# valida-xyz/valida

Measured on AMD Instinct MI355X. Metric: proofs/sec, 2^20-row Fibonacci trace, higher is better.
Workload: dtype u32; 1 GPU; C2: Fibonacci 2^20 cpu rows (mem 2^22), 14 chips, one proof per GPU; field=BabyBear / Ext5, mmcs=Keccak-256, fri_blowup=2, log_blowup=1, num_queries=40, pow_bits=8, parallelism=single GPU, proofs_in_flight_per_gpu=3, comm_stuck=False

## Files before the change

bindings/rust/src/lib.rs:

```rust
#![allow(non_camel_case_types, dead_code)]
use core::ffi::{c_char, c_int, c_void};

pub const VGPU_CBOR_CANONICAL_FIELDS: u32 = 1;
pub const VGPU_CBOR_PLAIN_DIGESTS: u32 = 2;
pub const VGPU_CBOR_IN_BARE_IS_MONTGOMERY: u32 = 1;
pub const VGPU_CBOR_SAW_FIELD_STRUCT: u32 = 1;
pub const VGPU_CBOR_SAW_FIELD_BARE: u32 = 2;
pub const VGPU_CBOR_SAW_DIGEST_STRUCT: u32 = 4;
pub const VGPU_CBOR_SAW_DIGEST_PLAIN: u32 = 8;
pub const VGPU_COMM_ID_BYTES: u32 = 128;
pub const VGPU_OK: i32 = 0;
pub const VGPU_ERR_INVALID_ARG: i32 = -1;
pub const VGPU_ERR_OOM: i32 = -2;
pub const VGPU_ERR_HIP: i32 = -3;
pub const VGPU_ERR_UNSUPPORTED: i32 = -4;
pub const VGPU_ERR_INTERNAL: i32 = -5;
pub const VGPU_ERR_FABRIC: i32 = -6;
pub const VGPU_HASH_KECCAK256: i32 = 0;
pub const VGPU_HASH_POSEIDON16: i32 = 1;
pub const VGPU_CPU_STORE32: i32 = 0;
pub const VGPU_CPU_LOAD32: i32 = 1;
pub const VGPU_CPU_JAL: i32 = 2;
pub const VGPU_CPU_JALV: i32 = 3;
pub const VGPU_CPU_BEQ: i32 = 4;
pub const VGPU_CPU_BNE: i32 = 5;
pub const VGPU_CPU_IMM32: i32 = 6;
pub const VGPU_CPU_BUS: i32 = 7;
pub const VGPU_CPU_BUS_LEFT_IMM: i32 = 8;
pub const VGPU_CPU_STOP: i32 = 9;
pub const VGPU_CPU_LOADFP: i32 = 10;
pub const VGPU_CPU_LOAD_U8: i32 = 11;
pub const VGPU_CPU_LOAD_S8: i32 = 12;
pub const VGPU_CPU_STORE_U8: i32 = 13;
pub const VGPU_CPU_READ_ADVICE: i32 = 14;

#[repr(C)] pub struct VgpuAir { _private: [u8; 0] }
#[repr(C)] pub struct VgpuMachine { _private: [u8; 0] }
#[repr(C)] pub struct VgpuChallenger { _private: [u8; 0] }
#[repr(C)] pub struct VgpuProver { _private: [u8; 0] }
#[repr(C)] pub struct VgpuTrace { _private: [u8; 0] }
#[repr(C)] pub struct VgpuPdata { _private: [u8; 0] }
#[repr(C)] pub struct VgpuProof { _private: [u8; 0] }
#[repr(C)] pub struct VgpuOpening { _private: [u8; 0] }
#[repr(C)] pub struct VgpuVerifier { _private: [u8; 0] }
#[repr(C)] pub struct VgpuTicket { _private: [u8; 0] }
#[repr(C)] pub struct VgpuBusReport { _private: [u8; 0] }
#[repr(C)] pub struct VgpuConstraintReport { _private: [u8; 0] }
#[repr(C)] pub struct VgpuMutationReport { _private: [u8; 0] }
#[repr(C)] pub struct VgpuPairReport { _private: [u8; 0] }
#[repr(C)] pub struct VgpuRankReport { _private: [u8; 0] }
#[repr(C)] pub struct VgpuFieldReport { _private: [u8; 0] }
#[repr(C)] pub struct VgpuLinkReport { _private: [u8; 0] }
#[repr(C)] pub struct VgpuStepReport { _private: [u8; 0] }
#[repr(C)] pub struct VgpuInvariantReport { _private: [u8; 0] }
#[repr(C)] pub struct VgpuTransitionReport { _private: [u8; 0] }
#[repr(C)] pub struct VgpuProductReport { _private: [u8; 0] }
#[repr(C)] pub struct VgpuDomainReport { _private: [u8; 0] }
#[repr(C)] pub struct VgpuMemoryReport { _private: [u8; 0] }
#[repr(C)] pub struct VgpuProgramReport { _private: [u8; 0] }
#[repr(C)] pub struct VgpuCoverageReport { _private: [u8; 0] }
#[repr(C)] pub struct VgpuComm { _private: [u8; 0] }
#[repr(C)] pub struct VgpuOplog { _private: [u8; 0] }
#[repr(C)] pub struct VgpuWorkload { _private: [u8; 0] }

#[repr(C)]
#[derive(Clone, Copy)]
pub struct VgpuConfig {
    pub device: i32,
    pub log_blowup: u32,
    pub num_queries: u32,
    pub pow_bits: u32,
    pub hash_kind: u32,
    pub observe_final_poly: u32,
    pub poseidon_rc: [u32; 480],
    pub interpret_air: u32,
}
#[repr(C)]
#[derive(Clone, Copy)]
pub struct VgpuVcolTerm {
    pub is_preprocessed: u32,
    pub column: u32,
    pub weight: u32,
}
#[repr(C)]
#[derive(Clone, Copy)]
// ... 179 lines not shown
}
#[repr(C)]
#[derive(Clone, Copy)]
pub struct VgpuMemOp {
    pub clk: u32,
    pub addr: u32,
    pub value: u32,
    pub is_write: u32,
}
#[repr(C)]
#[derive(Clone, Copy)]
pub struct VgpuAluOp {
    pub opcode: u32,
    pub a: u32,
    pub b: u32,
    pub c: u32,
}
#[repr(C)]
#[derive(Clone, Copy)]
pub struct VgpuOutOp {
    pub clk: u32,
    pub byte: u32,
}
#[repr(C)]
#[derive(Clone, Copy)]
pub struct VgpuOplogDesc {
    pub struct_size: u64,
    pub cpu: *const VgpuCpuOp,
    pub n_cpu: u64,
    pub mem: *const VgpuMemOp,
    pub n_mem: u64,
    pub alu: [*const VgpuAluOp; 4],
    pub n_alu: [u64; 4],
    pub static_cells: *const u32,
    pub n_static: u64,
    pub rom_len: u32,
    pub alu2: [*const VgpuAluOp; 4],
    pub n_alu2: [u64; 4],
    pub output: *const VgpuOutOp,
    pub n_output: u64,
}

#[link(name = "vgpu")]
extern "C" {
    pub fn vgpu_last_error() -> *const c_char;
    pub fn vgpu_version() -> *const c_char;
    pub fn vgpu_air_new(name: *const c_char, width: u32, preprocessed_width: u32, out: *mut *mut VgpuAir) -> i32;
    pub fn vgpu_air_free(air: *mut VgpuAir);
    pub fn vgpu_air_constant(air: *mut VgpuAir, canonical: u32) -> u32;
    pub fn vgpu_air_variable(air: *mut VgpuAir, is_preprocessed: u32, column: u32, is_next: u32) -> u32;
    pub fn vgpu_air_is_first_row(air: *mut VgpuAir) -> u32;
    pub fn vgpu_air_is_last_row(air: *mut VgpuAir) -> u32;
    pub fn vgpu_air_is_transition(air: *mut VgpuAir) -> u32;
    pub fn vgpu_air_add(air: *mut VgpuAir, a: u32, b: u32) -> u32;
    pub fn vgpu_air_sub(air: *mut VgpuAir, a: u32, b: u32) -> u32;
    pub fn vgpu_air_mul(air: *mut VgpuAir, a: u32, b: u32) -> u32;
    pub fn vgpu_air_neg(air: *mut VgpuAir, a: u32) -> u32;
    pub fn vgpu_air_assert_zero(air: *mut VgpuAir, node: u32);
    pub fn vgpu_air_add_interaction(air: *mut VgpuAir, it: *const VgpuInteraction) -> i32;
    pub fn vgpu_machine_new(out: *mut *mut VgpuMachine) -> i32;
    pub fn vgpu_machine_push_air(m: *mut VgpuMachine, air: *const VgpuAir) -> i32;
    pub fn vgpu_machine_basic(out: *mut *mut VgpuMachine) -> i32;
    pub fn vgpu_machine_basic_via_ffi(out: *mut *mut VgpuMachine) -> i32;
    pub fn vgpu_machine_free(m: *mut VgpuMachine);
    pub fn vgpu_machine_num_chips(m: *const VgpuMachine) -> u32;
    pub fn vgpu_machine_chip_info(m: *const VgpuMachine, chip: u32, out: *mut u32) -> i32;
    pub fn vgpu_machine_interaction_words(m: *const VgpuMachine, chip: u32, out: *mut u32, cap: u64) -> i64;
    pub fn vgpu_machine_eval_constraints(m: *const VgpuMachine, chip: u32, main_local: *const u32, main_next: *const u32, prep_local: *const u32, prep_next: *const u32, is_first: u32, is_last: u32, is_transition: u32, out: *mut u32, cap: u32) -> i32;
    pub fn vgpu_challenger_new(poseidon_rc: *const u32, out: *mut *mut VgpuChallenger) -> i32;
    pub fn vgpu_challenger_free(ch: *mut VgpuChallenger);
    pub fn vgpu_challenger_observe(ch: *mut VgpuChallenger, values: *const u32, n: u64);
    pub fn vgpu_challenger_sample(ch: *mut VgpuChallenger, out: *mut u32, n: u64);
    pub fn vgpu_challenger_sample_bits(ch: *mut VgpuChallenger, bits: u32) -> u64;
    pub fn vgpu_challenger_grind(ch: *mut VgpuChallenger, bits: u32) -> u32;
    pub fn vgpu_poseidon16_permute(poseidon_rc: *const u32, state: *mut u32);
    pub fn vgpu_poseidon16_permute_sparse(poseidon_rc: *const u32, state: *mut u32) -> i32;
    pub fn vgpu_prover_create(cfg: *const VgpuConfig, machine: *const VgpuMachine, out: *mut *mut VgpuProver) -> i32;
    pub fn vgpu_prover_destroy(p: *mut VgpuProver);
    pub fn vgpu_prover_memory(p: *const VgpuProver, live_bytes: *mut u64, peak_bytes: *mut u64);
    pub fn vgpu_prover_trim(p: *mut VgpuProver) -> u64;
    pub fn vgpu_prover_memory_reset_peak(p: *mut VgpuProver);
    pub fn vgpu_prover_set_dense_lane(p: *mut VgpuProver, on: u32, min_nodes: u64);
    pub fn vgpu_prover_set_const_columns(p: *mut VgpuProver, on: u32);
    pub fn vgpu_prover_lane_stats(p: *const VgpuProver, entered: *mut u64, waited: *mut u64);
    pub fn vgpu_prover_set_profiling(p: *mut VgpuProver, on: u32);
    pub fn vgpu_prover_set_prep_cache(p: *mut VgpuProver, on: u32);
    pub fn vgpu_prover_set_profiling_filter(p: *mut VgpuProver, kernel_name: *const c_char);
    pub fn vgpu_prover_profile(p: *mut VgpuProver, out: *mut c_char, cap: u64) -> i64;
    pub fn vgpu_shader_clock_probe(device: i32, iters: u32, out: *mut u64) -> i32;
    pub fn vgpu_host_alloc(bytes: u64, out: *mut *mut c_void) -> i32;
    pub fn vgpu_host_free(ptr: *mut c_void);
    pub fn vgpu_trace_upload(p: *mut VgpuProver, data: *const u32, height: u64, width: u64, out: *mut *mut VgpuTrace) -> i32;
    pub fn vgpu_trace_free(t: *mut VgpuTrace);
    pub fn vgpu_commit_batches(p: *mut VgpuProver, mats: *const *const VgpuTrace, n_mats: u32, coset_shifts: *const u32, root: *mut u32, out: *mut *mut VgpuPdata) -> i32;
    pub fn vgpu_commit_batches_flagged(p: *mut VgpuProver, mats: *const *const VgpuTrace, n_mats: u32, root: *mut u32, out: *mut *mut VgpuPdata, varies_out: *mut u32) -> i32;
    pub fn vgpu_pdata_lde(p: *mut VgpuProver, pd: *const VgpuPdata, idx: u32, out: *mut u32, cap_words: u64) -> i32;
    pub fn vgpu_pdata_num_matrices(pd: *const VgpuPdata) -> u32;
    pub fn vgpu_pdata_lde_view(pd: *const VgpuPdata, idx: u32, out: *mut VgpuLdeView) -> i32;
    pub fn vgpu_pdata_free(pd: *mut VgpuPdata);
    pub fn vgpu_perm_trace(p: *mut VgpuProver, chip: u32, main: *const VgpuTrace, preprocessed_or_null: *const VgpuTrace, challenges: *const u32, out: *mut u32, cap_words: u64, cumulative_sum: *mut u32) -> i32;
    pub fn vgpu_perm_trace_device(p: *mut VgpuProver, chip: u32, main: *const VgpuTrace, preprocessed_or_null: *const VgpuTrace, challenges: *const u32, out: *mut *mut VgpuTrace, cumulative_sum: *mut u32) -> i32;
    pub fn vgpu_quotient(p: *mut VgpuProver, chip: u32, prep_pd: *const VgpuPdata, prep_idx: u32, main_pd: *const VgpuPdata, main_idx: u32, perm_pd: *const VgpuPdata, perm_idx: u32, perm_challenges: *const u32, alpha: *const u32, cumulative_sum: *const u32, out: *mut *mut VgpuTrace) -> i32;
    pub fn vgpu_open_multi_batches(p: *mut VgpuProver, rounds: *const *const VgpuPdata, n_rounds: u32, n_points: *const u32, points: *const u32, ch: *mut VgpuChallenger, out: *mut *mut VgpuOpening) -> i32;
    pub fn vgpu_opening_values_len(o: *const VgpuOpening) -> u64;
    pub fn vgpu_opening_values(o: *const VgpuOpening) -> *const u32;
    pub fn vgpu_opening_proof_len(o: *const VgpuOpening) -> u64;
    pub fn vgpu_opening_proof(o: *const VgpuOpening) -> *const u32;
    pub fn vgpu_opening_free(o: *mut VgpuOpening);
    pub fn vgpu_verify_multi_batches(cfg: *const VgpuConfig, commits: *const u32, n_rounds: u32, n_mats: *const u32, heights: *const u64, widths: *const u32, n_points: *const u32, points: *const u32, values: *const u32, n_value_words: u64, proof: *const u32, n_proof_words: u64, ch: *mut VgpuChallenger) -> i32;
    pub fn vgpu_verify(cfg: *const VgpuConfig, machine: *const VgpuMachine, preprocessed_commit: *const u32, proof_words: *const u32, n_words: u64) -> i32;
    pub fn vgpu_verifier_create(cfg: *const VgpuConfig, machine: *const VgpuMachine, out: *mut *mut VgpuVerifier) -> i32;
    pub fn vgpu_verifier_destroy(v: *mut VgpuVerifier);
    pub fn vgpu_verifier_set_chunk_words(v: *mut VgpuVerifier, chunk_words: u64) -> i32;
    pub fn vgpu_verify_batch(v: *mut VgpuVerifier, proofs: *const *const u32, n_words: *const u64, preprocessed_commits: *const u32, n_proofs: u32, status: *mut i32) -> i32;
    pub fn vgpu_verifier_message(v: *const VgpuVerifier, i: u32, out: *mut c_char, cap: u64) -> i64;
    pub fn vgpu_verifier_timing(v: *const VgpuVerifier, host_ms: *mut f64, device_ms: *mut f64);
    pub fn vgpu_host_commit_root(cfg: *const VgpuConfig, mats: *const *const u32, heights: *const u64, widths: *const u64, n_mats: u32, coset_shifts: *const u32, root: *mut u32) -> i32;
    pub fn vgpu_fri_fold(p: *mut VgpuProver, f: *const u32, n: u64, beta: *const u32, out: *mut u32) -> i32;
    pub fn vgpu_field_probe(p: *mut VgpuProver, op: u32, operands: *const u32, operand_words: u64, n_items: u64, results: *mut u32, result_words: u64) -> i32;
    pub fn vgpu_prover_set_pool_poison(p: *mut VgpuProver, mode: u32, word: u32) -> i32;
    pub fn vgpu_prover_pool_poison_stats(p: *const VgpuProver, out: *mut u64);
    pub fn vgpu_prover_pool_peek(p: *mut VgpuProver, bytes: u64, out: *mut u32, n_words: u64) -> i32;
    pub fn vgpu_verifier_set_poison(v: *mut VgpuVerifier, on: u32, word: u32) -> i32;
    pub fn vgpu_prove(p: *mut VgpuProver, main: *const *const VgpuTrace, n_main: u32, prep_chips: *const u32, prep: *const *const VgpuTrace, n_prep: u32, debug_flags: u32, out: *mut *mut VgpuProof) -> i32;
    pub fn vgpu_prove_async(p: *mut VgpuProver, main: *const *const VgpuTrace, n_main: u32, prep_chips: *const u32, prep: *const *const VgpuTrace, n_prep: u32, out: *mut *mut VgpuTicket) -> i32;
    pub fn vgpu_ticket_wait(t: *mut VgpuTicket, out: *mut *mut VgpuProof) -> i32;
    pub fn vgpu_proof_cbor(proof_words: *const u32, n_words: u64, flags: u32, out: *mut u8, cap_bytes: u64) -> i64;
    pub fn vgpu_proof_from_cbor(bytes: *const u8, n_bytes: u64, out: *mut u32, cap_words: u64) -> i64;
    pub fn vgpu_proof_from_cbor_ex(bytes: *const u8, n_bytes: u64, flags: u32, out: *mut u32, cap_words: u64, forms_seen: *mut u32) -> i64;
    pub fn vgpu_proof_len(pr: *const VgpuProof) -> u64;
    pub fn vgpu_proof_words(pr: *const VgpuProof) -> *const u32;
    pub fn vgpu_proof_phase_ms(pr: *const VgpuProof, out: *mut f64);
    pub fn vgpu_proof_transcript(pr: *const VgpuProof, out: *mut u32);
    pub fn vgpu_proof_debug_perm_trace(pr: *const VgpuProof, chip: u32, out: *mut u32, cap_words: u64) -> i64;
    pub fn vgpu_proof_debug_quotient(pr: *const VgpuProof, chip: u32, out: *mut u32, cap_words: u64) -> i64;
    pub fn vgpu_proof_free(pr: *mut VgpuProof);
    pub fn vgpu_bus_audit(p: *mut VgpuProver, main: *const *const VgpuTrace, n_main: u32, prep_chips: *const u32, prep: *const *const VgpuTrace, n_prep: u32, opts: *const VgpuBusAuditOpts, out: *mut *mut VgpuBusReport) -> i32;
    pub fn vgpu_bus_audit_host(machine: *const VgpuMachine, main: *const *const u32, heights: *const u64, widths: *const u64, n_main: u32, prep_chips: *const u32, prep: *const *const u32, prep_heights: *const u64, prep_widths: *const u64, n_prep: u32, opts: *const VgpuBusAuditOpts, out: *mut *mut VgpuBusReport) -> i32;
    pub fn vgpu_bus_report_len(r: *const VgpuBusReport) -> u64;
    pub fn vgpu_bus_report_words(r: *const VgpuBusReport) -> *const u32;
    pub fn vgpu_bus_report_timing(r: *const VgpuBusReport, out: *mut f64);
    pub fn vgpu_bus_report_free(r: *mut VgpuBusReport);
    pub fn vgpu_constraint_audit(p: *mut VgpuProver, main: *const *const VgpuTrace, n_main: u32, prep_chips: *const u32, prep: *const *const VgpuTrace, n_prep: u32, opts: *const VgpuConstraintAuditOpts, out: *mut *mut VgpuConstraintReport) -> i32;
    pub fn vgpu_constraint_audit_host(machine: *const VgpuMachine, main: *const *const u32, heights: *const u64, widths: *const u64, n_main: u32, prep_chips: *const u32, prep: *const *const u32, prep_heights: *const u64, prep_widths: *const u64, n_prep: u32, opts: *const VgpuConstraintAuditOpts, out: *mut *mut VgpuConstraintReport) -> i32;
    pub fn vgpu_constraint_report_len(r: *const VgpuConstraintReport) -> u64;
    pub fn vgpu_constraint_report_words(r: *const VgpuConstraintReport) -> *const u32;
    pub fn vgpu_constraint_report_timing(r: *const VgpuConstraintReport, out: *mut f64);
    pub fn vgpu_constraint_report_free(r: *mut VgpuConstraintReport);
    pub fn vgpu_mutation_audit(p: *mut VgpuProver, main: *const *const VgpuTrace, n_main: u32, prep_chips: *const u32, prep: *const *const VgpuTrace, n_prep: u32, opts: *const VgpuMutationAuditOpts, out: *mut *mut VgpuMutationReport) -> i32;
    pub fn vgpu_mutation_audit_host(machine: *const VgpuMachine, main: *const *const u32, heights: *const u64, widths: *const u64, n_main: u32, prep_chips: *const u32, prep: *const *const u32, prep_heights: *const u64, prep_widths: *const u64, n_prep: u32, opts: *const VgpuMutationAuditOpts, out: *mut *mut VgpuMutationReport) -> i32;
    pub fn vgpu_mutation_report_len(r: *const VgpuMutationReport) -> u64;
    pub fn vgpu_mutation_report_words(r: *const VgpuMutationReport) -> *const u32;
    pub fn vgpu_mutation_report_timing(r: *const VgpuMutationReport, out: *mut f64);
    pub fn vgpu_mutation_report_free(r: *mut VgpuMutationReport);
    pub fn vgpu_pair_audit(p: *mut VgpuProver, main: *const *const VgpuTrace, n_main: u32, prep_chips: *const u32, prep: *const *const VgpuTrace, n_prep: u32, opts: *const VgpuPairAuditOpts, out: *mut *mut VgpuPairReport) -> i32;
    pub fn vgpu_pair_audit_host(machine: *const VgpuMachine, main: *const *const u32, heights: *const u64, widths: *const u64, n_main: u32, prep_chips: *const u32, prep: *const *const u32, prep_heights: *const u64, prep_widths: *const u64, n_prep: u32, opts: *const VgpuPairAuditOpts, out: *mut *mut VgpuPairReport) -> i32;
    pub fn vgpu_pair_report_len(r: *const VgpuPairReport) -> u64;
    pub fn vgpu_pair_report_words(r: *const VgpuPairReport) -> *const u32;
    pub fn vgpu_pair_report_timing(r: *const VgpuPairReport, out: *mut f64);
    pub fn vgpu_pair_report_free(r: *mut VgpuPairReport);
    pub fn vgpu_rank_audit(p: *mut VgpuProver, main: *const *const VgpuTrace, n_main: u32, prep_chips: *const u32, prep: *const *const VgpuTrace, n_prep: u32, opts: *const VgpuRankAuditOpts, out: *mut *mut VgpuRankReport) -> i32;
    pub fn vgpu_rank_audit_host(machine: *const VgpuMachine, main: *const *const u32, heights: *const u64, widths: *const u64, n_main: u32, prep_chips: *const u32, prep: *const *const u32, prep_heights: *const u64, prep_widths: *const u64, n_prep: u32, opts: *const VgpuRankAuditOpts, out: *mut *mut VgpuRankReport) -> i32;
    pub fn vgpu_rank_report_len(r: *const VgpuRankReport) -> u64;
    pub fn vgpu_rank_report_words(r: *const VgpuRankReport) -> *const u32;
    pub fn vgpu_rank_report_timing(r: *const VgpuRankReport, out: *mut f64);
    pub fn vgpu_rank_report_free(r: *mut VgpuRankReport);
// ... 94 lines not shown
```

include/vgpu.h:

```cpp
#ifndef VGPU_H
#define VGPU_H
#include <stdint.h>
#ifdef __cplusplus
extern "C" {
#endif

enum {
    VGPU_OK = 0,
    VGPU_ERR_INVALID_ARG = -1,
    VGPU_ERR_OOM = -2,
    VGPU_ERR_HIP = -3,
    VGPU_ERR_UNSUPPORTED = -4,
    VGPU_ERR_INTERNAL = -5,
    VGPU_ERR_FABRIC = -6
};
enum {
    VGPU_HASH_KECCAK256 = 0,
    VGPU_HASH_POSEIDON16 = 1
};

const char* vgpu_last_error(void);
const char* vgpu_version(void);

typedef struct vgpu_config {
    int32_t device;
    uint32_t log_blowup;
    uint32_t num_queries;
    uint32_t pow_bits;
    uint32_t hash_kind;
    uint32_t observe_final_poly;
    uint32_t poseidon_rc[480];
    uint32_t interpret_air;
} vgpu_config_t;

typedef struct vgpu_air vgpu_air_t;
typedef struct vgpu_vcol_term { uint32_t is_preprocessed; uint32_t column; uint32_t weight; } vgpu_vcol_term_t;
typedef struct vgpu_vcol { const vgpu_vcol_term_t* terms; uint32_t n_terms; uint32_t constant; } vgpu_vcol_t;
typedef struct vgpu_interaction {
    const vgpu_vcol_t* fields; uint32_t n_fields;
    vgpu_vcol_t count;
    uint32_t is_global;
    uint32_t bus_index;
    uint32_t is_send;
} vgpu_interaction_t;

int32_t vgpu_air_new(const char* name, uint32_t width, uint32_t preprocessed_width, vgpu_air_t** out);
void vgpu_air_free(vgpu_air_t* air);
uint32_t vgpu_air_constant(vgpu_air_t* air, uint32_t canonical);
uint32_t vgpu_air_variable(vgpu_air_t* air, uint32_t is_preprocessed, uint32_t column, uint32_t is_next);
uint32_t vgpu_air_is_first_row(vgpu_air_t* air);
uint32_t vgpu_air_is_last_row(vgpu_air_t* air);
uint32_t vgpu_air_is_transition(vgpu_air_t* air);
uint32_t vgpu_air_add(vgpu_air_t* air, uint32_t a, uint32_t b);
uint32_t vgpu_air_sub(vgpu_air_t* air, uint32_t a, uint32_t b);
uint32_t vgpu_air_mul(vgpu_air_t* air, uint32_t a, uint32_t b);
uint32_t vgpu_air_neg(vgpu_air_t* air, uint32_t a);
void vgpu_air_assert_zero(vgpu_air_t* air, uint32_t node);
int32_t vgpu_air_add_interaction(vgpu_air_t* air, const vgpu_interaction_t* it);

typedef struct vgpu_machine vgpu_machine_t;
int32_t vgpu_machine_new(vgpu_machine_t** out);
int32_t vgpu_machine_push_air(vgpu_machine_t* m, const vgpu_air_t* air);
int32_t vgpu_machine_basic(vgpu_machine_t** out);
int32_t vgpu_machine_basic_via_ffi(vgpu_machine_t** out);
void vgpu_machine_free(vgpu_machine_t* m);
uint32_t vgpu_machine_num_chips(const vgpu_machine_t* m);
int32_t vgpu_machine_chip_info(const vgpu_machine_t* m, uint32_t chip, uint32_t out[8]);
int64_t vgpu_machine_interaction_words(const vgpu_machine_t* m, uint32_t chip, uint32_t* out, uint64_t cap);
int32_t vgpu_machine_eval_constraints(const vgpu_machine_t* m, uint32_t chip, const uint32_t* main_local, const uint32_t* main_next,
                                      const uint32_t* prep_local, const uint32_t* prep_next, uint32_t is_first, uint32_t is_last,
                                      uint32_t is_transition, uint32_t* out, uint32_t cap);

typedef struct vgpu_challenger vgpu_challenger_t;
int32_t vgpu_challenger_new(const uint32_t poseidon_rc[480], vgpu_challenger_t** out);
void vgpu_challenger_free(vgpu_challenger_t* ch);
void vgpu_challenger_observe(vgpu_challenger_t* ch, const uint32_t* values, uint64_t n);
void vgpu_challenger_sample(vgpu_challenger_t* ch, uint32_t* out, uint64_t n);
uint64_t vgpu_challenger_sample_bits(vgpu_challenger_t* ch, uint32_t bits);
uint32_t vgpu_challenger_grind(vgpu_challenger_t* ch, uint32_t bits);
void vgpu_poseidon16_permute(const uint32_t poseidon_rc[480], uint32_t state[16]);
int32_t vgpu_poseidon16_permute_sparse(const uint32_t poseidon_rc[480], uint32_t state[16]);

typedef struct vgpu_prover vgpu_prover_t;
typedef struct vgpu_trace vgpu_trace_t;
typedef struct vgpu_pdata vgpu_pdata_t;
typedef struct vgpu_proof vgpu_proof_t;

int32_t vgpu_prover_create(const vgpu_config_t* cfg, const vgpu_machine_t* machine, vgpu_prover_t** out);
void vgpu_prover_destroy(vgpu_prover_t* p);
void vgpu_prover_memory(const vgpu_prover_t* p, uint64_t* live_bytes, uint64_t* peak_bytes);
uint64_t vgpu_prover_trim(vgpu_prover_t* p);
void vgpu_prover_memory_reset_peak(vgpu_prover_t* p);
void vgpu_prover_set_dense_lane(vgpu_prover_t* p, uint32_t on, uint64_t min_nodes);
void vgpu_prover_set_const_columns(vgpu_prover_t* p, uint32_t on);
void vgpu_prover_lane_stats(const vgpu_prover_t* p, uint64_t* entered, uint64_t* waited);

void vgpu_prover_set_profiling(vgpu_prover_t* p, uint32_t on);
void vgpu_prover_set_prep_cache(vgpu_prover_t* p, uint32_t on);
void vgpu_prover_set_profiling_filter(vgpu_prover_t* p, const char* kernel_name);
int64_t vgpu_prover_profile(vgpu_prover_t* p, char* out, uint64_t cap);
int32_t vgpu_shader_clock_probe(int32_t device, uint32_t iters, uint64_t out[2]);

int32_t vgpu_host_alloc(uint64_t bytes, void** out);
void vgpu_host_free(void* ptr);

int32_t vgpu_trace_upload(vgpu_prover_t* p, const uint32_t* data, uint64_t height, uint64_t width, vgpu_trace_t** out);
void vgpu_trace_free(vgpu_trace_t* t);

int32_t vgpu_commit_batches(vgpu_prover_t* p, const vgpu_trace_t* const* mats, uint32_t n_mats, const uint32_t* coset_shifts,
                            uint32_t root[8], vgpu_pdata_t** out);
int32_t vgpu_commit_batches_flagged(vgpu_prover_t* p, const vgpu_trace_t* const* mats, uint32_t n_mats, uint32_t root[8], vgpu_pdata_t** out,
                                    uint32_t* varies_out);
int32_t vgpu_pdata_lde(vgpu_prover_t* p, const vgpu_pdata_t* pd, uint32_t idx, uint32_t* out, uint64_t cap_words);
typedef struct vgpu_lde_view {
    const uint32_t* data;
    uint64_t height, width, stride;
    uint32_t log_blowup;
} vgpu_lde_view_t;
uint32_t vgpu_pdata_num_matrices(const vgpu_pdata_t* pd);
int32_t vgpu_pdata_lde_view(const vgpu_pdata_t* pd, uint32_t idx, vgpu_lde_view_t* out);
void vgpu_pdata_free(vgpu_pdata_t* pd);

int32_t vgpu_perm_trace(vgpu_prover_t* p, uint32_t chip, const vgpu_trace_t* main, const vgpu_trace_t* preprocessed_or_null,
                        const uint32_t challenges[15], uint32_t* out, uint64_t cap_words, uint32_t cumulative_sum[5]);

int32_t vgpu_perm_trace_device(vgpu_prover_t* p, uint32_t chip, const vgpu_trace_t* main, const vgpu_trace_t* preprocessed_or_null,
                               const uint32_t challenges[15], vgpu_trace_t** out, uint32_t cumulative_sum[5]);

int32_t vgpu_quotient(vgpu_prover_t* p, uint32_t chip, const vgpu_pdata_t* prep_pd, uint32_t prep_idx, const vgpu_pdata_t* main_pd, uint32_t main_idx,
                      const vgpu_pdata_t* perm_pd, uint32_t perm_idx, const uint32_t perm_challenges[15], const uint32_t alpha[5],
                      const uint32_t cumulative_sum[5], vgpu_trace_t** out);

typedef struct vgpu_opening vgpu_opening_t;
int32_t vgpu_open_multi_batches(vgpu_prover_t* p, const vgpu_pdata_t* const* rounds, uint32_t n_rounds, const uint32_t* n_points,
                                const uint32_t* points, vgpu_challenger_t* ch, vgpu_opening_t** out);
uint64_t vgpu_opening_values_len(const vgpu_opening_t* o);
const uint32_t* vgpu_opening_values(const vgpu_opening_t* o);
uint64_t vgpu_opening_proof_len(const vgpu_opening_t* o);
const uint32_t* vgpu_opening_proof(const vgpu_opening_t* o);
void vgpu_opening_free(vgpu_opening_t* o);

int32_t vgpu_verify_multi_batches(const vgpu_config_t* cfg, const uint32_t* commits, uint32_t n_rounds, const uint32_t* n_mats, const uint64_t* heights,
                                  const uint32_t* widths, const uint32_t* n_points, const uint32_t* points, const uint32_t* values, uint64_t n_value_words,
                                  const uint32_t* proof, uint64_t n_proof_words, vgpu_challenger_t* ch);

int32_t vgpu_verify(const vgpu_config_t* cfg, const vgpu_machine_t* machine, const uint32_t* preprocessed_commit, const uint32_t* proof_words,
                    uint64_t n_words);
typedef struct vgpu_verifier vgpu_verifier_t;
int32_t vgpu_verifier_create(const vgpu_config_t* cfg, const vgpu_machine_t* machine, vgpu_verifier_t** out);
void vgpu_verifier_destroy(vgpu_verifier_t* v);
int32_t vgpu_verifier_set_chunk_words(vgpu_verifier_t* v, uint64_t chunk_words);
int32_t vgpu_verify_batch(vgpu_verifier_t* v, const uint32_t* const* proofs, const uint64_t* n_words, const uint32_t* preprocessed_commits,
                          uint32_t n_proofs, int32_t* status);
int64_t vgpu_verifier_message(const vgpu_verifier_t* v, uint32_t i, char* out, uint64_t cap);
void vgpu_verifier_timing(const vgpu_verifier_t* v, double* host_ms, double* device_ms);
int32_t vgpu_host_commit_root(const vgpu_config_t* cfg, const uint32_t* const* mats, const uint64_t* heights, const uint64_t* widths, uint32_t n_mats,
                              const uint32_t* coset_shifts, uint32_t root[8]);

int32_t vgpu_fri_fold(vgpu_prover_t* p, const uint32_t* f, uint64_t n, const uint32_t beta[5], uint32_t* out);

int32_t vgpu_field_probe(vgpu_prover_t* p, uint32_t op, const uint32_t* operands, uint64_t operand_words, uint64_t n_items, uint32_t* results, uint64_t result_words);

int32_t vgpu_prover_set_pool_poison(vgpu_prover_t* p, uint32_t mode, uint32_t word);
void vgpu_prover_pool_poison_stats(const vgpu_prover_t* p, uint64_t out[4]);
int32_t vgpu_prover_pool_peek(vgpu_prover_t* p, uint64_t bytes, uint32_t* out, uint64_t n_words);
int32_t vgpu_verifier_set_poison(vgpu_verifier_t* v, uint32_t on, uint32_t word);

int32_t vgpu_prove(vgpu_prover_t* p, const vgpu_trace_t* const* main, uint32_t n_main, const uint32_t* prep_chips,
                   const vgpu_trace_t* const* prep, uint32_t n_prep, uint32_t debug_flags, vgpu_proof_t** out);
typedef struct vgpu_ticket vgpu_ticket_t;
int32_t vgpu_prove_async(vgpu_prover_t* p, const vgpu_trace_t* const* main, uint32_t n_main, const uint32_t* prep_chips,
                         const vgpu_trace_t* const* prep, uint32_t n_prep, vgpu_ticket_t** out);
int32_t vgpu_ticket_wait(vgpu_ticket_t* t, vgpu_proof_t** out);
#define VGPU_CBOR_CANONICAL_FIELDS 1u
#define VGPU_CBOR_PLAIN_DIGESTS 2u
int64_t vgpu_proof_cbor(const uint32_t* proof_words, uint64_t n_words, uint32_t flags, uint8_t* out, uint64_t cap_bytes);
int64_t vgpu_proof_from_cbor(const uint8_t* bytes, uint64_t n_bytes, uint32_t* out, uint64_t cap_words);
// ... 357 lines not shown
```

valida_amd/__init__.py:

```python
import ctypes
import os

import numpy as np

P = 2013265921
NUM_CHIPS = 14
CHIP_NAMES = ["cpu", "program", "mem", "add", "sub", "mul", "div", "shift", "lt", "com", "bitwise", "output", "range", "static_data"]

_HERE = os.path.dirname(os.path.abspath(__file__))
_LIB_PATH = os.environ.get("VGPU_LIB_PATH") or os.path.join(_HERE, "libvgpu.so")

c_u32p = ctypes.POINTER(ctypes.c_uint32)
c_u64p = ctypes.POINTER(ctypes.c_uint64)


HASH_KECCAK256, HASH_POSEIDON16 = 0, 1


class VgpuError(RuntimeError):
    def __init__(self, code, msg):
        super().__init__("vgpu error %d: %s" % (code, msg))
        self.code = code


class VgpuConfig(ctypes.Structure):
    _fields_ = [
        ("device", ctypes.c_int32),
        ("log_blowup", ctypes.c_uint32),
        ("num_queries", ctypes.c_uint32),
        ("pow_bits", ctypes.c_uint32),
        ("hash_kind", ctypes.c_uint32),
        ("observe_final_poly", ctypes.c_uint32),
        ("poseidon_rc", ctypes.c_uint32 * 480),
        ("interpret_air", ctypes.c_uint32),
    ]


_lib = None


def lib():
    global _lib
    if _lib is None:
        if not os.path.exists(_LIB_PATH):
            raise ImportError("libvgpu.so is not built: run `python valida_amd/build.py` (or __graft_entry__.build())")
        L = ctypes.CDLL(_LIB_PATH)
        L.vgpu_last_error.restype = ctypes.c_char_p
        L.vgpu_version.restype = ctypes.c_char_p
        L.vgpu_proof_len.restype = ctypes.c_uint64
        L.vgpu_proof_words.restype = c_u32p
        L.vgpu_challenger_sample_bits.restype = ctypes.c_uint64
        L.vgpu_proof_debug_perm_trace.restype = ctypes.c_int64
        L.vgpu_proof_debug_quotient.restype = ctypes.c_int64
        L.vgpu_prover_profile.restype = ctypes.c_int64
        L.vgpu_verifier_message.restype = ctypes.c_int64
        L.vgpu_verifier_message.argtypes = [ctypes.c_void_p, ctypes.c_uint32, ctypes.c_char_p, ctypes.c_uint64]
        L.vgpu_verifier_timing.argtypes = [ctypes.c_void_p, ctypes.POINTER(ctypes.c_double), ctypes.POINTER(ctypes.c_double)]
        L.vgpu_verifier_timing.restype = None
        L.vgpu_shader_clock_probe.argtypes = [ctypes.c_int32, ctypes.c_uint32, ctypes.POINTER(ctypes.c_uint64)]
        L.vgpu_shader_clock_probe.restype = ctypes.c_int32
        L.vgpu_workload_from_executable.argtypes = [ctypes.c_char_p, ctypes.c_uint64, ctypes.c_uint32, ctypes.c_char_p, ctypes.c_uint64, ctypes.c_uint64,
                                                    ctypes.POINTER(ctypes.c_void_p)]
        L.vgpu_workload_output.argtypes = [ctypes.c_void_p, ctypes.c_char_p, ctypes.c_uint64]
        L.vgpu_workload_output.restype = ctypes.c_int64
        for name in ("vgpu_air_constant", "vgpu_air_variable", "vgpu_air_is_first_row", "vgpu_air_is_last_row", "vgpu_air_is_transition", "vgpu_air_add",
                     "vgpu_air_sub", "vgpu_air_mul", "vgpu_air_neg", "vgpu_machine_num_chips", "vgpu_challenger_grind"):
            getattr(L, name).restype = ctypes.c_uint32
        _lib = L
    return _lib


def _check(code):
    if code != 0:
        raise VgpuError(code, lib().vgpu_last_error().decode())


def _u32(a):
    a = np.ascontiguousarray(a, dtype=np.uint32)
    return a, a.ctypes.data_as(c_u32p)


def shader_clock_hz(device=0, iters=8192):
    out = (ctypes.c_uint64 * 2)()
    _check(lib().vgpu_shader_clock_probe(ctypes.c_int32(device), ctypes.c_uint32(iters), out))
    return float(out[0]) / float(out[1]) * 1e8


def poseidon_round_constants(seed=0x56414C494441, source="splitmix", **cli_switches):
    if source == "cli":
        from .cli_constants import cli_poseidon_round_constants

        return cli_poseidon_round_constants(**cli_switches)
    if source != "splitmix":
        raise ValueError("source must be 'splitmix' or 'cli'")
    out = []
    x = seed & 0xFFFFFFFFFFFFFFFF
    while len(out) < 480:
        x = (x + 0x9E3779B97F4A7C15) & 0xFFFFFFFFFFFFFFFF
        z = x
# ... 1900 lines not shown

def _coverage_opts(deltas, max_cells, max_workgroups):
    if int(max_cells) < 1:
        raise VgpuError(-1, "coverage_audit: max_cells must be at least 1")
    ds = [int(d) for d in ((1, P - 1) if deltas is None else deltas)]
    if not 1 <= len(ds) <= 4:
        raise VgpuError(-1, "coverage_audit: 1 to 4 deltas (got %d)" % len(ds))
    if any(d < 0 or d > 0xFFFFFFFF for d in ds):
        raise VgpuError(-1, "coverage_audit: a delta must be a canonical value in 1..p-1")
    if not 0 <= int(max_workgroups) <= 0xFFFFFFFF:
        raise VgpuError(-1, "coverage_audit: max_workgroups is a 32-bit count (0: the default)")
    return CoverageAuditOpts(int(max_cells), len(ds), (ctypes.c_uint32 * 4)(*ds), int(max_workgroups), (ctypes.c_uint32 * 2)(0, 0))


def coverage_audit_host(machine, main_matrices, preprocessed, deltas=None, max_cells=8192):
    opts = _coverage_opts(deltas, max_cells, 0)
    return _audit_host("coverage", machine, main_matrices, preprocessed, opts)


_AUDIT_REPORTS = dict(bus=BusReport, constraint=ConstraintReport, mutation=MutationReport, pair=PairReport, rank=RankReport, step=StepReport, invariant=InvariantReport, transition=TransitionReport, product=ProductReport, domain=DomainReport, memory=MemoryReport, program=ProgramReport, field=FieldReport,
                      link=LinkReport, coverage=CoverageReport)


def _report_of(name):
    return lambda h: _audit_report(name, _AUDIT_REPORTS[name], h)


_rank_report, _step_report, _field_report, _link_report = _report_of("rank"), _report_of("step"), _report_of("field"), _report_of("link")

def _pool_poison_from_env(environ):
    text = environ.get("VGPU_POOL_POISON", "").strip()
    if not text:
        return None
    hexa = text[:2] in ("0x", "0X")
    digits = text[2:] if hexa else text
    if not digits or any(ch not in ("0123456789abcdefABCDEF" if hexa else "0123456789") for ch in digits):
        raise ValueError("VGPU_POOL_POISON must be a 32-bit word in decimal or 0x hex, not %r" % text)
    word = int(digits, 16 if hexa else 10)
    if word > 0xFFFFFFFF:
        raise ValueError("VGPU_POOL_POISON must be a 32-bit word (at most 0xFFFFFFFF), not %r" % text)
    return word


class Ticket:

    def __init__(self, handle, keep):
        self._h, self._keep = handle, keep

    def wait(self):
        h = ctypes.c_void_p()
        t, self._h = self._h, None
        _check(lib().vgpu_ticket_wait(t, ctypes.byref(h)))
        self._keep = None
        return Proof(h)

    def __del__(self):
        if getattr(self, "_h", None):
            try:
                self.wait()
            except Exception:
                pass


class Prover:

    def __init__(self, machine, rc, device=0, log_blowup=1, num_queries=40, pow_bits=8, observe_final_poly=False, interpret_air=False, hash_kind=HASH_KECCAK256):
        cfg = VgpuConfig()
        cfg.device, cfg.log_blowup, cfg.num_queries, cfg.pow_bits = device, log_blowup, num_queries, pow_bits
        cfg.hash_kind, cfg.observe_final_poly, cfg.interpret_air = int(hash_kind), int(observe_final_poly), int(interpret_air)
        rc = np.ascontiguousarray(rc, dtype=np.uint32)
        assert rc.size == 480
        ctypes.memmove(cfg.poseidon_rc, rc.ctypes.data, 480 * 4)
        self.machine, self.rc, self.log_blowup, self.num_queries, self.pow_bits = machine, rc, log_blowup, num_queries, pow_bits
        self._h = ctypes.c_void_p()
        lane_off, lane_min = os.environ.get("VGPU_DENSE_LANE", "1") == "0", os.environ.get("VGPU_DENSE_LANE_MIN_NODES", "").strip()
        if lane_min and not lane_min.isdigit():
            raise ValueError("VGPU_DENSE_LANE_MIN_NODES must be a number of leaf rows, not %r" % lane_min)
        poison = _pool_poison_from_env(os.environ)
        _check(lib().vgpu_prover_create(ctypes.byref(cfg), machine._h, ctypes.byref(self._h)))
        if lane_off or int(lane_min or 0) > 0:
            self.set_dense_lane(not lane_off, int(lane_min or 0))
        if os.environ.get("VGPU_CONST_COLS", "1") == "0":
            self.set_const_columns(False)
        if poison is not None:
            self.set_pool_poison(poison)

    def set_const_columns(self, on):
        lib().vgpu_prover_set_const_columns(self._h, ctypes.c_uint32(1 if on else 0))

    def set_dense_lane(self, on, min_nodes=0):
        lib().vgpu_prover_set_dense_lane(self._h, ctypes.c_uint32(1 if on else 0), ctypes.c_uint64(int(min_nodes)))

    def upload(self, matrix):
        m = np.ascontiguousarray(matrix, dtype=np.uint32)
        assert m.ndim == 2
        h = ctypes.c_void_p()
        _check(lib().vgpu_trace_upload(self._h, m.ctypes.data_as(c_u32p), ctypes.c_uint64(m.shape[0]), ctypes.c_uint64(m.shape[1]), ctypes.byref(h)))
        return DeviceTrace(self, h, m.shape)

    def upload_oplog(self, desc):
        h = ctypes.c_void_p()
        _check(lib().vgpu_oplog_upload(self._h, ctypes.byref(desc), ctypes.byref(h)))
        nbytes = 48 * desc.n_cpu + 16 * desc.n_mem + 16 * sum(desc.n_alu) + 8 * desc.n_static
        log = DeviceOplog(self, h, int(nbytes))
        log._desc = desc
        return log

    def generate_trace(self, log, chip):
        h = ctypes.c_void_p()
        _check(lib().vgpu_generate_trace(self._h, log._h, ctypes.c_uint32(chip), ctypes.byref(h)))
        hh, ww = ctypes.c_uint64(), ctypes.c_uint64()
        lib().vgpu_trace_shape(h, ctypes.byref(hh), ctypes.byref(ww))
        return DeviceTrace(self, h, (int(hh.value), int(ww.value)))

    def commit_batches(self, traces, coset_shifts=None):
        arr = (ctypes.c_void_p * len(traces))(*[t._h for t in traces])
        root = np.zeros(8, dtype=np.uint32)
        sh = None
        if coset_shifts is not None:
            shv, sh = _u32(coset_shifts)
        h = ctypes.c_void_p()
        _check(lib().vgpu_commit_batches(self._h, arr, ctypes.c_uint32(len(traces)), sh, root.ctypes.data_as(c_u32p), ctypes.byref(h)))
        return ProverData(self, h, root, [t.shape for t in traces])

    def commit_batches_flagged(self, traces):
        arr = (ctypes.c_void_p * len(traces))(*[t._h for t in traces])
        root = np.zeros(8, dtype=np.uint32)
        varies = np.zeros(sum(t.shape[1] for t in traces), dtype=np.uint32)
        h = ctypes.c_void_p()
        _check(lib().vgpu_commit_batches_flagged(self._h, arr, ctypes.c_uint32(len(traces)), root.ctypes.data_as(c_u32p), ctypes.byref(h), varies.ctypes.data_as(c_u32p)))
        return ProverData(self, h, root, [t.shape for t in traces]), np.split(varies, np.cumsum([t.shape[1] for t in traces])[:-1])

    def generate_permutation_trace(self, chip, main, challenges, preprocessed=None):
        info = self.machine.chip_info(chip)
        n = main.shape[0]
        out = np.zeros((n, 5 * (info["interactions"] + 1)), dtype=np.uint32)
        ch, chp = _u32(challenges)
        cs = np.zeros(5, dtype=np.uint32)
        _check(lib().vgpu_perm_trace(self._h, ctypes.c_uint32(chip), main._h, preprocessed._h if preprocessed is not None else None, chp,
                                     out.ctypes.data_as(c_u32p), ctypes.c_uint64(out.size), cs.ctypes.data_as(c_u32p)))
        return out, cs

    def permutation_trace_device(self, chip, main, challenges, preprocessed=None):
        ch, chp = _u32(challenges)
        cs = np.zeros(5, dtype=np.uint32)
        h = ctypes.c_void_p()
        _check(lib().vgpu_perm_trace_device(self._h, ctypes.c_uint32(chip), main._h, preprocessed._h if preprocessed is not None else None, chp, ctypes.byref(h),
                                            cs.ctypes.data_as(c_u32p)))
        hh, ww = ctypes.c_uint64(), ctypes.c_uint64()
        lib().vgpu_trace_shape(h, ctypes.byref(hh), ctypes.byref(ww))
        return DeviceTrace(self, h, (int(hh.value), int(ww.value))), cs

    def quotient(self, chip, main_pd, main_idx, perm_pd, perm_idx, perm_challenges, alpha, cumulative_sum, prep_pd=None, prep_idx=0):
        a, ap = _u32(perm_challenges)
        b, bp = _u32(alpha)
        c, cp = _u32(cumulative_sum)
        h = ctypes.c_void_p()
        _check(lib().vgpu_quotient(self._h, ctypes.c_uint32(chip), prep_pd._h if prep_pd is not None else None, ctypes.c_uint32(prep_idx), main_pd._h,
                                   ctypes.c_uint32(main_idx), perm_pd._h, ctypes.c_uint32(perm_idx), ap, bp, cp, ctypes.byref(h)))
        hh, ww = ctypes.c_uint64(), ctypes.c_uint64()
        lib().vgpu_trace_shape(h, ctypes.byref(hh), ctypes.byref(ww))
        return DeviceTrace(self, h, (int(hh.value), int(ww.value)))

    def open_multi_batches(self, rounds, points, challenger):
        arr = (ctypes.c_void_p * len(rounds))(*[r._h for r in rounds])
        n_points = np.array([len(pts) for rnd in points for pts in rnd], dtype=np.uint32)
        flat = np.array([w for rnd in points for pts in rnd for z in pts for w in z], dtype=np.uint32)
        h = ctypes.c_void_p()
# ... 172 lines not shown
```

valida_amd/csrc/capi.cpp:

```cpp
#include "../../include/vgpu.h"
#include <algorithm>
#include <cstring>
#include <future>
#include <map>
#include <mutex>
#include <memory>
#include <string>
#include "host/cbor.hpp"
#include "host/comm.hpp"
#include "host/sharded.hpp"
#include "host/sharded_prover.hpp"
#include "host/verifier.hpp"
#include "host/machine_verifier.hpp"
#include "host/verify_batch.hpp"
#include "host/poseidon_opt.hpp"
#include "host/prover.hpp"
#include "workload/basic_vm.hpp"
#include "workload/executable.hpp"

using namespace vhost;

static thread_local std::string g_err;
static int32_t fail(int32_t code, const std::string& msg) { g_err = msg; return code; }
#define VG_TRY(...)                                                         \
// ... 237 lines not shown
        for (auto& f : it.fields) vcol(f);
    }
    if (out && cap >= w.size()) memcpy(out, w.data(), w.size() * 4);
    return (int64_t)w.size();
}
int32_t vgpu_machine_eval_constraints(const vgpu_machine_t* m, uint32_t chip, const uint32_t* main_local, const uint32_t* main_next,
                                      const uint32_t* prep_local, const uint32_t* prep_next, uint32_t is_first, uint32_t is_last,
                                      uint32_t is_transition, uint32_t* out, uint32_t cap) {
    try {
        if (!m || chip >= m->desc.airs.size()) throw std::invalid_argument("bad chip index");
        const AirDesc& a = m->desc.airs[chip];
        std::vector<Fp> ml(a.width), mn(a.width), pl(a.prep_width), pn(a.prep_width);
        for (uint32_t i = 0; i < a.width; i++) { ml[i] = Fp::from_canonical(main_local[i]); mn[i] = Fp::from_canonical(main_next[i]); }
        for (uint32_t i = 0; i < a.prep_width; i++) { pl[i] = Fp::from_canonical(prep_local[i]); pn[i] = Fp::from_canonical(prep_next[i]); }
        vair::HostEval ev{ml.data(), mn.data(), pl.data(), pn.data(), Fp::from_canonical(is_first), Fp::from_canonical(is_last), Fp::from_canonical(is_transition)};
        auto vals = ev.run(a.program);
        if (vals.size() > cap) throw std::invalid_argument("output buffer too small");
        for (size_t i = 0; i < vals.size(); i++) out[i] = vals[i].canonical();
        return (int32_t)vals.size();
    } catch (const std::exception& e) { return fail(VGPU_ERR_INVALID_ARG, e.what()); }
}

int32_t vgpu_challenger_new(const uint32_t rc[480], vgpu_challenger_t** out) {
    VG_TRY({
        if (!rc || !out) throw std::invalid_argument("null argument");
        auto* c = new vgpu_challenger();
        c->perm.reset(new Poseidon16(rc));
        c->ch.reset(new Challenger(c->perm.get()));
        *out = c;
    })
}
void vgpu_challenger_free(vgpu_challenger_t* ch) { delete ch; }
void vgpu_challenger_observe(vgpu_challenger_t* ch, const uint32_t* v, uint64_t n) { for (uint64_t i = 0; i < n; i++) ch->ch->observe_canonical(v[i]); }
void vgpu_challenger_sample(vgpu_challenger_t* ch, uint32_t* out, uint64_t n) { for (uint64_t i = 0; i < n; i++) out[i] = ch->ch->sample().canonical(); }
uint64_t vgpu_challenger_sample_bits(vgpu_challenger_t* ch, uint32_t bits) { return ch->ch->sample_bits(bits); }
uint32_t vgpu_challenger_grind(vgpu_challenger_t* ch, uint32_t bits) { return ch->ch->grind(bits); }
void vgpu_poseidon16_permute(const uint32_t rc[480], uint32_t state[16]) {
    Poseidon16 p(rc);
    Fp st[16];
    for (int i = 0; i < 16; i++) st[i] = Fp::from_canonical(state[i]);
    p.permute(st);
    for (int i = 0; i < 16; i++) state[i] = st[i].canonical();
}

int32_t vgpu_poseidon16_permute_sparse(const uint32_t rc[480], uint32_t state[16]) {
    Poseidon16 p(rc);
    PoseidonOptTables t(p);
    if (!t.valid) return VGPU_ERR_UNSUPPORTED;
    Fp st[16];
    for (int i = 0; i < 16; i++) st[i] = Fp::from_canonical(state[i]);
    t.permute(p, st);
    for (int i = 0; i < 16; i++) state[i] = st[i].canonical();
    return VGPU_OK;
}

int32_t vgpu_prover_create(const vgpu_config_t* cfg, const vgpu_machine_t* machine, vgpu_prover_t** out) {
    VG_TRY({
        if (!cfg || !machine || !out) throw std::invalid_argument("null argument");
        if (cfg->hash_kind != VGPU_HASH_KECCAK256 && cfg->hash_kind != VGPU_HASH_POSEIDON16) { g_err = "hash_kind must be VGPU_HASH_KECCAK256 or VGPU_HASH_POSEIDON16"; return VGPU_ERR_UNSUPPORTED; }
        if (cfg->log_blowup < 1 || cfg->log_blowup > 4) throw std::invalid_argument("log_blowup must be in 1..4");
        int count = 0;
        if (hipGetDeviceCount(&count) != hipSuccess || count <= cfg->device) throw std::runtime_error("hip: no usable device (the product path has no CPU fallback)");
        FriParams fp;
        fp.log_blowup = cfg->log_blowup; fp.num_queries = cfg->num_queries; fp.pow_bits = cfg->pow_bits; fp.observe_final_poly = cfg->observe_final_poly != 0;
        fp.interpret_air = cfg->interpret_air != 0;
        fp.hash_kind = (int)cfg->hash_kind;
        auto* p = new vgpu_prover();
        p->p.reset(new Prover(cfg->device, machine->desc, cfg->poseidon_rc, fp));
        *out = p;
    })
}
void vgpu_prover_destroy(vgpu_prover_t* p) { delete p; }
void vgpu_prover_memory(const vgpu_prover_t* p, uint64_t* live, uint64_t* peak) {
    auto& c = const_cast<vgpu_prover_t*>(p)->p->ctx();
    if (live) *live = c.live;
    if (peak) *peak = c.peak_live;
}
void vgpu_prover_set_const_columns(vgpu_prover_t* p, uint32_t on) {
    if (!p) return;
    DeviceCtx& c = p->p->ctx();
    std::lock_guard<std::mutex> lk(c.prove_mu);
    c.const_cols_on = on != 0;
}
void vgpu_prover_set_dense_lane(vgpu_prover_t* p, uint32_t on, uint64_t min_nodes) {
    if (!p) return;
    DeviceCtx& c = p->p->ctx();
    std::lock_guard<std::mutex> lk(c.prove_mu);
    c.lane_on = on != 0;
    if (min_nodes) c.lane_min_nodes = min_nodes;
}
void vgpu_prover_lane_stats(const vgpu_prover_t* p, uint64_t* entered, uint64_t* waited) {
    if (!p) return;
    auto& c = const_cast<vgpu_prover_t*>(p)->p->ctx();
    if (entered) *entered = c.lane_entered.load();
    if (waited) *waited = c.lane_waited.load();
}
void vgpu_prover_memory_reset_peak(vgpu_prover_t* p) {
    if (!p) return;
    DeviceCtx& c = p->p->ctx();
    std::lock_guard<std::mutex> lk(c.pool_mu);
    c.peak_live = c.live;
}
uint64_t vgpu_prover_trim(vgpu_prover_t* p) {
    if (!p) return 0;
    DeviceCtx& c = p->p->ctx();
    (void)hipSetDevice(c.device);
    return (uint64_t)c.trim();
}
void vgpu_prover_set_profiling(vgpu_prover_t* p, uint32_t on) {
    auto& c = p->p->ctx();
    c.profiler.reset();
    c.profiler.enabled = on != 0;
}
int32_t vgpu_shader_clock_probe(int32_t device, uint32_t iters, uint64_t out[2]) {
    VG_TRY({
        if (!out || !iters) throw std::invalid_argument("shader_clock_probe: null output or zero iterations");
        struct Probe { hipStream_t st = nullptr; uint64_t* buf = nullptr; };
        static std::mutex mu;
        static std::map<int, Probe> probes;
        std::lock_guard<std::mutex> lk(mu);
        VG_HIP_CHECK(hipSetDevice(device));
        Probe& pr = probes[device];
        if (!pr.st) {
            VG_HIP_CHECK(hipStreamCreateWithFlags(&pr.st, hipStreamNonBlocking));
            VG_HIP_CHECK(hipHostMalloc((void**)&pr.buf, 64));
        }
        pr.buf[0] = pr.buf[1] = 0;
        vk::launch_clock_probe(pr.st, pr.buf, iters);
        VG_HIP_CHECK(hipStreamSynchronize(pr.st));
        if (!pr.buf[1]) throw std::runtime_error("hip: the clock probe wrote nothing");
        out[0] = pr.buf[0]; out[1] = pr.buf[1];
    })
}
void vgpu_prover_set_prep_cache(vgpu_prover_t* p, uint32_t on) { if (p) p->p->set_prep_cache(on != 0); }
void vgpu_prover_set_profiling_filter(vgpu_prover_t* p, const char* kernel_name) { p->p->ctx().profiler.only = kernel_name ? kernel_name : ""; }
int64_t vgpu_prover_profile(vgpu_prover_t* p, char* out, uint64_t cap) {
    std::string s;
    {
        DeviceCtx& c = p->p->ctx();
        (void)hipSetDevice(c.device);
        (void)hipDeviceSynchronize();
        c.profiler.collect();
    }
    for (auto& kv : p->p->ctx().profiler.stats) {
        char line[256];
        snprintf(line, sizeof line, "%s %llu %.6f %.0f %.0f\n", kv.first.c_str(), (unsigned long long)kv.second.launches, kv.second.ms, kv.second.bytes,
                 kv.second.valu_ops);
        s += line;
    }
    if (out && cap > s.size()) memcpy(out, s.c_str(), s.size() + 1);
    return (int64_t)s.size() + 1;
}
int32_t vgpu_host_alloc(uint64_t bytes, void** out) {
    VG_TRY({
        if (!out || !bytes) throw std::invalid_argument("vgpu_host_alloc: null output or zero size");
        void* ptr = nullptr;
        hipError_t e = hipHostMalloc(&ptr, bytes, hipHostMallocPortable);
        if (e == hipErrorOutOfMemory) throw std::bad_alloc();
        if (e != hipSuccess) throw std::runtime_error(std::string("hipHostMalloc: ") + hipGetErrorString(e));
        *out = ptr;
    })
}
void vgpu_host_free(void* ptr) { if (ptr) (void)hipHostFree(ptr); }
int32_t vgpu_trace_upload(vgpu_prover_t* p, const uint32_t* data, uint64_t height, uint64_t width, vgpu_trace_t** out) {
    VG_TRY({
        if (!p || !data || !out || !height || !width) throw std::invalid_argument("bad trace");
        std::unique_ptr<vgpu_trace> t(new vgpu_trace());
        t->owner = p->p;
        p->p->ctx().activate();
        t->t = p->p->upload_trace(HostMatrix{data, height, width});
        *out = t.release();
    })
}
void vgpu_trace_free(vgpu_trace_t* t) { delete t; }
void vgpu_trace_shape(const vgpu_trace_t* t, uint64_t* height, uint64_t* width) { *height = t->t->height; *width = t->t->width; }
int32_t vgpu_trace_download(vgpu_prover_t* p, const vgpu_trace_t* t, uint32_t* out, uint64_t cap_words) {
    VG_TRY({
        if (!p || !t || !out) throw std::invalid_argument("null argument");
        if (cap_words < t->t->height * t->t->width) throw std::invalid_argument("output buffer too small");
        p->p->ctx().activate();
        p->p->download_trace(*t->t, out);
    })
}
static HostOplog checked_oplog(const vgpu_oplog_desc_t* log) {
    if (log->struct_size != sizeof(vgpu_oplog_desc_t))
        throw std::invalid_argument("oplog: struct_size " + std::to_string(log->struct_size) + " is not this library's sizeof(vgpu_oplog_desc_t) = " + std::to_string(sizeof(vgpu_oplog_desc_t)) +
                                    " (host compiled against another vgpu.h?)");
    HostOplog h;
    h.cpu = (const vk::TgCpuOp*)log->cpu; h.n_cpu = log->n_cpu;
    h.mem = (const vk::TgMemOp*)log->mem; h.n_mem = log->n_mem;
// ... 20 lines not shown
    }
    for (uint64_t i = 1; i < h.n_static; i++)
        if (log->static_cells[2 * i] <= log->static_cells[2 * i - 2]) throw std::invalid_argument("oplog: static cells must be in ascending address order");
    if (!h.n_cpu || !log->cpu) throw std::invalid_argument("oplog: empty cpu log");
    if ((h.n_mem && !log->mem) || (h.n_static && !log->static_cells)) throw std::invalid_argument("oplog: null log with a nonzero length");
    for (int k = 0; k < 4; k++) if (h.n_alu[k] && !h.alu[k]) throw std::invalid_argument("oplog: null ALU log with a nonzero length");
    for (uint64_t i = 0; i < h.n_cpu; i++) {
        const vgpu_cpu_op_t& o = log->cpu[i];
        if (o.mem_first > h.n_mem || (i && o.mem_first < log->cpu[i - 1].mem_first) || o.kind > VGPU_CPU_READ_ADVICE)
            throw std::invalid_argument("oplog: cpu record " + std::to_string(i) + " is malformed");
        if (h.rom_len && o.pc >= h.rom_len) throw std::invalid_argument("oplog: cpu record " + std::to_string(i) + ": pc beyond the ROM length");
        if (o.kind == VGPU_CPU_BUS || o.kind == VGPU_CPU_BUS_LEFT_IMM) {
            using namespace vchips;
            const uint32_t op = o.opcode;
            const bool known = (op >= OP_ADD32 && op <= OP_SLE32) || op == OP_WRITE;
            if (!known) throw std::invalid_argument("oplog: cpu record " + std::to_string(i) + ": opcode " + std::to_string(op) + " is no bus operation of the BasicMachine's chips");
        }
    }
    for (uint64_t i = 1; i < h.n_mem; i++)
        if (log->mem[i].clk < log->mem[i - 1].clk) throw std::invalid_argument("oplog: memory log entry " + std::to_string(i) + " is out of clock order");
    return h;
}
int32_t vgpu_oplog_validate(const vgpu_oplog_desc_t* log) {
    VG_TRY({
        if (!log) throw std::invalid_argument("null argument");
        checked_oplog(log);
    })
}
int32_t vgpu_oplog_upload(vgpu_prover_t* p, const vgpu_oplog_desc_t* log, vgpu_oplog_t** out) {
    VG_TRY({
        if (!p || !log || !out) throw std::invalid_argument("null argument");
        const HostOplog h = checked_oplog(log);
        p->p->ctx().activate();
        std::unique_ptr<vgpu_oplog> l(new vgpu_oplog());
        l->owner = p->p;
        l->log = p->p->upload_oplog(h);
        *out = l.release();
    })
}
void vgpu_oplog_free(vgpu_oplog_t* log) { delete log; }
int32_t vgpu_generate_trace(vgpu_prover_t* p, const vgpu_oplog_t* log, uint32_t chip, vgpu_trace_t** out) {
    VG_TRY({
        if (!p || !log || !out) throw std::invalid_argument("null argument");
        p->p->ctx().activate();
        std::unique_ptr<vgpu_trace> t(new vgpu_trace());
        t->owner = p->p;
        t->t = p->p->generate_trace(*log->log, (int)chip);
        *out = t.release();
    })
}

static DMat ingest(DeviceCtx& c, const DeviceTrace& t) {
    if (t.height & (t.height - 1)) throw std::invalid_argument("matrix height must be a power of two");
    DMat m(&c, t.height, t.width);
    if (!t.nat.empty()) VG_HIP_CHECK(hipMemcpyAsync(m.data, t.nat.data, t.height * t.width * 4, hipMemcpyDeviceToDevice, c.stream));
    else vk::launch_ingest(c.stream, t.raw.data, m.view(), false);
    return m;
}

int32_t vgpu_commit_batches(vgpu_prover_t* p, const vgpu_trace_t* const* mats, uint32_t n_mats, const uint32_t* coset_shifts, uint32_t root[8],
                            vgpu_pdata_t** out) {
    VG_TRY({
        if (!p || !mats || !n_mats || !root || !out) throw std::invalid_argument("null argument");
        DeviceCtx& c = p->p->ctx();
        c.activate();
        std::vector<DMat> nat;
        for (uint32_t i = 0; i < n_mats; i++) { if (!mats[i] || mats[i]->owner != p->p) throw std::invalid_argument("null trace or trace of another prover"); nat.push_back(ingest(c, *mats[i]->t)); }
        std::vector<CommitInput> in;
        for (uint32_t i = 0; i < n_mats; i++) in.push_back({&nat[i], mats[i]->t->nat_rows_bitrev, mats[i]->t->nat_rows_bitrev});
        std::vector<Fp> shifts;
        if (coset_shifts) for (uint32_t i = 0; i < n_mats; i++) shifts.push_back(Fp::from_canonical(coset_shifts[i]));
        std::unique_ptr<vgpu_pdata> pd(new vgpu_pdata());
        pd->owner = p->p;
        pd->pd = commit_batches(&c, in, coset_shifts ? &shifts : nullptr, p->p->fri());
        memcpy(root, pd->pd->tree.root, 32);
        *out = pd.release();
    })
}
int32_t vgpu_commit_batches_flagged(vgpu_prover_t* p, const vgpu_trace_t* const* mats, uint32_t n_mats, uint32_t root[8], vgpu_pdata_t** out, uint32_t* varies_out) {
    VG_TRY({
        if (!p || !mats || !n_mats || !root || !out) throw std::invalid_argument("null argument");
        DeviceCtx& c = p->p->ctx();
        c.activate();
        size_t words = 0;
        for (uint32_t i = 0; i < n_mats; i++) {
            if (!mats[i] || mats[i]->owner != p->p) throw std::invalid_argument("null trace or trace of another prover");
            const DeviceTrace& t = *mats[i]->t;
            if (!t.nat.empty()) throw std::invalid_argument("commit_batches_flagged: uploaded (row-major) matrices only");
            if (t.height == 0 || (t.height & (t.height - 1))) throw std::invalid_argument("matrix height must be a power of two");
            words += t.width;
        }
        DBuf flags(&c, words);
        VG_HIP_CHECK(hipMemsetAsync(flags.data, 0, words * 4, c.stream));
        std::vector<DMat> nat;
        std::vector<CommitInput> in;
        size_t off = 0;
        for (uint32_t i = 0; i < n_mats; i++) {
            const DeviceTrace& t = *mats[i]->t;
            nat.emplace_back(&c, t.height, t.width);
            vk::launch_ingest(c.stream, t.raw.data, nat.back().view(), false, flags.data + off);
            off += t.width;
        }
        off = 0;
        for (uint32_t i = 0; i < n_mats; i++) { in.push_back({&nat[i], false, false, c.const_cols_on ? flags.data + off : nullptr}); off += nat[i].width; }
        std::unique_ptr<vgpu_pdata> pd(new vgpu_pdata());
        pd->owner = p->p;
        pd->pd = commit_batches(&c, in, nullptr, p->p->fri());
        memcpy(root, pd->pd->tree.root, 32);
        if (varies_out) c.download(varies_out, flags.data, words * 4);
        *out = pd.release();
    })
}
int32_t vgpu_pdata_lde(vgpu_prover_t* p, const vgpu_pdata_t* pd, uint32_t idx, uint32_t* out, uint64_t cap_words) {
    VG_TRY({
        if (!p || !pd || idx >= pd->pd->ldes.size() || !out) throw std::invalid_argument("bad argument");
        DeviceCtx& c = p->p->ctx();
        c.activate();
        const DMat& l = pd->pd->ldes[idx];
        if (cap_words < l.height * l.width) throw std::invalid_argument("output buffer too small");
        DBuf tmp(&c, (size_t)(l.height * l.width));
        vk::launch_export_rows(c.stream, l.view(), 0, l.height, tmp.data);
        c.download(out, tmp.data, l.height * l.width * 4);
    })
}
uint32_t vgpu_pdata_num_matrices(const vgpu_pdata_t* pd) { return pd ? (uint32_t)pd->pd->ldes.size() : 0; }
int32_t vgpu_pdata_lde_view(const vgpu_pdata_t* pd, uint32_t idx, vgpu_lde_view_t* out) {
    VG_TRY({
        if (!pd || !out || idx >= pd->pd->ldes.size()) throw std::invalid_argument("bad argument");
        const DMat& l = pd->pd->ldes[idx];
        out->data = l.data; out->height = l.height; out->width = l.width; out->stride = l.height;
        out->log_blowup = pd->owner->fri().log_blowup;
    })
}
void vgpu_pdata_free(vgpu_pdata_t* pd) { delete pd; }

static Ext5 ext_of(const uint32_t* w) { Ext5 e; for (int k = 0; k < 5; k++) e.c[k] = Fp::from_canonical(w[k]); return e; }

int32_t vgpu_perm_trace_device(vgpu_prover_t* p, uint32_t chip, const vgpu_trace_t* main, const vgpu_trace_t* prep, const uint32_t challenges[15],
                               vgpu_trace_t** out, uint32_t cumulative_sum[5]) {
    VG_TRY({
        if (!p || !main || !challenges || !out) throw std::invalid_argument("null argument");
        const MachineDesc& md = p->p->machine();
        if (chip >= md.airs.size()) throw std::invalid_argument("bad chip index");
        if (main->t->width != md.airs[chip].width) throw std::invalid_argument("trace width mismatch");
        DeviceCtx& c = p->p->ctx();
        c.activate();
        DMat m = ingest(c, *main->t);
        DMat pm;
        if (prep) pm = ingest(c, *prep->t);
        Ext5 rnd[3] = {ext_of(challenges), ext_of(challenges + 5), ext_of(challenges + 10)};
        Ext5 cs;
        std::unique_ptr<vgpu_trace> t(new vgpu_trace());
        t->owner = p->p;
        t->t = std::make_shared<DeviceTrace>();
        t->t->nat = p->p->permutation_trace((int)chip, m, prep ? &pm : nullptr, rnd, &cs);
        t->t->height = t->t->nat.height; t->t->width = t->t->nat.width;
        if (cumulative_sum) for (int k = 0; k < 5; k++) cumulative_sum[k] = cs.c[k].canonical();
        *out = t.release();
    })
}

int32_t vgpu_quotient(vgpu_prover_t* p, uint32_t chip, const vgpu_pdata_t* prep_pd, uint32_t prep_idx, const vgpu_pdata_t* main_pd, uint32_t main_idx,
                      const vgpu_pdata_t* perm_pd, uint32_t perm_idx, const uint32_t perm_challenges[15], const uint32_t alpha[5],
                      const uint32_t cumulative_sum[5], vgpu_trace_t** out) {
    VG_TRY({
        if (!p || !main_pd || !perm_pd || !perm_challenges || !alpha || !cumulative_sum || !out) throw std::invalid_argument("null argument");
// ... 1219 lines not shown
```

valida_amd/csrc/host/pcs.hpp:

```cpp
#pragma once
#include <algorithm>
#include <functional>
#include <memory>
#include "fri_params.hpp"
#include "runtime.hpp"

namespace vhost {


struct ColMat {
    uint64_t height = 0;
    std::vector<const uint32_t*> cols;
};

struct DeviceTree {
    static constexpr uint64_t TOP_FIRST_LEN = 256;
    DeviceCtx* ctx = nullptr;
    std::vector<DBuf> layers;
    std::vector<uint64_t> layer_len;
    unsigned log_max_height = 0;
    uint32_t root[8] = {0};
    static constexpr uint64_t DROP_MIN_LEAVES = 1ull << 16;
    bool drop_bottom = false;
    unsigned dropped = 0;
// ... 96 lines not shown
            mid.block_len = vk::KECCAK_LEVELS_BLOCK_LEN;
            if (leaves_in_mid) {
                if (mid.prev != layers[0].data) throw std::logic_error("mmcs: leaf prologue without a launch over the leaf layer");
                mid.leaf_base = single_view->data; mid.leaf_stride = single_view->stride; mid.leaf_elems = (int)single_view->width; mid.leaf_rows = maxh;
            }
            vk::launch_keccak_levels(st, mid);
            mid.levels = 0;
        };
        for (uint64_t len = maxh / 2; len >= 1; len /= 2) {
            layers.emplace_back(c, (size_t)len * 8);
            layer_len.push_back(len);
            const Group* inj = (gi < groups.size() && groups[gi].height == len) ? &groups[gi] : nullptr;
            if (inj && before_injection_) { (*before_injection_)(); before_injection_ = nullptr; }
            if (pos ? vk::poseidon_levels_take(len) : (len <= TOP_FIRST_LEN || vk::keccak_levels_fused(len))) lane_guard.leave();
            if (pos) {
                if (!vk::poseidon_levels_take(len)) vk::launch_poseidon_compress(st, tab, c->poseidon_sparse, layers[layers.size() - 2].data, inj ? pd + inj->first : nullptr, inj ? (int)inj->count : 0, len, layers.back().data);
                else {
                    if (pgrp.levels && vk::poseidon_levels_group(len) != pgroup) flush_pos(false);
                    pgroup = vk::poseidon_levels_group(len);
                    add_level(pgrp, len, inj);
                }
            } else if (len > TOP_FIRST_LEN) {
                if (vk::keccak_levels_fused(len)) add_level(mid, len, inj);
                else vk::launch_keccak_compress(st, layers[layers.size() - 2].data, inj ? pd + inj->first : nullptr, inj ? (int)inj->count : 0, len,
                                                layers.back().data);
            } else {
                flush_mid();
                add_level(top, len, inj);
            }
            if (inj) gi++;
            if (len == 1) break;
        }
        lane_guard.leave();
        flush_mid();
        if (leaves_in_mid && layers.size() < 2) throw std::logic_error("mmcs: leaf prologue on a tree without parents");
        if (leaves_in_top) {
            if (!top.levels || top.prev != layers[0].data) throw std::logic_error("mmcs: leaf prologue without a top launch over the leaf layer");
            top.leaf_base = single_view->data; top.leaf_stride = single_view->stride; top.leaf_elems = (int)single_view->width; top.leaf_rows = maxh;
        }
        flush_pos(true);
        if (challenger_ && !pos) {
            if (!top.levels) throw std::logic_error("mmcs: the challenger epilogue needs a tree with at least one parent layer");
            top.ch_pos = challenger_->pos; top.ch_state = challenger_->state; top.ch_beta5 = challenger_->beta5; top.ch_commit8 = challenger_->commit8;
        }
        if (top.levels) vk::launch_keccak_top(st, top);
        if (gi != groups.size()) throw std::runtime_error("mmcs: matrix heights must be powers of two >= 1 and <= max height");
        c->check_launch("mmcs build");
        dropped = 0;
        if (drop_bottom && st == c->stream && !c->in_section && maxh >= DROP_MIN_LEAVES && layers.size() >= 4) {
            leaf_elems = (int)groups[0].count;
            if (single) { leaf_ptr = single_view->data; leaf_stride = single_view->stride; }
            else { leaf_ptr = pd + groups[0].first; leaf_stride = 0; }
            layers[0] = DBuf();
            dropped = 1;
            if (!(groups.size() > 1 && groups[1].height == maxh / 2)) { layers[1] = DBuf(); dropped = 2; }
        }
        if (fetch_root) c->download_small(root, layers.back().data, 32);
        if (!fetch_root || dropped) ptr_table_ = std::move(ptr_buf);
    }

};

struct ProverData {
    std::vector<DMat> ldes;
    DeviceTree tree;
};

struct CommitInput {
    DMat* mat;
    bool rows_bitrev;
    bool consume;
    const uint32_t* varies = nullptr;
};

inline DMat coset_lde(DeviceCtx* c, hipStream_t st, const CommitInput& in, unsigned log_blowup, Fp lde_shift) {
    const uint64_t n = in.mat->height, b = 1ull << log_blowup;
    if (n == 0 || (n & (n - 1))) throw std::invalid_argument("commit: matrix heights must be powers of two");
    if (vg::log2_strict_u64(n) + log_blowup > 27)
        throw std::invalid_argument("commit: LDE height 2^" + std::to_string(vg::log2_strict_u64(n) + log_blowup) + " exceeds the field's two-adicity (2^27)");
    const unsigned k = vg::log2_strict_u64(n);
    static const bool fused = [] { const char* e = getenv("VGPU_LDE_FUSED"); return !(e && e[0] == '0'); }();
    if (!in.rows_bitrev && fused) {
        DMat lde(c, n * b, in.mat->width);
        const vk::LdeTables lt = c->lde_tables((int)k, (int)log_blowup, lde_shift);
        DMat s1, s2;
        if (k > 12) { s1 = DMat(c, n, in.mat->width); s2 = DMat(c, n * b, in.mat->width); }
        DBuf colmap;
        if (in.varies && k > 12) {
            colmap = DBuf(c, vk::lde_colmap_words(in.mat->width));
            vk::launch_lde_colmap(st, in.varies, in.mat->width, colmap.data);
        }
        vk::launch_lde_natural(st, in.mat->view(), lde.view(), (int)log_blowup, c->tables, lt, s1.empty() ? vk::DMatView{nullptr, 0, 0, 0} : s1.view(),
                               s2.empty() ? vk::DMatView{nullptr, 0, 0, 0} : s2.view(), colmap.data);
        c->check_launch("coset_lde");
        return lde;
    }
    DMat coeffs;
    if (in.rows_bitrev && in.consume) coeffs = std::move(*in.mat);
    else {
        coeffs = DMat(c, n, in.mat->width);
        if (in.rows_bitrev) VG_HIP_CHECK(hipMemcpyAsync(coeffs.data, in.mat->data, n * in.mat->width * 4, hipMemcpyDeviceToDevice, st));
        else vk::launch_bitrev_rows(st, in.mat->view(), coeffs.view());
    }
    vk::launch_intt(st, coeffs.view(), c->tables);
    DMat lde(c, n * b, coeffs.width);
    Fp w = vg::two_adic_generator(k + log_blowup), wt = Fp::one();
    for (uint64_t t = 0; t < b; t++) {
        uint64_t block = vg::reverse_bits_len((uint32_t)t, log_blowup);
        vk::launch_coset_ntt(st, coeffs.view(), lde.view(), block * n, lde_shift * wt, c->tables);
        wt *= w;
    }
    c->check_launch("coset_lde");
    return lde;
}

struct CommitRider {
    const std::vector<CommitInput>* mats;
    std::unique_ptr<ProverData>* out;
};
inline std::unique_ptr<ProverData> commit_batches(DeviceCtx* c, const std::vector<CommitInput>& mats, const std::vector<Fp>* coset_shifts,
                                                  const FriParams& fri, const CommitRider* rider = nullptr) {
    auto pd = std::make_unique<ProverData>();
    Fp g = Fp::from_canonical(vg::GENERATOR);
    uint64_t maxh = 0;
    for (auto& m : mats) maxh = std::max<uint64_t>(maxh, m.mat->height);
    Section lde_section(c);
    if (rider) {
        auto rp = std::make_unique<ProverData>();
        hipStream_t ax = c->aux[0];
        for (auto& m : *rider->mats) rp->ldes.push_back(coset_lde(c, ax, m, fri.log_blowup, g));
        std::vector<vk::DMatView> rviews;
        for (auto& l : rp->ldes) rviews.push_back(l.view());
        rp->tree.build(c, rviews, false, nullptr, nullptr, ax);
        VG_HIP_CHECK(hipMemcpyAsync(c->rider_root_pin, rp->tree.layers.back().data, 32, hipMemcpyDeviceToHost, ax));
        *rider->out = std::move(rp);
    }
    pd->ldes.resize(mats.size());
    for (int pass = 0; pass < 2; pass++)
        for (size_t i = 0; i < mats.size(); i++) {
            const bool tallest = mats[i].mat->height == maxh;
            if (tallest != (pass == 0)) continue;
            Fp shift = coset_shifts ? g * (*coset_shifts)[i].inv() : g;
            hipStream_t st = c->stream_for(i, mats[i].mat->height);
            pd->ldes[i] = coset_lde(c, st, mats[i], fri.log_blowup, shift);
        }
    std::vector<vk::DMatView> views;
    for (auto& l : pd->ldes) views.push_back(l.view());
    lde_section.join();
    pd->tree.drop_bottom = true;
    pd->tree.build(c, views);
    if (rider) {
        VG_HIP_CHECK(hipStreamSynchronize(c->aux[0]));
        memcpy((*rider->out)->tree.root, c->rider_root_pin, 32);
    }
    return pd;
}

}
```

valida_amd/csrc/host/prover.cpp:

```cpp
#include "prover.hpp"
#include "poseidon_opt.hpp"

namespace vhost {

static Ext5 ext_from_canonical(const uint32_t* w) { Ext5 e; for (int k = 0; k < 5; k++) e.c[k] = Fp::from_canonical(w[k]); return e; }
static void ext_to_canonical(const Ext5& e, uint32_t* w) { for (int k = 0; k < 5; k++) w[k] = e.c[k].canonical(); }

Prover::Prover(int device, const MachineDesc& machine, const uint32_t* poseidon_rc480, const FriParams& fri)
    : ctx_(new DeviceCtx(device)), machine_(machine), fri_(fri), perm16_(poseidon_rc480) {
    for (auto& a : machine_.airs) {
        if (a.log_quotient_degree < 1 || a.log_quotient_degree > 3) throw std::invalid_argument("chip " + a.name + ": log_quotient_degree must be 1..3");
        if (a.native_chip != -2 && (a.native_chip < 0 || a.native_chip >= 14)) throw std::invalid_argument("chip " + a.name + ": native_chip must be a BasicMachine chip id (0..13) or -2 (captured AIR)");
        if (a.log_quotient_degree != 1 && a.native_chip >= 0) throw std::invalid_argument("chip " + a.name + ": the compiled chip kernels assume log_quotient_degree = 1");
        if (fri_.log_blowup < a.log_quotient_degree)
            throw std::invalid_argument("chip " + a.name + ": log_blowup must be >= log_quotient_degree (the quotient domain must lie inside the committed LDE)");
        std::vector<uint32_t> pw(a.program.instrs.size() * 2 + 2, 0);
        if (!a.program.instrs.empty()) memcpy(pw.data(), a.program.instrs.data(), a.program.instrs.size() * 8);
        prog_dev_.emplace_back(ctx_.get(), pw);
        iw_dev_.emplace_back(ctx_.get(), a.interaction_words);
    }
    bool sparse = false;
    const std::vector<uint32_t> pos = poseidon_device_image(poseidon_rc480, perm16_, sparse);
    pow_pos_ = DBuf(ctx_.get(), pos);
    VG_HIP_CHECK(hipHostMalloc((void**)&cs_pinned_, CS_PINNED_WORDS * 4));
// ... 193 lines not shown
DMat Prover::permutation_trace(int chip, const DMat& main_nat, const DMat* prep_nat, const Ext5 rnd[3], Ext5* cumulative_sum) {
    DeviceCtx& c = *ctx_;
    const AirDesc& air = machine_.airs.at((size_t)chip);
    const uint32_t M = (uint32_t)air.interactions.size();
    std::vector<uint32_t> pool;
    size_t maxf = 0;
    for (auto& it : air.interactions) { put_ext(pool, (it.is_local() ? rnd[0] : rnd[1]).pow((uint64_t)it.bus_index + 1)); maxf = std::max(maxf, it.fields.size()); }
    Ext5 bp = Ext5::one();
    for (size_t j = 0; j < maxf; j++) { put_ext(pool, bp); bp *= rnd[2]; }
    pool.push_back(0);
    DBuf pool_dev(&c, pool), scratch(&c, (size_t)vk::perm_scratch_words(main_nat.height));
    DMat perm(&c, main_nat.height, 5 * (M + 1));
    vk::launch_perm_trace(c.stream, main_nat.view(), prep_nat ? prep_nat->view() : vk::DMatView{nullptr, 0, 0, 0}, iw_dev_[chip].data, pool_dev.data, M, perm.view(), scratch.data, fri_.interpret_air ? -2 : machine_.airs[(size_t)chip].native_chip);
    c.check_launch("perm trace");
    if (cumulative_sum) {
        GatherList gl;
        const uint64_t n = main_nat.height;
        gl.add(perm.data + (uint64_t)(5 * M) * n + (n - 1), n, 5, 0);
        DBuf gd(&c, gl.desc), gout(&c, 8);
        vk::launch_gather(c.stream, gd.data, gl.n(), gout.data);
        uint32_t cs[5];
        c.download(cs, gout.data, 20);
        *cumulative_sum = ext_from_canonical(cs);
    } else c.sync();
    return perm;
}

DMat Prover::quotient_chunks(int chip, const DMat& main_lde, const DMat& perm_lde, const DMat* prep_lde, const Ext5 rnd[3], const Ext5& alpha,
                             const Ext5& cumulative_sum) {
    DeviceCtx& c = *ctx_;
    const AirDesc& air = machine_.airs.at((size_t)chip);
    const unsigned lb = fri_.log_blowup;
    const unsigned log_n = vg::log2_strict_u64(main_lde.height) - lb;
    if (main_lde.width != air.width || perm_lde.width != 5 * (air.interactions.size() + 1) || perm_lde.height != main_lde.height ||
        (air.prep_width && (!prep_lde || prep_lde->width != air.prep_width || prep_lde->height != main_lde.height)))
        throw std::invalid_argument("quotient: LDE shapes do not match chip " + air.name);
    std::vector<uint32_t> pool;
    vk::QuotientArgs a{};
    a.K = quotient_consts(air, rnd, alpha, cumulative_sum, pool);
    DBuf pool_dev(&c, pool);
    fill_quotient_args(a, chip, main_lde.view(), perm_lde.view(), prep_lde ? prep_lde->view() : vk::DMatView{nullptr, 0, 0, 0}, log_n, pool_dev.data);
    DMat q(&c, 1ull << log_n, 5ull << air.log_quotient_degree);
    a.out = q.view();
    vk::launch_quotient(c.stream, a, c.tables);
    c.check_launch("quotient");
    c.sync();
    return q;
}

void Prover::fill_quotient_args(vk::QuotientArgs& a, int chip, vk::DMatView main_lde, vk::DMatView perm_lde, vk::DMatView prep_lde, unsigned log_n, const uint32_t* consts_dev) {
    const AirDesc& air = machine_.airs[(size_t)chip];
    const Fp s = Fp::from_canonical(vg::GENERATOR);
    a.main_lde = main_lde; a.perm_lde = perm_lde; a.prep_lde = prep_lde;
    a.log_n = (int)log_n;
    a.prog = (const vair::Instr*)prog_dev_[chip].data;
    a.n_instrs = (uint32_t)air.program.instrs.size();
    a.n_regs = air.program.num_regs;
    a.n_air_asserts = air.program.num_asserts;
    a.native_chip = fri_.interpret_air ? vk::QuotientArgs::INTERPRET : air.native_chip;
    a.iw = iw_dev_[chip].data;
    a.consts = consts_dev;
    a.coset_shift = s.v;
    a.coset_shift_inv = s.inv().v;
    a.lqd = (int)air.log_quotient_degree;
    const Fp sn = s.exp_power_of_2(log_n), wq = vg::two_adic_generator(air.log_quotient_degree);
    Fp wp = Fp::one();
    for (unsigned r = 0; r < (1u << air.log_quotient_degree); r++) { Fp z = sn * wp - Fp::one(); a.zh[r] = z.v; a.zh_inv[r] = z.inv().v; wp *= wq; }
    a.g_inv = vg::two_adic_generator(log_n).inv().v;
}


std::vector<uint32_t> Prover::prove(const std::vector<const DeviceTrace*>& main, const std::vector<std::pair<int, const DeviceTrace*>>& preprocessed,
                                    PhaseTimes* times, ProveDebugOut* dbg) {
    DeviceCtx& c = *ctx_;
    c.activate();
    std::unique_lock<std::mutex> one_at_a_time(c.prove_mu);
    c.activate();
    struct Running {
        std::atomic<int>& n;
        explicit Running(std::atomic<int>& a) : n(a) { n.fetch_add(1); }
        ~Running() { n.fetch_sub(1); }
    } running(c.proofs_running);
    struct LaneOpen { explicit LaneOpen(const DeviceCtx* x) { DeviceCtx::lane_thread_ctx() = x; } ~LaneOpen() { DeviceCtx::lane_thread_ctx() = nullptr; } } lane_open(&c);
    const size_t NC = machine_.airs.size();
    if (main.size() != NC) throw std::invalid_argument("prove: need one main trace per chip");
    const Fp s = Fp::from_canonical(vg::GENERATOR);
    const unsigned lb = fri_.log_blowup;
    Challenger ch(&perm16_);
    PhaseTimes tm;
    auto t_total = Clock::now();
    auto t0 = Clock::now();

    std::vector<unsigned> log_deg(NC);
    std::vector<DMat> main_own(NC);
    std::vector<const DMat*> main_nat(NC);
    const size_t NO_FLAGS = (size_t)-1;
    std::vector<size_t> main_flags(NC, NO_FLAGS), prep_flags(preprocessed.size(), NO_FLAGS);
    size_t flag_words = 0;
    auto wants_flags = [&](const DeviceTrace* t) { return c.const_cols_on && t->nat.empty() && t->height > (1ull << 12) && t->width <= vk::INGEST_FLAGS_MAX_WIDTH; };
    for (size_t i = 0; i < NC; i++)
        if (wants_flags(main[i])) { main_flags[i] = flag_words; flag_words += main[i]->width; }
    for (size_t k = 0; k < preprocessed.size(); k++)
        if (wants_flags(preprocessed[k].second)) { prep_flags[k] = flag_words; flag_words += preprocessed[k].second->width; }
    DBuf flags;
    if (flag_words) {
        flags = DBuf(&c, flag_words);
        VG_HIP_CHECK(hipMemsetAsync(flags.data, 0, flag_words * 4, c.stream));
    }
    auto flags_at = [&](size_t off) -> uint32_t* { return off == NO_FLAGS ? nullptr : flags.data + off; };
    Section ingest_section(&c);
    for (size_t i = 0; i < NC; i++) {
        if (main[i]->width != machine_.airs[i].width) throw std::invalid_argument("prove: trace width mismatch for chip " + machine_.airs[i].name);
        uint64_t h = main[i]->height;
        if (h == 0 || (h & (h - 1))) throw std::invalid_argument("prove: trace heights must be powers of two");
        log_deg[i] = vg::log2_strict_u64(h);
        if (!main[i]->nat.empty()) { main_nat[i] = &main[i]->nat; continue; }
        main_own[i] = DMat(&c, h, main[i]->width);
        main_nat[i] = &main_own[i];
        vk::launch_ingest(c.stream_for(i, h), main[i]->raw.data, main_own[i].view(), false, flags_at(main_flags[i]));
    }
    std::vector<std::pair<int, uint64_t>> prep_key;
    for (auto& pr : preprocessed) prep_key.emplace_back(pr.first, pr.second->uid);
    const bool prep_hit = prep_cache_enabled_ && !prep_key.empty() && prep_key == prep_key_ && prep_pd_cache_;
    if (!prep_hit) { prep_key_.clear(); prep_pd_cache_.reset(); prep_nat_cache_.clear(); prep_nat_cache_.resize(preprocessed.size()); }
    std::vector<DMat>& prep_nat = prep_nat_cache_;
    struct DropPrep { Prover* p; ~DropPrep() { if (!p->prep_cache_enabled_) { p->prep_key_.clear(); p->prep_pd_cache_.reset(); p->prep_nat_cache_.clear(); } } } drop_prep{this};
    std::vector<int> prep_slot(NC, -1);
    for (size_t k = 0; k < preprocessed.size(); k++) {
        const DeviceTrace* t = preprocessed[k].second;
        int chip = preprocessed[k].first;
        if (chip < 0 || (size_t)chip >= NC || prep_slot[chip] >= 0) throw std::invalid_argument("prove: bad or repeated preprocessed chip index");
        if (t->width != machine_.airs[chip].prep_width || t->height != main[chip]->height) throw std::invalid_argument("prove: preprocessed trace shape mismatch");
        prep_slot[chip] = (int)k;
        if (prep_hit) continue;
        prep_nat[k] = DMat(&c, t->height, t->width);
        if (!t->nat.empty())
            VG_HIP_CHECK(hipMemcpyAsync(prep_nat[k].data, t->nat.data, t->height * t->width * 4, hipMemcpyDeviceToDevice, c.stream_for(k, t->height)));
        else
            vk::launch_ingest(c.stream_for(k, t->height), t->raw.data, prep_nat[k].view(), false, flags_at(prep_flags[k]));
    }
    ingest_section.join();
    c.check_launch("ingest");
    tm.ingest = ms_since(t0);

    t0 = Clock::now();
    ProverData* prep_pd = nullptr;
    std::vector<CommitInput> prep_in;
    const bool ride = !prep_nat.empty() && !prep_hit;
    if (ride)
        for (size_t k = 0; k < prep_nat.size(); k++) prep_in.push_back({&prep_nat[k], false, false, flags_at(prep_flags[k])});
    std::unique_ptr<ProverData> main_pd;
    {
        std::vector<CommitInput> in;
        for (size_t i = 0; i < NC; i++) in.push_back({const_cast<DMat*>(main_nat[i]), false, false, flags_at(main_flags[i])});
        const CommitRider rider{&prep_in, &prep_pd_cache_};
        main_pd = commit_batches(&c, in, nullptr, fri_, ride ? &rider : nullptr);
    }
    if (!prep_nat.empty()) {
        if (!prep_hit && prep_cache_enabled_) prep_key_ = prep_key;
        prep_pd = prep_pd_cache_.get();
        ch.observe_digest(prep_pd->tree.root);
    }
    ch.observe_digest(main_pd->tree.root);
    tm.commit_main = ms_since(t0);

    t0 = Clock::now();
// ... 67 lines not shown
            uint32_t M = (uint32_t)air.interactions.size(), K = air.program.num_asserts + M + 3;
            Ks[i] = K;
            off[i] = pool.size();
            Ext5 pw = Ext5::one();
            std::vector<Ext5> ap(K);
            for (uint32_t k = 0; k < K; k++) { ap[K - 1 - k] = pw; pw *= rnd[2]; }
            for (auto& e : ap) put_ext(pool, e);
            for (auto& e : bus_alphas[i]) put_ext(pool, e);
            for (auto& e : betas[i]) put_ext(pool, e);
            put_ext(pool, cumulative_sums[i]);
        }
        DBuf pool_dev(&c, pool);
        std::vector<uint32_t> init(2 * NC, 0xffffffffu);
        DBuf bad_dev(&c, init);
        for (size_t i = 0; i < NC; i++) {
            auto& air = machine_.airs[i];
            vk::QuotientArgs a{};
            a.main_lde = main_nat[i]->view();
            a.perm_lde = perm_nat[i].view();
            a.prep_lde = prep_slot[i] >= 0 ? prep_nat[prep_slot[i]].view() : vk::DMatView{nullptr, 0, 0, 0};
            a.log_n = (int)log_deg[i];
            a.prog = (const vair::Instr*)prog_dev_[i].data;
            a.n_instrs = (uint32_t)air.program.instrs.size();
            a.n_regs = air.program.num_regs;
            a.n_air_asserts = air.program.num_asserts;
            a.iw = iw_dev_[i].data;
            a.consts = pool_dev.data + off[i];
            a.K = Ks[i];
            a.native_chip = fri_.interpret_air ? vk::QuotientArgs::INTERPRET : air.native_chip;
            vk::launch_check_constraints(c.stream, a, reinterpret_cast<unsigned long long*>(bad_dev.data) + i);
        }
        c.check_launch("check_constraints");
        std::vector<uint32_t> bad(2 * NC);
        c.download(bad.data(), bad_dev.data, bad.size() * 4);
        for (size_t i = 0; i < NC; i++) {
            const uint64_t v = ((uint64_t)bad[2 * i + 1] << 32) | bad[2 * i];
            if (v == ~0ull) continue;
            const uint64_t row = v >> 16;
            const uint32_t code = (uint32_t)(v & 0xffff);
            std::string what = code == 0xFFFE ? "a permutation (bus) constraint" : code == 0xFFFD ? "an AIR constraint" : "AIR constraint " + std::to_string(code);
            throw std::invalid_argument("check_constraints: chip " + machine_.airs[i].name + ": " + what + " is not satisfied on row " + std::to_string(row));
        }
        Ext5 total = Ext5::zero();
        for (auto& s5 : cumulative_sums) total += s5;
        if (!total.is_zero()) throw std::invalid_argument("check_cumulative_sums: the chips' cumulative sums do not cancel (a bus is unbalanced)");
    }
    t0 = Clock::now();
    std::unique_ptr<ProverData> perm_pd;
    {
        std::vector<CommitInput> in;
        for (auto& m : perm_nat) in.push_back({&m, false, false});
        perm_pd = commit_batches(&c, in, nullptr, fri_);
    }
    ch.observe_digest(perm_pd->tree.root);
    read_cumulative_sums();
    perm_nat.clear();
    main_own.clear();
    tm.commit_perm = ms_since(t0);

    t0 = Clock::now();
    const Ext5 alpha = ch.sample_ext();
    std::vector<DMat> quot(NC);
    std::vector<char> quot_is_natural(NC, 0);
    std::vector<Fp> quot_shifts(NC);
    {
        std::vector<uint32_t> pool;
        std::vector<size_t> off(NC);
        std::vector<uint32_t> Ks(NC);
        uint32_t maxK = 0;
        for (size_t i = 0; i < NC; i++) maxK = std::max<uint32_t>(maxK, machine_.airs[i].program.num_asserts + (uint32_t)machine_.airs[i].interactions.size() + 3);
        std::vector<Ext5> apow_all(maxK);
        { Ext5 p = Ext5::one(); for (auto& e : apow_all) { e = p; p *= alpha; } }
        for (size_t i = 0; i < NC; i++) {
            auto& air = machine_.airs[i];
            uint32_t M = (uint32_t)air.interactions.size(), K = air.program.num_asserts + M + 3;
            Ks[i] = K;
            off[i] = pool.size();
            for (uint32_t k = 0; k < K; k++) put_ext(pool, apow_all[K - 1 - k]);
            for (auto& e : bus_alphas[i]) put_ext(pool, e);
            for (auto& e : betas[i]) put_ext(pool, e);
            put_ext(pool, cumulative_sums[i]);
        }
        DBuf pool_dev(&c, pool);
        Section quotient_section(&c);
        for (size_t i = 0; i < NC; i++) {
            auto& air = machine_.airs[i];
            vk::QuotientArgs a{};
            fill_quotient_args(a, (int)i, main_pd->ldes[i].view(), perm_pd->ldes[i].view(),
                               prep_slot[i] >= 0 ? prep_pd->ldes[prep_slot[i]].view() : vk::DMatView{nullptr, 0, 0, 0}, log_deg[i], pool_dev.data + off[i]);
            a.K = Ks[i];
            quot[i] = DMat(&c, 1ull << log_deg[i], 5ull << air.log_quotient_degree);
            a.out = quot[i].view();
            a.out_natural = air.log_quotient_degree == 1 ? 1 : 0;
            quot_is_natural[i] = a.out_natural != 0;
            vk::launch_quotient(c.stream_for(i, 1ull << log_deg[i]), a, c.tables);
            quot_shifts[i] = s.exp_power_of_2(air.log_quotient_degree);
        }
        quotient_section.join();
        c.check_launch("quotient");
    }
    tm.quotient = ms_since(t0);
    if (dbg && dbg->keep_matrices) {
        dbg->quotient_chunks.resize(NC);
        for (size_t i = 0; i < NC; i++) {
            auto& q = quot[i];
            DMat nat(&c, q.height, q.width);
            if (q.height > 1 && !quot_is_natural[i]) vk::launch_bitrev_rows(c.stream, q.view(), nat.view());
            else VG_HIP_CHECK(hipMemcpyAsync(nat.data, q.data, q.height * q.width * 4, hipMemcpyDeviceToDevice, c.stream));
            DBuf tmp(&c, (size_t)(q.height * q.width));
            vk::launch_export_rows(c.stream, nat.view(), 0, q.height, tmp.data);
            dbg->quotient_chunks[i].resize(q.height * q.width);
            c.download(dbg->quotient_chunks[i].data(), tmp.data, dbg->quotient_chunks[i].size() * 4);
        }
    }
    t0 = Clock::now();
    std::unique_ptr<ProverData> quot_pd;
    {
        std::vector<CommitInput> in;
        for (size_t i = 0; i < quot.size(); i++) in.push_back({&quot[i], !quot_is_natural[i], !quot_is_natural[i]});
        quot_pd = commit_batches(&c, in, &quot_shifts, fri_);
    }
    ch.observe_digest(quot_pd->tree.root);
    quot.clear();
    tm.commit_quotient = ms_since(t0);

    const Ext5 zeta = ch.sample_ext();
    std::vector<OpenRound> rounds(3);
    rounds[0].pd = main_pd.get(); rounds[1].pd = perm_pd.get(); rounds[2].pd = quot_pd.get();
    for (size_t i = 0; i < NC; i++) {
        Fp g = vg::two_adic_generator(log_deg[i]);
        rounds[0].points.push_back({zeta, zeta * g});
        rounds[1].points.push_back({zeta, zeta * g});
        rounds[2].points.push_back({zeta.exp_power_of_2(machine_.airs[i].log_quotient_degree)});
    }
    PcsOpening opening = open_multi_batches(rounds, ch);
    tm.open_values = opening.ms_values; tm.open_reduce = opening.ms_reduce; tm.fri = opening.ms_fri;
    t0 = Clock::now();
    const auto& opened = opening.opened;

    std::vector<uint32_t> pw;
    {
        size_t chip_words = 26;
        for (size_t i = 0; i < NC; i++) chip_words += 11 + 5 * (2 * machine_.airs[i].width + 10 * (machine_.airs[i].interactions.size() + 1) + 10);
        pw.reserve(chip_words + opening.proof_words.size());
    }
    pw.push_back(PROOF_MAGIC);
    pw.push_back((uint32_t)NC);
    for (int k = 0; k < 8; k++) pw.push_back(main_pd->tree.root[k]);
    for (int k = 0; k < 8; k++) pw.push_back(perm_pd->tree.root[k]);
    for (int k = 0; k < 8; k++) pw.push_back(quot_pd->tree.root[k]);
    auto put_vec = [&](const std::vector<Ext5>& v) {
        pw.push_back((uint32_t)v.size());
        for (auto& e : v) { uint32_t w5[5]; ext_to_canonical(e, w5); pw.insert(pw.end(), w5, w5 + 5); }
    };
    for (size_t i = 0; i < NC; i++) {
        pw.push_back(log_deg[i]);
        put_vec(opened[0][i][0]); put_vec(opened[0][i][1]);
        put_vec(opened[1][i][0]); put_vec(opened[1][i][1]);
        put_vec(opened[2][i][0]);
        uint32_t w5[5]; ext_to_canonical(cumulative_sums[i], w5); pw.insert(pw.end(), w5, w5 + 5);
    }
    pw.insert(pw.end(), opening.proof_words.begin(), opening.proof_words.end());
    tm.queries = opening.ms_queries + ms_since(t0);
    c.profiler.collect();
    tm.total = ms_since(t_total);
    if (times) *times = tm;
    if (dbg) {
        if (prep_pd) memcpy(dbg->prep_root, prep_pd->tree.root, 32); else memset(dbg->prep_root, 0, 32);
        for (int i = 0; i < 3; i++) ext_to_canonical(rnd[i], dbg->perm_challenges + 5 * i);
        ext_to_canonical(alpha, dbg->alpha);
// ... 431 lines not shown
```

valida_amd/csrc/host/runtime.hpp:

```cpp
#pragma once
#include <new>
#include <cstdio>
#include <cstdlib>
#include <hip/hip_runtime.h>
#include <cstring>
#include <atomic>
#include <map>
#include <mutex>
#include <stdexcept>
#include <string>
#include <tuple>
#include <vector>
#include "../kernels/launch.hpp"
#include "dense_lane.hpp"

namespace vhost {
using vg::Ext5;
using vg::Fp;

struct HipLaneApi {
    using Event = hipEvent_t;
    using Stream = hipStream_t;
    static Event create() { hipEvent_t e = nullptr; VG_HIP_CHECK(hipEventCreateWithFlags(&e, hipEventDisableTiming)); return e; }
    static void destroy(Event e) noexcept { if (e) (void)hipEventDestroy(e); }
    static bool record(Event e, Stream s) noexcept { return hipEventRecord(e, s) == hipSuccess; }
    static void wait(Stream s, Event e) { VG_HIP_CHECK(hipStreamWaitEvent(s, e, 0)); }
};
using HipDenseLane = DenseLane<HipLaneApi>;
inline HipDenseLane& dense_lane_of(int device) {
    static std::mutex* mu = new std::mutex;
    static std::map<int, HipDenseLane*>* lanes = new std::map<int, HipDenseLane*>;
    std::lock_guard<std::mutex> lk(*mu);
    HipDenseLane*& l = (*lanes)[device];
    if (!l) l = new HipDenseLane;
    return *l;
}

struct DeviceCtx {
    int device = 0;
    hipStream_t stream = nullptr;
    vk::DeviceTables tables{};
    std::multimap<size_t, void*> free_blocks;
    std::map<void*, size_t> live_blocks;
    size_t bytes_allocated = 0, peak_live = 0, live = 0;
    uint32_t* table_mem = nullptr;
    void* pinned = nullptr;
    size_t pinned_bytes = 0;
    uint8_t* stage = nullptr;
    static constexpr size_t STAGE_BYTES = 16u << 20;
    size_t stage_pos = 0;
    vk::Profiler profiler;
    int hash_kind = 0;
    const uint32_t* poseidon_tab = nullptr;
    bool poseidon_sparse = false;
    static constexpr int NUM_AUX = 1;
    hipStream_t aux[NUM_AUX] = {};
    hipEvent_t fork_ev = nullptr, join_ev[NUM_AUX] = {};
    hipEvent_t rider_ev = nullptr;
    uint32_t* rider_root_pin = nullptr;
    bool in_section = false;
    HipDenseLane* lane = nullptr;
    HipDenseLane::SlotPtr lane_slot;
    bool lane_on = true;
    uint64_t lane_min_nodes = 1ull << 18;
    std::atomic<uint64_t> lane_entered{0}, lane_waited{0};
    static const DeviceCtx*& lane_thread_ctx() { static thread_local const DeviceCtx* c = nullptr; return c; }
    bool lane_open_here() const { return lane_on && lane && lane_thread_ctx() == this; }
    bool const_cols_on = true;
    std::vector<void*> deferred;
    std::mutex pool_mu;
    uint32_t poison_mode = 0, poison_word = 0;
    uint64_t poison_stats[4] = {0, 0, 0, 0};
    std::atomic<int> proofs_running{0};
    std::atomic<int> async_pending{0};
    std::mutex prove_mu;
    std::mutex upload_mu;
    hipStream_t upload_stream = nullptr;
    hipEvent_t upload_ev = nullptr;

    explicit DeviceCtx(int dev) : device(dev) {
        VG_HIP_CHECK(hipSetDevice(dev));
        VG_HIP_CHECK(hipStreamCreateWithFlags(&stream, hipStreamNonBlocking));
        for (int i = 0; i < NUM_AUX; i++) {
            VG_HIP_CHECK(hipStreamCreateWithFlags(&aux[i], hipStreamNonBlocking));
            VG_HIP_CHECK(hipEventCreateWithFlags(&join_ev[i], hipEventDisableTiming));
        }
        VG_HIP_CHECK(hipEventCreateWithFlags(&fork_ev, hipEventDisableTiming));
        VG_HIP_CHECK(hipEventCreateWithFlags(&rider_ev, hipEventDisableTiming));
        VG_HIP_CHECK(hipHostMalloc((void**)&rider_root_pin, 64));
        lane = &dense_lane_of(dev);
        lane_slot = std::make_shared<HipDenseLane::Slot>();
        init_tables();
    }
    void activate() {
        VG_HIP_CHECK(hipSetDevice(device));
        vk::g_profiler = &profiler;
    }
    ~DeviceCtx() {
        if (vk::g_profiler == &profiler) vk::g_profiler = nullptr;
        (void)hipSetDevice(device);
        (void)hipStreamSynchronize(stream);
        if (lane) lane->retire(lane_slot);
        for (int i = 0; i < NUM_AUX; i++) { (void)hipStreamSynchronize(aux[i]); (void)hipStreamDestroy(aux[i]); (void)hipEventDestroy(join_ev[i]); }
        (void)hipEventDestroy(fork_ev);
        if (rider_ev) (void)hipEventDestroy(rider_ev);
        if (rider_root_pin) (void)hipHostFree(rider_root_pin);
        if (sync_ev) (void)hipEventDestroy(sync_ev);
        for (auto& kv : free_blocks) (void)hipFree(kv.second);
        for (auto& kv : live_blocks) (void)hipFree(kv.first);
        if (table_mem) (void)hipFree(table_mem);
        for (auto& kv : lde_tabs) (void)hipFree(kv.second);
        if (upload_stream) { (void)hipStreamSynchronize(upload_stream); (void)hipStreamDestroy(upload_stream); (void)hipEventDestroy(upload_ev); }
        if (pinned) (void)hipHostFree(pinned);
        if (stage) (void)hipHostFree(stage);
        (void)hipStreamDestroy(stream);
    }
    DeviceCtx(const DeviceCtx&) = delete;

    void* alloc(size_t bytes) {
        std::lock_guard<std::mutex> lk(pool_mu);
        if (bytes == 0) bytes = 4;
        bytes = (bytes + 255) & ~(size_t)255;
        auto it = free_blocks.find(bytes);
        void* p;
        if (it != free_blocks.end()) { p = it->second; free_blocks.erase(it); }
        else {
            hipError_t e = hipMalloc(&p, bytes);
            if (e == hipErrorOutOfMemory) {
                (void)hipGetLastError();
                trim_locked();
                e = hipMalloc(&p, bytes);
            }
            if (e != hipSuccess) throw std::bad_alloc();
            bytes_allocated += bytes;
        }
        live_blocks[p] = bytes;
        live += bytes;
        if (live > peak_live) peak_live = live;
        if (poison_mode & 1) {
            if (!poison_fill_locked(p, bytes)) throw std::runtime_error("hip: the pool's poison fill failed");
            poison_stats[0]++; poison_stats[1] += bytes;
        }
        return p;
    }
    bool poison_fill_locked(void* p, size_t bytes) noexcept {
        int cur = -1;
        if (hipGetDevice(&cur) != hipSuccess) { (void)hipGetLastError(); cur = -1; }
        if (cur != device && hipSetDevice(device) != hipSuccess) { (void)hipGetLastError(); return false; }
        bool ok = hipDeviceSynchronize() == hipSuccess;
        ok = ok && hipMemsetD32((hipDeviceptr_t)p, (int)poison_word, bytes / 4) == hipSuccess;
        ok = ok && hipDeviceSynchronize() == hipSuccess;
        if (!ok) (void)hipGetLastError();
        if (cur >= 0 && cur != device) (void)hipSetDevice(cur);
        return ok;
    }
    size_t trim() {
        std::lock_guard<std::mutex> lk(pool_mu);
        return trim_locked();
    }
    size_t trim_locked() {
        (void)hipDeviceSynchronize();
        size_t freed = 0;
        for (auto& kv : free_blocks) { (void)hipFree(kv.second); freed += kv.first; }
        free_blocks.clear();
        bytes_allocated -= freed;
        return freed;
    }
    void fork() {
        if (in_section) throw std::runtime_error("nested fork");
        VG_HIP_CHECK(hipEventRecord(fork_ev, stream));
        for (int i = 0; i < NUM_AUX; i++) VG_HIP_CHECK(hipStreamWaitEvent(aux[i], fork_ev, 0));
        std::lock_guard<std::mutex> lk(pool_mu);
        in_section = true;
    }
    void join() {
        for (int i = 0; i < NUM_AUX; i++) {
            VG_HIP_CHECK(hipEventRecord(join_ev[i], aux[i]));
            VG_HIP_CHECK(hipStreamWaitEvent(stream, join_ev[i], 0));
        }
        std::vector<void*> d;
        {
            std::lock_guard<std::mutex> lk(pool_mu);
            in_section = false;
            d.swap(deferred);
        }
        for (void* p : d) release(p);
    }
    hipStream_t stream_for(size_t i, uint64_t rows) const {
        if (!in_section || rows >= (1ull << 16)) return stream;
        return aux[i % NUM_AUX];
    }
    void release(void* p) {
        if (!p) return;
        std::lock_guard<std::mutex> lk(pool_mu);
// ... 22 lines not shown
        static const bool on = [] { const char* e = getenv("VGPU_SPIN_WAIT"); return e && e[0] == '1'; }();
        return on;
    }
    std::recursive_mutex host_mu;
    void sync() {
        if (!spin_wait()) { VG_HIP_CHECK(hipStreamSynchronize(stream)); return; }
        hipEvent_t ev;
        {
            std::lock_guard<std::recursive_mutex> lk(host_mu);
            if (!sync_ev) VG_HIP_CHECK(hipEventCreateWithFlags(&sync_ev, hipEventDisableTiming));
            ev = sync_ev;
            VG_HIP_CHECK(hipEventRecord(ev, stream));
        }
        for (;;) {
            hipError_t e = hipEventQuery(ev);
            if (e == hipSuccess) return;
            if (e != hipErrorNotReady) throw std::runtime_error(std::string("hipEventQuery: ") + hipGetErrorString(e));
#if defined(__x86_64__)
            __builtin_ia32_pause();
#endif
        }
    }
    void check_launch(const char* what) {
        hipError_t e = hipGetLastError();
        if (e != hipSuccess) throw std::runtime_error(std::string(what) + ": " + hipGetErrorString(e));
    }
    void upload(void* dst, const void* src, size_t bytes) {
        VG_HIP_CHECK(hipMemcpyAsync(dst, src, bytes, hipMemcpyHostToDevice, stream));
        sync();
    }
    void upload_beside_proof(void* dst, const void* src, size_t bytes) {
        std::lock_guard<std::mutex> lk(upload_mu);
        if (!upload_stream) {
            VG_HIP_CHECK(hipStreamCreateWithFlags(&upload_stream, hipStreamNonBlocking));
            VG_HIP_CHECK(hipEventCreateWithFlags(&upload_ev, hipEventDisableTiming));
        }
        VG_HIP_CHECK(hipEventRecord(upload_ev, stream));
        VG_HIP_CHECK(hipStreamWaitEvent(upload_stream, upload_ev, 0));
        VG_HIP_CHECK(hipMemcpyAsync(dst, src, bytes, hipMemcpyHostToDevice, upload_stream));
        VG_HIP_CHECK(hipStreamSynchronize(upload_stream));
    }
    void download(void* dst, const void* src, size_t bytes) {
        VG_HIP_CHECK(hipMemcpyAsync(dst, src, bytes, hipMemcpyDeviceToHost, stream));
        sync();
    }
    void download_small(void* dst, const void* src, size_t bytes) {
        std::lock_guard<std::recursive_mutex> lk(host_mu);
        void* pin = pinned_buffer(bytes);
        VG_HIP_CHECK(hipMemcpyAsync(pin, src, bytes, hipMemcpyDeviceToHost, stream));
        sync();
        memcpy(dst, pin, bytes);
    }
    void upload_async(void* dst, const void* src, size_t bytes) {
        if (!bytes) return;
        if (bytes > STAGE_BYTES / 2) { upload(dst, src, bytes); return; }
        std::lock_guard<std::recursive_mutex> lk(host_mu);
        if (!stage) VG_HIP_CHECK(hipHostMalloc((void**)&stage, STAGE_BYTES));
        size_t pos = (stage_pos + 63) & ~(size_t)63;
        if (pos + bytes > STAGE_BYTES) {
            VG_HIP_CHECK(hipStreamSynchronize(stream));
            pos = 0;
        }
        memcpy(stage + pos, src, bytes);
        VG_HIP_CHECK(hipMemcpyAsync(dst, stage + pos, bytes, hipMemcpyHostToDevice, stream));
        stage_pos = pos + bytes;
    }
    std::map<std::tuple<int, int, uint32_t>, uint32_t*> lde_tabs;
    std::mutex lde_tabs_mu;
    vk::LdeTables lde_tables(int k, int log_blowup, Fp shift) {
        std::lock_guard<std::mutex> lk(lde_tabs_mu);
        const auto key = std::make_tuple(k, log_blowup, shift.v);
        auto it = lde_tabs.find(key);
        if (it == lde_tabs.end()) {
            std::vector<uint32_t> h(vk::lde_tables_words(k, log_blowup));
            vk::build_lde_tables(k, log_blowup, shift, h.data());
            uint32_t* d = nullptr;
            VG_HIP_CHECK(hipMalloc((void**)&d, h.size() * 4));
            VG_HIP_CHECK(hipMemcpy(d, h.data(), h.size() * 4, hipMemcpyHostToDevice));
            it = lde_tabs.emplace(key, d).first;
        }
        const size_t n_lo = (size_t)1 << vk::lde_k_lo(k);
        return vk::LdeTables{it->second, it->second + ((size_t)1 << log_blowup) * n_lo};
    }
    uint32_t* upload_words(const std::vector<uint32_t>& w) {
        uint32_t* d = alloc_words(w.size());
        upload_async(d, w.data(), w.size() * 4);
        return d;
    }

  private:
    void init_tables() {
        std::vector<uint32_t> t(vk::device_tables_words(), 0);
        vk::build_device_tables(tables, t.data());
        VG_HIP_CHECK(hipMalloc((void**)&table_mem, t.size() * 4));
        VG_HIP_CHECK(hipMemcpy(table_mem, t.data(), t.size() * 4, hipMemcpyHostToDevice));
        vk::bind_device_tables(tables, table_mem);
    }
};

struct Section {
    DeviceCtx* c;
    bool open;
    explicit Section(DeviceCtx* ctx) : c(ctx), open(true) { c->fork(); }
    void join() { if (open) { open = false; c->join(); } }
    ~Section() { if (open) { try { c->join(); } catch (...) { std::lock_guard<std::mutex> lk(c->pool_mu); c->in_section = false; } } }
    Section(const Section&) = delete;
    Section& operator=(const Section&) = delete;
};

struct DMat {
    DeviceCtx* ctx = nullptr;
    uint32_t* data = nullptr;
    uint64_t height = 0, width = 0;
    DMat() {}
    DMat(DeviceCtx* c, uint64_t h, uint64_t w) : ctx(c), data(c->alloc_words(h * w)), height(h), width(w) {}
    DMat(DMat&& o) noexcept { *this = std::move(o); }
    DMat& operator=(DMat&& o) noexcept {
        if (this != &o) { reset(); ctx = o.ctx; data = o.data; height = o.height; width = o.width; o.data = nullptr; o.ctx = nullptr; }
        return *this;
    }
    DMat(const DMat&) = delete;
    DMat& operator=(const DMat&) = delete;
    ~DMat() { reset(); }
    void reset() { if (data && ctx) ctx->release(data); data = nullptr; }
    vk::DMatView view() const { return vk::DMatView{data, height, width, height}; }
    bool empty() const { return data == nullptr; }
};

struct DBuf {
    DeviceCtx* ctx = nullptr;
    uint32_t* data = nullptr;
    size_t words = 0;
    DBuf() {}
    DBuf(DeviceCtx* c, size_t n) : ctx(c), data(c->alloc_words(n)), words(n) {}
    DBuf(DeviceCtx* c, const std::vector<uint32_t>& w) : ctx(c), data(c->upload_words(w)), words(w.size()) {}
    DBuf(DBuf&& o) noexcept { *this = std::move(o); }
    DBuf& operator=(DBuf&& o) noexcept {
        if (this != &o) { reset(); ctx = o.ctx; data = o.data; words = o.words; o.data = nullptr; o.ctx = nullptr; }
        return *this;
    }
    DBuf(const DBuf&) = delete;
    DBuf& operator=(const DBuf&) = delete;
    ~DBuf() { reset(); }
    void reset() { if (data && ctx) ctx->release(data); data = nullptr; }
};

inline void put_ext(std::vector<uint32_t>& w, const Ext5& e) { for (int k = 0; k < 5; k++) w.push_back(e.c[k].v); }
inline void put_ptr(std::vector<uint32_t>& w, const void* p) { uint64_t v = (uint64_t)p; w.push_back((uint32_t)v); w.push_back((uint32_t)(v >> 32)); }
inline void put_u64(std::vector<uint32_t>& w, uint64_t v) { w.push_back((uint32_t)v); w.push_back((uint32_t)(v >> 32)); }

}
```

valida_amd/csrc/kernels/device_common.hpp:

```cpp
#pragma once
#include <hip/hip_runtime.h>
#include "../field.hpp"

namespace vk {
using vg::Ext5;
using vg::Fp;

struct DMatView {
    uint32_t* data;
    uint64_t height, width, stride;
    __device__ __forceinline__ Fp get(uint64_t r, uint64_t c) const { return Fp::raw(data[c * stride + r]); }
    __device__ __forceinline__ void set(uint64_t r, uint64_t c, Fp v) const { data[c * stride + r] = v.v; }
    __device__ __forceinline__ uint32_t* col(uint64_t c) const { return data + c * stride; }
};

#ifndef VGPU_QUOT_SADDR
#define VGPU_QUOT_SADDR 1
#endif
__device__ __forceinline__ uint32_t load_at(const uint32_t* ubase, uint32_t byte_off) {
#if VGPU_QUOT_SADDR && defined(__HIP_DEVICE_COMPILE__)
    const __amdgpu_buffer_rsrc_t r = __builtin_amdgcn_make_buffer_rsrc(const_cast<uint32_t*>(ubase), 0, 0x7fffffff, 0x00020000);
    return (uint32_t)__builtin_amdgcn_raw_buffer_load_b32(r, (int)byte_off, 0, 0);
#else
    return *reinterpret_cast<const uint32_t*>(reinterpret_cast<const char*>(ubase) + byte_off);
#endif
}
__device__ __forceinline__ void store_at(uint32_t* ubase, uint32_t byte_off, uint32_t v) {
#if VGPU_QUOT_SADDR && defined(__HIP_DEVICE_COMPILE__)
    const __amdgpu_buffer_rsrc_t r = __builtin_amdgcn_make_buffer_rsrc(ubase, 0, 0x7fffffff, 0x00020000);
    __builtin_amdgcn_raw_buffer_store_b32((int)v, r, (int)byte_off, 0, 0);
#else
    *reinterpret_cast<uint32_t*>(reinterpret_cast<char*>(ubase) + byte_off) = v;
#endif
}

__device__ __forceinline__ uint32_t load_at(const uint32_t* ubase, uint32_t byte_off, uint32_t uniform_off) {
#if VGPU_QUOT_SADDR && defined(__HIP_DEVICE_COMPILE__)
    const __amdgpu_buffer_rsrc_t r = __builtin_amdgcn_make_buffer_rsrc(const_cast<uint32_t*>(ubase), 0, 0x7fffffff, 0x00020000);
    return (uint32_t)__builtin_amdgcn_raw_buffer_load_b32(r, (int)byte_off, (int)uniform_off, 0);
#else
    return *reinterpret_cast<const uint32_t*>(reinterpret_cast<const char*>(ubase) + byte_off + uniform_off);
#endif
}
__device__ __forceinline__ void store_at(uint32_t* ubase, uint32_t byte_off, uint32_t uniform_off, uint32_t v) {
#if VGPU_QUOT_SADDR && defined(__HIP_DEVICE_COMPILE__)
    const __amdgpu_buffer_rsrc_t r = __builtin_amdgcn_make_buffer_rsrc(ubase, 0, 0x7fffffff, 0x00020000);
    __builtin_amdgcn_raw_buffer_store_b32((int)v, r, (int)byte_off, (int)uniform_off, 0);
#else
    *reinterpret_cast<uint32_t*>(reinterpret_cast<char*>(ubase) + byte_off + uniform_off) = v;
#endif
}

struct DeviceTables {
    uint32_t roots[28];
    uint32_t inv_roots[28];
    const uint32_t* brt_lo;
    const uint32_t* brt_hi;
    const uint32_t* brt_top;
    const uint32_t* ibrt_lo;
    const uint32_t* ibrt_hi;
    const uint32_t* ibrt_top;
    const uint32_t* twc;
    const uint32_t* itwc;
};

constexpr int DEVICE_TABLES_TWC = 1 << 14;
inline size_t device_tables_words() { return 2048 * 4 + 64 + 2 * DEVICE_TABLES_TWC; }
inline void build_device_tables(DeviceTables& tb, uint32_t* h) {
    Fp roots[28], inv_roots[28];
    for (int i = 0; i <= 27; i++) { roots[i] = vg::two_adic_generator(i); inv_roots[i] = roots[i].inv(); }
    for (int i = 0; i < 28; i++) { tb.roots[i] = roots[i].v; tb.inv_roots[i] = inv_roots[i].v; }
    auto fill = [&](uint32_t* dst, int count, int first_bit, const Fp* r) {
        for (int j = 0; j < count; j++) {
            Fp p = Fp::one();
            for (int b = 0; (j >> b) != 0; b++) if ((j >> b) & 1) p *= r[first_bit + b + 1];
            dst[j] = p.v;
        }
    };
    for (size_t i = 0; i < device_tables_words(); i++) h[i] = 0;
    fill(h, 2048, 0, roots);
    fill(h + 2048, 2048, 11, roots);
    fill(h + 4096, 32, 22, roots);
    fill(h + 4096 + 32, 2048, 0, inv_roots);
    fill(h + 4096 + 32 + 2048, 2048, 11, inv_roots);
    fill(h + 4096 + 32 + 4096, 32, 22, inv_roots);
    uint32_t* twc = h + 4096 + 32 + 4096 + 32;
    for (int s = 1; s <= 14; s++) {
        Fp ws = roots[s], wsi = inv_roots[s], a = Fp::one(), b = Fp::one();
        int off = (1 << (s - 1)) - 1;
        for (int j = 0; j < (1 << (s - 1)); j++) { twc[off + j] = a.v; twc[DEVICE_TABLES_TWC + off + j] = b.v; a *= ws; b *= wsi; }
    }
}
inline void bind_device_tables(DeviceTables& tb, const uint32_t* base) {
    tb.brt_lo = base;
    tb.brt_hi = base + 2048;
    tb.brt_top = base + 4096;
    tb.ibrt_lo = base + 4096 + 32;
    tb.ibrt_hi = base + 4096 + 32 + 2048;
    tb.ibrt_top = base + 4096 + 32 + 4096;
    tb.twc = base + 4096 + 32 + 4096 + 32;
    tb.itwc = tb.twc + DEVICE_TABLES_TWC;
}

struct LdeTables { const uint32_t* fac; const uint32_t* sig; };
inline int lde_k_lo(int k) { return k < 12 ? k : (k >= 23 ? 14 : 12); }
inline size_t lde_tables_words(int k, int log_blowup) { const int k_lo = lde_k_lo(k); return ((size_t)1 << log_blowup) * (((size_t)1 << k_lo) + ((size_t)1 << (k - k_lo))); }
inline void build_lde_tables(int k, int log_blowup, Fp shift, uint32_t* h) {
    const int k_lo = lde_k_lo(k), k_hi = k - k_lo;
    const size_t n_lo = (size_t)1 << k_lo, n_hi = (size_t)1 << k_hi, b = (size_t)1 << log_blowup;
    const Fp w = vg::two_adic_generator((unsigned)(k + log_blowup)), ninv = Fp::from_canonical((uint32_t)(((uint64_t)1 << k) % vg::P)).inv();
    uint32_t* fac = h;
    uint32_t* sig = h + b * n_lo;
    Fp sigma = shift;
    for (size_t t = 0; t < b; t++) {
        const Fp g = sigma.exp_power_of_2((unsigned)k_hi);
        Fp pw = ninv;
        for (size_t j = 0; j < n_lo; j++) { fac[t * n_lo + (k_lo ? vg::reverse_bits_len((uint32_t)j, (unsigned)k_lo) : 0)] = pw.v; pw *= g; }
        Fp a = Fp::one();
        for (size_t c = 0; c < n_hi; c++) { sig[t * n_hi + c] = a.v; a *= sigma; }
        sigma *= w;
    }
}

__device__ __forceinline__ Fp domain_point(const DeviceTables& t, uint32_t j) {
    Fp r = Fp::raw(t.brt_lo[j & 2047]);
    if (j >> 11) r *= Fp::raw(t.brt_hi[(j >> 11) & 2047]);
    if (j >> 22) r *= Fp::raw(t.brt_top[j >> 22]);
    return r;
}
__device__ __forceinline__ Fp inv_domain_point(const DeviceTables& t, uint32_t j) {
    Fp r = Fp::raw(t.ibrt_lo[j & 2047]);
    if (j >> 11) r *= Fp::raw(t.ibrt_hi[(j >> 11) & 2047]);
    if (j >> 22) r *= Fp::raw(t.ibrt_top[j >> 22]);
    return r;
}

__device__ __forceinline__ Ext5 load_ext(const uint32_t* base, uint64_t stride, uint64_t r) {
    Ext5 e;
#pragma unroll
    for (int k = 0; k < 5; k++) e.c[k] = Fp::raw(base[k * stride + r]);
    return e;
}
__device__ __forceinline__ void store_ext(uint32_t* base, uint64_t stride, uint64_t r, const Ext5& e) {
#pragma unroll
    for (int k = 0; k < 5; k++) base[k * stride + r] = e.c[k].v;
}
__device__ __forceinline__ Ext5 ext_from_words(const uint32_t* w) {
    Ext5 e;
#pragma unroll
    for (int k = 0; k < 5; k++) e.c[k] = Fp::raw(w[k]);
    return e;
}

}

#define VG_HIP_CHECK(expr)                                                                                     \
    do {                                                                                                       \
        hipError_t _e = (expr);                                                                                \
        if (_e != hipSuccess) throw std::runtime_error(std::string(#expr) + ": " + hipGetErrorString(_e));     \
    } while (0)
```

valida_amd/csrc/kernels/launch.hpp:

```cpp
#pragma once
#include <vector>
#include "device_common.hpp"
#include "profiler.hpp"
#include "../air/symbolic.hpp"
#include "verify_args.hpp"

namespace vk {

struct QuotientArgs {
    DMatView main_lde, perm_lde, prep_lde;
    int log_n;
    const vair::Instr* prog;
    uint32_t n_instrs, n_regs, n_air_asserts;
    const uint32_t* iw;
    const uint32_t* consts;
    uint32_t K;
    uint32_t coset_shift, coset_shift_inv;
    int lqd;
    uint32_t zh_inv[8];
    uint32_t zh[8];
    uint32_t g_inv;
    DMatView out;
    int out_natural;
    static constexpr int INTERPRET = -2;
    int native_chip;
    const uint32_t* main_nx;
    const uint32_t* perm_nx;
    const uint32_t* prep_nx;
    uint32_t next_step_p1;
    QuotientArgs normalised() const {
        QuotientArgs b = *this;
        if (!b.main_nx) b.main_nx = b.main_lde.data;
        if (!b.perm_nx) b.perm_nx = b.perm_lde.data;
        if (!b.prep_nx) b.prep_nx = b.prep_lde.data;
        if (!b.next_step_p1) b.next_step_p1 = 1u + (1u << (b.lqd > 0 ? b.lqd : 1));
        return b;
    }
};

constexpr uint32_t INTERP_LDS_MIN_THREADS = 64;
constexpr uint32_t INTERP_LDS_BYTES_PAIR = 148 * 1024, INTERP_LDS_BYTES_GENERAL = 160 * 1024;
constexpr uint32_t INTERP_LDS_MAX_REGS_PAIR = INTERP_LDS_BYTES_PAIR / (4 * INTERP_LDS_MIN_THREADS);
constexpr uint32_t INTERP_LDS_MAX_REGS_GENERAL = INTERP_LDS_BYTES_GENERAL / (4 * INTERP_LDS_MIN_THREADS);
constexpr uint32_t interp_lds_max_regs(unsigned lqd) { return lqd == 1 ? INTERP_LDS_MAX_REGS_PAIR : INTERP_LDS_MAX_REGS_GENERAL; }
inline unsigned interp_lds_threads(uint32_t n_regs) {
    unsigned threads = 256;
    while (threads > INTERP_LDS_MIN_THREADS && (size_t)n_regs * threads * 4 > 64 * 1024) threads >>= 1;
    return threads;
}

void launch_ingest(hipStream_t st, const uint32_t* src_dev, DMatView dst, bool bitrev, uint32_t* varies = nullptr);
constexpr uint64_t INGEST_FLAGS_MAX_WIDTH = 512;
void launch_bitrev_rows(hipStream_t st, DMatView src, DMatView dst);
void launch_clock_probe(hipStream_t st, uint64_t* out3, uint32_t iters);
void launch_interleave_blocks(hipStream_t st, const uint32_t* src, uint32_t* dst, uint64_t rows, uint32_t log_wq, uint64_t n_cols);
void launch_export_rows(hipStream_t st, DMatView src, uint64_t row0, uint64_t nrows, uint32_t* dst_dev);
enum FieldProbeOp {
    FP_REDUCE_ONCE = 0, FP_SUB_MOD, FP_ADD, FP_SUB, FP_NEG, FP_MUL, FP_MONTY_REDUCE, FP_MONTY_REDUCE_WIDE, FP_FROM_CANONICAL, FP_CANONICAL, FP_INV,
    FP_EXT_MUL, FP_EXT_SQUARE, FP_EXT_SCALE, FP_EXT_INV, FP_BFLY_DIT_LB0, FP_BFLY_DIT, FP_BFLY_DIF_LB0, FP_BFLY_DIF, FP_MONTY_SIGNED, FP_SBOX, FP_SBOX_PLUS,
    FP_PERMUTE, FP_PERMUTE_PLAIN, FIELD_PROBE_OPS
};
bool field_probe_shape(uint32_t op, int* in_words, int* out_words);
void field_probe_check_twiddle_range(uint32_t op, const uint32_t* in_host, uint64_t n);
void launch_field_probe(hipStream_t st, uint32_t op, const uint32_t* in_dev, uint64_t n, const DeviceTables& tb, const uint32_t* pos_dev, bool sparse, uint32_t* out_dev);
void launch_intt(hipStream_t st, DMatView m, const DeviceTables& tb);
void launch_coset_ntt(hipStream_t st, DMatView coeffs, DMatView dst, uint64_t dst_row0, Fp shift, const DeviceTables& tb);
void launch_lde_natural(hipStream_t st, DMatView nat, DMatView lde, int log_blowup, const DeviceTables& tb, const LdeTables& lt, DMatView s1, DMatView s2,
                        const uint32_t* colmap = nullptr);
constexpr uint32_t COLMAP_LIVE_COUNT = 0, COLMAP_CONST_COUNT = 1, COLMAP_LIVE = 2;
inline size_t lde_colmap_words(uint64_t width) { return 2 + 2 * (size_t)width; }
void launch_lde_colmap(hipStream_t st, const uint32_t* varies, uint64_t width, uint32_t* colmap);
void launch_verify_chunk(hipStream_t st, const VerifyChunkArgs& a);
void launch_keccak_leaves(hipStream_t st, const uint32_t* const* cols_dev, int n_elems, uint64_t n_rows, uint32_t* digests);
void launch_keccak_leaves_strided(hipStream_t st, const uint32_t* base, uint64_t stride, int n_elems, uint64_t n_rows, uint32_t* digests);
void launch_keccak_compress(hipStream_t st, const uint32_t* prev, const uint32_t* const* cols_dev, int n_elems, uint64_t n_out, uint32_t* next);
void launch_keccak_bottom_q(hipStream_t st, const uint32_t* jobs_dev, uint32_t n_jobs, const uint32_t* indices_dev, uint32_t* dst);
void launch_poseidon_bottom_q(hipStream_t st, const uint32_t* pos_dev, bool sparse, const uint32_t* jobs_dev, uint32_t n_jobs, const uint32_t* indices_dev, uint32_t* dst);
constexpr int KECCAK_TOP_MAX_LEVELS = 11;
struct KeccakTopArgs {
    const uint32_t* prev;
    uint64_t first_len;
    int levels;
    uint32_t* out[KECCAK_TOP_MAX_LEVELS];
    const uint32_t* const* cols[KECCAK_TOP_MAX_LEVELS];
    int n_elems[KECCAK_TOP_MAX_LEVELS];
    const uint32_t* leaf_base = nullptr;
    uint64_t leaf_stride = 0;
    int leaf_elems = 0;
    uint64_t leaf_rows = 0;
    uint64_t block_len = 0;
    const uint32_t* ch_pos = nullptr;
    uint32_t* ch_state = nullptr;
    uint32_t* ch_beta5 = nullptr;
    uint32_t* ch_commit8 = nullptr;
};
void launch_keccak_top(hipStream_t st, const KeccakTopArgs& a);
constexpr uint64_t KECCAK_LEVELS_BLOCK_LEN = 64;
void launch_keccak_levels(hipStream_t st, const KeccakTopArgs& a);
bool keccak_levels_fused(uint64_t len);
bool keccak_levels_take_leaves(uint64_t n_rows);
bool keccak_top_takes_leaves(uint64_t n_rows);
void launch_poseidon_leaves(hipStream_t st, const uint32_t* pos_dev, bool sparse, const uint32_t* const* cols_dev, int n_elems, uint64_t n_rows, uint32_t* digests);
void launch_poseidon_leaves_strided(hipStream_t st, const uint32_t* pos_dev, bool sparse, const uint32_t* base, uint64_t stride, int n_elems, uint64_t n_rows, uint32_t* digests);
void launch_poseidon_compress(hipStream_t st, const uint32_t* pos_dev, bool sparse, const uint32_t* prev, const uint32_t* const* cols_dev, int n_elems, uint64_t n_out, uint32_t* next);
bool poseidon_levels_take(uint64_t parents);
int poseidon_levels_group(uint64_t parents);
void launch_poseidon_levels(hipStream_t st, const uint32_t* pos_dev, bool sparse, const KeccakTopArgs& a);
void launch_poseidon_top(hipStream_t st, const uint32_t* pos_dev, bool sparse, const KeccakTopArgs& a);
uint64_t perm_scratch_words(uint64_t n);
void launch_add_ext_const(hipStream_t st, uint32_t* data, uint64_t stride, uint64_t n, const uint32_t* off5_dev);
void launch_perm_trace(hipStream_t st, DMatView main, DMatView prep, const uint32_t* iw_dev, const uint32_t* chal_dev, uint32_t M, DMatView perm,
                       uint32_t* scratch, int native_chip = -2);
void launch_quotient(hipStream_t st, const QuotientArgs& a, const DeviceTables& tb);
void launch_check_constraints(hipStream_t st, const QuotientArgs& a, unsigned long long* first_bad_dev);
struct TgCpuOp { uint32_t pc, fp, opcode; int32_t operands[5]; uint32_t kind, has_imm, imm, mem_first; };
struct TgMemOp { uint32_t clk, addr, value, is_write; };
struct TgAluOp { uint32_t opcode, a, b, c; };
struct TgOutOp { uint32_t clk, byte; };
enum { TG_CPU_STORE32 = 0, TG_CPU_LOAD32, TG_CPU_JAL, TG_CPU_JALV, TG_CPU_BEQ, TG_CPU_BNE, TG_CPU_IMM32, TG_CPU_BUS, TG_CPU_BUS_LEFT_IMM, TG_CPU_STOP,
       TG_CPU_LOADFP, TG_CPU_LOAD_U8, TG_CPU_LOAD_S8, TG_CPU_STORE_U8, TG_CPU_READ_ADVICE };
void launch_tracegen_cpu(hipStream_t st, const TgCpuOp* ops, uint64_t n, const TgMemOp* mem, uint64_t n_mem, DMatView t);
size_t tracegen_mem_sort_scratch_bytes(uint64_t n);
hipError_t launch_tracegen_mem(hipStream_t st, const TgMemOp* mem, uint64_t n, const uint32_t* static_cells, uint64_t n_static, uint32_t* keys2, uint32_t* idx2,
                               void* sort_tmp, size_t sort_tmp_bytes, DMatView t);
void launch_tracegen_alu(hipStream_t st, int chip, const TgAluOp* ops, uint64_t n, DMatView t);
void launch_tracegen_idle(hipStream_t st, int mode, const uint32_t* static_cells, uint64_t n_static, DMatView t);
hipError_t launch_tracegen_range(hipStream_t st, const TgCpuOp* ops, uint64_t n, const TgMemOp* mem, uint64_t n_mem, uint32_t* counts, DMatView t);
void launch_tracegen_alu2(hipStream_t st, int chip, const TgAluOp* ops, uint64_t n, DMatView t);
void launch_tracegen_output(hipStream_t st, const TgOutOp* vals, const uint32_t* row0, uint64_t n, uint64_t n_rows, DMatView t);
hipError_t launch_tracegen_program(hipStream_t st, const TgCpuOp* ops, uint64_t n, uint64_t padded_n, uint32_t rom_len, uint32_t* counts, DMatView t);
size_t bus_audit_sort_scratch_words(uint64_t n);
size_t bus_audit_scan_scratch_words(uint64_t n);
void launch_ba_records(hipStream_t st, const uint32_t* desc, uint32_t chip, uint64_t height, uint32_t width, uint32_t M, uint32_t hash_bits, unsigned long long* keys, uint32_t* ids,
                       uint32_t* cnt, uint32_t* live_out);
void launch_ba_iota(hipStream_t st, uint32_t* ids, uint64_t n);
void launch_ba_rekey(hipStream_t st, const uint32_t* desc, uint32_t chunk, const uint32_t* ids, const uint32_t* cnt, unsigned long long* keys, uint64_t n);
int launch_ba_sort(hipStream_t st, unsigned long long* keys2, uint32_t* vals2, uint64_t n, uint32_t* counts, const int* shifts, int n_shifts, int half);
void launch_ba_groups(hipStream_t st, const uint32_t* desc, const unsigned long long* keys, const uint32_t* ids, uint64_t n, bool exact, uint32_t* gid, uint32_t* head_pos,
                      uint32_t* scan_tmp, uint32_t* counters);
void launch_ba_reduce(hipStream_t st, const uint32_t* desc, const uint32_t* ids, const uint32_t* cnt, const uint32_t* gid, const uint32_t* head_pos, uint64_t n, bool check,
                      unsigned long long* sums, uint32_t* nrec, uint32_t* counters);
void launch_ba_select(hipStream_t st, const uint32_t* desc, const uint32_t* ids, const uint32_t* head_pos, const unsigned long long* sums, uint64_t n_groups_max, bool collect,
                      uint32_t cap, unsigned long long* ukeys, uint32_t* uvals, uint32_t* counters);
void launch_ba_report(hipStream_t st, const uint32_t* desc, const uint32_t* ids, const uint32_t* cnt, const uint32_t* head_pos, const unsigned long long* sums, const uint32_t* nrec,
                      const uint32_t* uvals, uint32_t n_rep, uint32_t R, uint32_t* out);
constexpr uint32_t CA_MAX_CONSTRAINTS = 96, CA_MASK_WORDS = 3;
constexpr int CA_INTERPRET = -2;
struct CaListed { uint32_t w[CA_MASK_WORDS]; };
struct CaArgs {
    const uint32_t* main;
    uint64_t mstride;
    const uint32_t* prep;
    uint64_t pstride;
    uint64_t n;
    uint32_t width, prep_width;
    const vair::Instr* prog;
    uint32_t n_instrs, n_regs, K;
    int native_chip;
    uint32_t T, NB;
};
uint32_t ca_block_threads(const CaArgs& a);
void launch_ca_count(hipStream_t st, const CaArgs& a, unsigned long long* totals, uint32_t* table);
void launch_ca_scan(hipStream_t st, const CaArgs& a, const uint32_t* table, uint32_t* prefix, const CaListed& listed);
void launch_ca_list(hipStream_t st, const CaArgs& a, const uint32_t* table, const uint32_t* prefix, const CaListed& listed, uint32_t R, uint32_t* rows);
void launch_ca_values(hipStream_t st, const CaArgs& a, const unsigned long long* totals, const CaListed& listed, uint32_t R, const uint32_t* rows, uint32_t* values);
constexpr int MA_BUS_ONLY = -1;
constexpr uint32_t MA_COUNT = 0, MA_LIST = 1;
struct MaArgs {
    const uint32_t* main;
    uint64_t mstride;
    const uint32_t* prep;
    uint64_t pstride;
    uint64_t n;
    uint32_t width, prep_width;
    const vair::Instr* prog;
    uint32_t n_instrs, n_regs, K;
    const uint32_t* iw;
    const uint32_t* flags;
    uint32_t bus_walk;
    uint32_t CY;
    uint32_t D, delta[4];
    int native_chip;
    uint32_t T, NB;
    double evaluations;
};
uint32_t ma_block_threads(const MaArgs& a);
uint32_t ma_column_slices(const MaArgs& a, uint32_t NB);
void launch_ma_count(hipStream_t st, const MaArgs& a, unsigned long long* totals, uint32_t* table);
void launch_ma_scan(hipStream_t st, const MaArgs& a, const unsigned long long* totals, const uint32_t* table, uint32_t* prefix, uint32_t e_cut);
void launch_ma_list(hipStream_t st, const MaArgs& a, const uint32_t* table, const uint32_t* prefix, uint32_t e_cut, uint32_t R, uint32_t* rows);
constexpr uint32_t PA_SLICE_ENTRIES = 1024;
struct PaArgs {
    MaArgs m;
    const uint32_t* pairs;
    const uint32_t* pmasks;
    uint32_t P, PPS;
// ... 226 lines not shown
```

valida_amd/csrc/kernels/ntt.hip:

```cpp
#include "launch.hpp"
#include "butterfly.hpp"

namespace vk {

template <bool PAD> __device__ __forceinline__ int tile_addr(int i, int c, int LD) { return PAD ? i + (i >> 4) : i * LD + c; }

template <int R>
__device__ __forceinline__ void load_round_twiddles(Fp (&held)[(1 << R) - 1], const uint32_t* tw, int low, int lowbits) {
#pragma unroll
    for (int st = 0; st < R; st++) {
        const uint32_t* t = tw + ((1 << (lowbits + st)) - 1) + low;
#pragma unroll
        for (int k = 0; k < (1 << st); k++) held[(1 << st) - 1 + k] = Fp::raw(t[k << lowbits]);
    }
}

template <int R, bool DIT, bool PAD, int LB>
__device__ __forceinline__ void ntt_round(uint32_t* buf, const uint32_t* tw, int logn, int s_lo, int logT, int LD) {
    constexpr int G = 1 << R;
    const int n_items = (1 << (logn - R)) << logT;
    const int maskT = (1 << logT) - 1, lowbits = LB >= 0 ? LB : s_lo - 1, lowmask = (1 << lowbits) - 1;
    const bool linear = !PAD || lowbits >= 4 || lowbits + R <= 4;
    const int gs = PAD ? (lowbits >= 4 ? (1 << lowbits) + (1 << (lowbits - 4)) : (1 << lowbits)) : (LD << lowbits);
    for (int w = threadIdx.x; w < n_items; w += blockDim.x) {
// ... 340 lines not shown
template <int FK_HI, int FLOGT, bool MAPPED = false>
__global__ void __launch_bounds__(FK_HI ? 512 : 1024) k_lde_a(DMatView src, DMatView dst, int k, int k_lo, int logT_arg, DeviceTables tb, const uint32_t* colmap) {
    extern __shared__ uint32_t lds[];
    uint64_t src_col = blockIdx.y;
    if constexpr (MAPPED) {
        if (blockIdx.y >= colmap[COLMAP_LIVE_COUNT]) return;
        src_col = colmap[COLMAP_LIVE + blockIdx.y];
    }
    const int k_hi = FK_HI ? FK_HI : k - k_lo, logT = FK_HI ? FLOGT : logT_arg, n_hi = 1 << k_hi, T = 1 << logT, LD = T + 1;
    const uint64_t n_lo = 1ull << k_lo, r0 = (uint64_t)strided_tile_of_block(blockIdx.x, gridDim.x) * T;
    uint32_t* tw = lds + n_hi * LD;
    const uint32_t* in = src.col(src_col) + r0;
    uint32_t* out = dst.col(blockIdx.y) + r0;
    const int total = n_hi << logT;
    if constexpr (FK_HI != 0) strided_tile_load<FK_HI, FLOGT, false>(in, (uint32_t)n_lo, lds);
    else {
        int e = threadIdx.x;
        for (; e + 7 * (int)blockDim.x < total; e += 8 * blockDim.x) {
            uint32_t v[8];
#pragma unroll
            for (int u = 0; u < 8; u++) { const int eu = e + u * (int)blockDim.x; v[u] = in[(uint64_t)(eu >> logT) * n_lo + (eu & (T - 1))]; }
#pragma unroll
            for (int u = 0; u < 8; u++) { const int eu = e + u * (int)blockDim.x; lds[(eu >> logT) * LD + (eu & (T - 1))] = v[u]; }
        }
        for (; e < total; e += blockDim.x) { int c = e & (T - 1), h = e >> logT; lds[h * LD + c] = in[(uint64_t)h * n_lo + c]; }
    }
    stage_twiddles(tw, tb.itwc, k_hi);
    __syncthreads();
    if constexpr (FK_HI != 0) strided_transform<false, FK_HI, FLOGT>(lds, tw);
    else tile_transform<false, false>(lds, tw, k_hi, logT, LD);
    for (int p = threadIdx.x; p < n_hi; p += blockDim.x) {
        const uint32_t ca = __brev((uint32_t)p) >> (32 - k_hi);
        const Fp base = inv_root_pow(tb, k, ca);
        Fp cur = inv_root_pow(tb, k, (uint32_t)(((uint64_t)ca * r0) & ((1ull << k) - 1)));
        for (int c = 0; c < T; c++) { lds[p * LD + c] = (Fp::raw(lds[p * LD + c]) * cur).v; cur *= base; }
    }
    __syncthreads();
    if constexpr (FK_HI != 0) strided_tile_store<FK_HI, FLOGT>(out, (uint32_t)n_lo, lds);
    else
        for (int e = threadIdx.x; e < total; e += blockDim.x) { int c = e & (T - 1), h = e >> logT; out[(uint64_t)h * n_lo + c] = lds[h * LD + c]; }
}

template <int MAXT, bool MAPPED = false>
__global__ void __launch_bounds__(MAXT) k_lde_mid(DMatView src, DMatView dst, int k, int k_lo, int lb, DeviceTables tb, LdeTables lt, const uint32_t* colmap) {
    extern __shared__ uint32_t lds[];
    const int n_lo = 1 << k_lo, k_hi = k - k_lo, n_hi = 1 << k_hi, b = 1 << lb;
    uint32_t* A = lds;
    uint32_t* W = lds + padded_words(n_lo);
    const uint64_t N = 1ull << k, tiles_per_col = (uint64_t)n_hi, total = tiles_per_col * (MAPPED ? (uint64_t)colmap[COLMAP_LIVE_COUNT] : src.width);
    const uint32_t nmask = (uint32_t)(N - 1);
    auto tile_ptr = [&](uint64_t t) { const uint64_t cidx = t >> k_hi; return src.col(cidx) + (t & (tiles_per_col - 1)) * n_lo; };
    uint32_t pre[CONTIG_MAX_PER_THREAD];
    if (blockIdx.x < total) prefetch_tile(pre, tile_ptr(blockIdx.x), n_lo);
    for (uint64_t t = blockIdx.x; t < total; t += gridDim.x) {
        const uint64_t cidx = t >> k_hi, p = t & (tiles_per_col - 1);
        commit_tile(pre, A, n_lo);
        __syncthreads();
        if (t + gridDim.x < total) prefetch_tile(pre, tile_ptr(t + gridDim.x), n_lo);
        tile_transform<false, true>(A, tb.itwc, k_lo, 0, 0);
        const uint32_t ca = k_hi ? __brev((uint32_t)p) >> (32 - k_hi) : 0u;
        for (int tc = 0; tc < b; tc++) {
            const uint32_t* fac = lt.fac + (size_t)tc * n_lo;
            for (int i = threadIdx.x; i < n_lo; i += blockDim.x) W[tile_addr<true>(i, 0, 0)] = (Fp::raw(A[tile_addr<true>(i, 0, 0)]) * Fp::raw(fac[i])).v;
            __syncthreads();
            tile_transform<true, true>(W, tb.twc, k_lo, 0, 0);
            if (k_hi > 0) {
                uint32_t* out = dst.col(cidx) + (uint64_t)tc * N + p * n_lo;
                const Fp step = root_pow(tb, k, (ca * blockDim.x) & nmask);
                Fp cur = Fp::raw(lt.sig[(size_t)tc * n_hi + ca]) * root_pow(tb, k, (ca * threadIdx.x) & nmask);
                for (int q = threadIdx.x; q < n_lo; q += blockDim.x) { out[q] = (Fp::raw(W[tile_addr<true>(q, 0, 0)]) * cur).v; cur *= step; }
            } else {
                const uint32_t blk = lb ? __brev((uint32_t)tc) >> (32 - lb) : 0u;
                uint32_t* out = dst.col(cidx) + (uint64_t)blk * N;
                for (int j = threadIdx.x; j < n_lo; j += blockDim.x) {
                    const int q = k ? (int)(__brev((uint32_t)j) >> (32 - k)) : 0;
                    out[j] = W[tile_addr<true>(q, 0, 0)];
                }
            }
            __syncthreads();
        }
    }
}

template <bool MAPPED>
__global__ void __launch_bounds__(256) k_lde_mid12(DMatView src, DMatView dst, int k, int lb, DeviceTables tb, LdeTables lt, const uint32_t* colmap) {
    extern __shared__ uint32_t lds[];
    constexpr int K_LO = 12, N_LO = 1 << K_LO;
    const int k_hi = k - K_LO, n_hi = 1 << k_hi, b = 1 << lb, tid = threadIdx.x;
    const uint64_t N = 1ull << k, tiles_per_col = (uint64_t)n_hi, total = tiles_per_col * (MAPPED ? (uint64_t)colmap[COLMAP_LIVE_COUNT] : src.width);
    const uint32_t nmask = (uint32_t)(N - 1);
    auto tile_ptr = [&](uint64_t t) { const uint64_t cidx = t >> k_hi; return src.col(cidx) + (t & (tiles_per_col - 1)) * N_LO; };
    Fp tw_in[15], tw_out[15];
    load_round_twiddles<4>(tw_in, tb.itwc, tid, 8);
    load_round_twiddles<4>(tw_out, tb.twc, tid, 8);
    const Fp* const held_in = tw_in;
    const Fp* const held_out = tw_out;
    uint32_t pre[16];
    if (blockIdx.x < total) {
        const uint32_t* sp = tile_ptr(blockIdx.x);
#pragma unroll
        for (int g = 0; g < 16; g++) pre[g] = sp[tid + 256 * g];
    }
    for (uint64_t t = blockIdx.x; t < total; t += gridDim.x) {
        const uint64_t cidx = t >> k_hi, p = t & (tiles_per_col - 1);
        Fp x[16];
#pragma unroll
        for (int g = 0; g < 16; g++) x[g] = Fp::raw(pre[g]);
        if (t + gridDim.x < total) {
            const uint32_t* sp = tile_ptr(t + gridDim.x);
#pragma unroll
            for (int g = 0; g < 16; g++) pre[g] = sp[tid + 256 * g];
        }
        butterflies<4, false, false>(x, tb.itwc, tid, 8, held_in);
        {
            uint32_t* p0 = lds + tile_addr<true>(tid, 0, 0);
#pragma unroll
            for (int g = 0; g < 16; g++) p0[g * 272] = x[g].v;
        }
        __syncthreads();
        ntt_round<4, false, true, 4>(lds, tb.itwc, 12, 5, 0, 0);
        {
            const uint32_t* p0 = lds + 17 * tid;
#pragma unroll
            for (int g = 0; g < 16; g++) x[g] = Fp::raw(p0[g]);
        }
        butterflies<4, false, true>(x, tb.itwc, 0, 0);
        const uint32_t ca = __brev((uint32_t)p) >> (32 - k_hi);
        const Fp step = root_pow(tb, k, (ca * 256u) & nmask), tw0 = root_pow(tb, k, (ca * (uint32_t)tid) & nmask);
        for (int tc = 0; tc < b; tc++) {
            Fp y[16];
            {
                const uint32_t* fac = lt.fac + (size_t)tc * N_LO + 16 * tid;
#pragma unroll
                for (int g = 0; g < 16; g++) y[g] = x[g] * Fp::raw(fac[g]);
            }
            butterflies<4, true, true>(y, tb.twc, 0, 0);
            {
                uint32_t* p0 = lds + 17 * tid;
#pragma unroll
                for (int g = 0; g < 16; g++) p0[g] = y[g].v;
            }
            __syncthreads();
            ntt_round<4, true, true, 4>(lds, tb.twc, 12, 5, 0, 0);
            {
                const uint32_t* p0 = lds + tile_addr<true>(tid, 0, 0);
#pragma unroll
                for (int g = 0; g < 16; g++) y[g] = Fp::raw(p0[g * 272]);
            }
            butterflies<4, true, false>(y, tb.twc, tid, 8, held_out);
            uint32_t* out = dst.col(cidx) + (uint64_t)tc * N + p * N_LO + tid;
            Fp cur = Fp::raw(lt.sig[(size_t)tc * n_hi + ca]) * tw0;
#pragma unroll
            for (int g = 0; g < 16; g++) { out[256 * g] = (y[g] * cur).v; cur *= step; }
            __syncthreads();
        }
    }
}

template <bool MAPPED>
__global__ void __launch_bounds__(1024) k_lde_mid14(DMatView src, DMatView dst, int k, int lb, DeviceTables tb, LdeTables lt, const uint32_t* colmap) {
    extern __shared__ uint32_t lds[];
    constexpr int K_LO = 14, N_LO = 1 << K_LO, NT = 1024;
    uint32_t* const coef = lds + (N_LO + (N_LO >> 4));
    const int k_hi = k - K_LO, n_hi = 1 << k_hi, b = 1 << lb, tid = threadIdx.x;
    const uint64_t N = 1ull << k, tiles_per_col = (uint64_t)n_hi, total = tiles_per_col * (MAPPED ? (uint64_t)colmap[COLMAP_LIVE_COUNT] : src.width);
    const uint32_t nmask = (uint32_t)(N - 1);
    for (uint64_t t = blockIdx.x; t < total; t += gridDim.x) {
        const uint64_t cidx = t >> k_hi, p = t & (tiles_per_col - 1);
        const uint32_t* sp = src.col(cidx) + p * N_LO;
#pragma unroll
        for (int j = 0; j < 4; j++) {
            const int w = tid + NT * j;
            Fp x4[4];
#pragma unroll
            for (int g = 0; g < 4; g++) x4[g] = Fp::raw(sp[w + 4096 * g]);
            butterflies<2, false, false>(x4, tb.itwc, w, 12);
#pragma unroll
            for (int g = 0; g < 4; g++) lds[tile_addr<true>(w + 4096 * g, 0, 0)] = x4[g].v;
        }
        __syncthreads();
        ntt_round<4, false, true, 8>(lds, tb.itwc, 14, 9, 0, 0);
        ntt_round<4, false, true, 4>(lds, tb.itwc, 14, 5, 0, 0);
        {
            Fp x[16];
            const uint32_t* p0 = lds + 17 * tid;
#pragma unroll
            for (int g = 0; g < 16; g++) x[g] = Fp::raw(p0[g]);
            butterflies<4, false, true>(x, tb.itwc, 0, 0);
            uint32_t* c0 = coef + 17 * tid;
#pragma unroll
            for (int g = 0; g < 16; g++) c0[g] = x[g].v;
        }
        const uint32_t ca = k_hi ? __brev((uint32_t)p) >> (32 - k_hi) : 0u;
        const Fp step = root_pow(tb, k, (ca * 4096u) & nmask);
        for (int tc = 0; tc < b; tc++) {
            Fp y[16];
            {
                const uint32_t* fac = lt.fac + (size_t)tc * N_LO + 16 * tid;
                const uint32_t* c0 = coef + 17 * tid;
#pragma unroll
                for (int g = 0; g < 16; g++) y[g] = Fp::raw(c0[g]) * Fp::raw(fac[g]);
            }
            butterflies<4, true, true>(y, tb.twc, 0, 0);
            {
                uint32_t* p0 = lds + 17 * tid;
#pragma unroll
                for (int g = 0; g < 16; g++) p0[g] = y[g].v;
            }
            __syncthreads();
            ntt_round<4, true, true, 4>(lds, tb.twc, 14, 5, 0, 0);
            ntt_round<4, true, true, 8>(lds, tb.twc, 14, 9, 0, 0);
            uint32_t* out = dst.col(cidx) + (uint64_t)tc * N + p * N_LO;
            const Fp sg = Fp::raw(lt.sig[(size_t)tc * n_hi + ca]);
#pragma unroll 1
            for (int j = 0; j < 4; j++) {
                const int w = tid + NT * j;
                Fp y4[4];
#pragma unroll
                for (int g = 0; g < 4; g++) y4[g] = Fp::raw(lds[tile_addr<true>(w + 4096 * g, 0, 0)]);
                butterflies<2, true, false>(y4, tb.twc, w, 12);
                Fp cur = sg * root_pow(tb, k, (ca * (uint32_t)w) & nmask);
#pragma unroll
                for (int g = 0; g < 4; g++) { out[w + 4096 * g] = (y4[g] * cur).v; cur *= step; }
            }
            __syncthreads();
        }
    }
}

template <int FK_HI, int FLOGT, bool MAPPED = false>
__global__ void __launch_bounds__(FK_HI ? 512 : 1024) k_lde_c(DMatView src, DMatView dst, int k, int k_lo, int lb, int logT_arg, DeviceTables tb, const uint32_t* colmap) {
    extern __shared__ uint32_t lds[];
    uint64_t dst_col = blockIdx.y;
    if constexpr (MAPPED) {
        if (blockIdx.y >= colmap[COLMAP_LIVE_COUNT]) return;
        dst_col = colmap[COLMAP_LIVE + blockIdx.y];
// ... 77 lines not shown
    return p;
}

static void set_lds_limit() {
    static bool done = false;
    if (done) return;
    const int lim = 160 * 1024;
    (void)hipFuncSetAttribute((const void*)k_intt_strided, hipFuncAttributeMaxDynamicSharedMemorySize, lim);
    (void)hipFuncSetAttribute((const void*)k_ntt_strided, hipFuncAttributeMaxDynamicSharedMemorySize, lim);
    (void)hipFuncSetAttribute((const void*)k_intt_contig, hipFuncAttributeMaxDynamicSharedMemorySize, lim);
    (void)hipFuncSetAttribute((const void*)k_ntt_contig, hipFuncAttributeMaxDynamicSharedMemorySize, lim);
    (void)hipFuncSetAttribute((const void*)k_lde_a<0, 0>, hipFuncAttributeMaxDynamicSharedMemorySize, lim);
    (void)hipFuncSetAttribute((const void*)k_lde_a<8, 6>, hipFuncAttributeMaxDynamicSharedMemorySize, lim);
    (void)hipFuncSetAttribute((const void*)k_lde_a<10, 4>, hipFuncAttributeMaxDynamicSharedMemorySize, lim);
    (void)hipFuncSetAttribute((const void*)k_lde_mid<256>, hipFuncAttributeMaxDynamicSharedMemorySize, lim);
    (void)hipFuncSetAttribute((const void*)k_lde_mid<1024>, hipFuncAttributeMaxDynamicSharedMemorySize, lim);
    (void)hipFuncSetAttribute((const void*)k_lde_c<0, 0>, hipFuncAttributeMaxDynamicSharedMemorySize, lim);
    (void)hipFuncSetAttribute((const void*)k_lde_c<8, 6>, hipFuncAttributeMaxDynamicSharedMemorySize, lim);
    (void)hipFuncSetAttribute((const void*)k_lde_c<10, 4>, hipFuncAttributeMaxDynamicSharedMemorySize, lim);
    (void)hipFuncSetAttribute((const void*)k_lde_mid12<false>, hipFuncAttributeMaxDynamicSharedMemorySize, lim);
    (void)hipFuncSetAttribute((const void*)k_lde_mid14<false>, hipFuncAttributeMaxDynamicSharedMemorySize, lim);
    (void)hipFuncSetAttribute((const void*)k_lde_a<0, 0, true>, hipFuncAttributeMaxDynamicSharedMemorySize, lim);
    (void)hipFuncSetAttribute((const void*)k_lde_a<8, 6, true>, hipFuncAttributeMaxDynamicSharedMemorySize, lim);
    (void)hipFuncSetAttribute((const void*)k_lde_a<10, 4, true>, hipFuncAttributeMaxDynamicSharedMemorySize, lim);
    (void)hipFuncSetAttribute((const void*)k_lde_mid<256, true>, hipFuncAttributeMaxDynamicSharedMemorySize, lim);
    (void)hipFuncSetAttribute((const void*)k_lde_mid<1024, true>, hipFuncAttributeMaxDynamicSharedMemorySize, lim);
    (void)hipFuncSetAttribute((const void*)k_lde_c<0, 0, true>, hipFuncAttributeMaxDynamicSharedMemorySize, lim);
    (void)hipFuncSetAttribute((const void*)k_lde_c<8, 6, true>, hipFuncAttributeMaxDynamicSharedMemorySize, lim);
    (void)hipFuncSetAttribute((const void*)k_lde_c<10, 4, true>, hipFuncAttributeMaxDynamicSharedMemorySize, lim);
    (void)hipFuncSetAttribute((const void*)k_lde_mid12<true>, hipFuncAttributeMaxDynamicSharedMemorySize, lim);
    (void)hipFuncSetAttribute((const void*)k_lde_mid14<true>, hipFuncAttributeMaxDynamicSharedMemorySize, lim);
    done = true;
}

void launch_intt(hipStream_t st, DMatView m, const DeviceTables& tb) {
    set_lds_limit();
    int k = (int)vg::log2_strict_u64(m.height);
    NttPlan p = make_plan(k);
    uint32_t ninv = Fp::from_canonical((uint32_t)(m.height % vg::P)).inv().v;
    const uint64_t tiles_c = (m.height >> p.k_lo) * m.width;
    dim3 gc((unsigned)(tiles_c < 4096 ? tiles_c : 4096));
    const double pass_bytes = 8.0 * m.height * m.width;
    {
        ProfScope ps("k_intt_contig", st, pass_bytes);
        VK_LAUNCH(k_intt_contig, gc, dim3(p.threads_contig), p.lds_contig, st, m, k, p.k_lo, tb, ninv);
    }
    if (p.k_hi > 0) {
        dim3 gs((unsigned)((1u << p.k_lo) >> p.logT), (unsigned)m.width);
        ProfScope ps("k_intt_strided", st, pass_bytes);
        VK_LAUNCH(k_intt_strided, gs, dim3(p.threads_strided), p.lds_strided, st, m, k, p.k_lo, p.logT, tb, ninv);
    }
}

void launch_coset_ntt(hipStream_t st, DMatView coeffs, DMatView dst, uint64_t dst_row0, Fp shift, const DeviceTables& tb) {
    set_lds_limit();
    int k = (int)vg::log2_strict_u64(coeffs.height);
    NttPlan p = make_plan(k);
    const uint64_t tiles_c = (coeffs.height >> p.k_lo) * coeffs.width;
    dim3 gc((unsigned)(tiles_c < 4096 ? tiles_c : 4096));
    const double pass_bytes = 8.0 * coeffs.height * coeffs.width;
    if (p.k_hi > 0) {
        dim3 gs((unsigned)((1u << p.k_lo) >> p.logT), (unsigned)coeffs.width);
        {
            CosetPowers cp;
            const unsigned hstep = p.threads_strided >> p.logT;
            Fp a = Fp::one(), s64 = shift.pow(64), sn = shift.pow(1ull << p.k_lo);
            for (int i = 0; i < 64; i++) { cp.lo[i] = a.v; a *= shift; }
            a = Fp::one();
            for (int i = 0; i < 256; i++) { cp.hi[i] = a.v; a *= s64; }
            a = Fp::one();
            cp.step = 0;
            for (unsigned i = 0; i < 128; i++) { cp.hp[i] = a.v; a *= sn; if (i + 1 == hstep) cp.step = a.v; }
            ProfScope ps("k_ntt_strided", st, pass_bytes);
            VK_LAUNCH(k_ntt_strided, gs, dim3(p.threads_strided), p.lds_strided, st, coeffs, dst, dst_row0, k, p.k_lo, p.logT, tb, cp);
        }
        ProfScope ps("k_ntt_contig", st, pass_bytes);
        VK_LAUNCH(k_ntt_contig, gc, dim3(p.threads_contig), p.lds_contig, st, coeffs, dst, dst_row0, k, p.k_lo, tb, shift.v, 0);
    } else {
        ProfScope ps("k_ntt_contig", st, pass_bytes);
        VK_LAUNCH(k_ntt_contig, gc, dim3(p.threads_contig), p.lds_contig, st, coeffs, dst, dst_row0, k, p.k_lo, tb, shift.v, 1);
    }
}

void launch_lde_colmap(hipStream_t st, const uint32_t* varies, uint64_t width, uint32_t* colmap) {
    if (width == 0 || width > 16384) throw std::invalid_argument("lde colmap: width out of range");
    ProfScope ps("k_lde_colmap", st, 4.0 * 3 * width);
    VK_LAUNCH(k_lde_colmap, dim3(1), dim3(256), (size_t)width * 4, st, varies, (uint32_t)width, colmap);
}

void launch_lde_natural(hipStream_t st, DMatView nat, DMatView lde, int log_blowup, const DeviceTables& tb, const LdeTables& lt, DMatView s1, DMatView s2,
                        const uint32_t* colmap) {
    set_lds_limit();
    const int k = (int)vg::log2_strict_u64(nat.height);
    NttPlan p = make_plan(k);
    const uint64_t tiles = ((uint64_t)1 << p.k_hi) * nat.width;
    dim3 gm((unsigned)(tiles < 4096 ? tiles : 4096));
    const size_t lds_mid = 2 * (size_t)padded_words(1 << p.k_lo) * 4;
    const double nw = 4.0 * nat.height * nat.width, b = (double)(1u << log_blowup);
    if (p.k_hi == 0) {
        ProfScope ps("k_lde_mid", st, nw * (1.0 + b));
        VK_LAUNCH(k_lde_mid<256>, gm, dim3(p.threads_contig), lds_mid, st, nat, lde, k, p.k_lo, log_blowup, tb, lt, nullptr);
        return;
    }
    if (colmap) {
        const uint64_t quads = lde.height >> 2, per_block = 256 * 16;
        ProfScope ps("k_lde_fill_const", st, 0.0);
        VK_LAUNCH(k_lde_fill_const, dim3((unsigned)((quads + per_block - 1) / per_block), (unsigned)nat.width), dim3(256), 0, st, nat, lde, colmap);
    }
    dim3 gs((unsigned)((1u << p.k_lo) >> p.logT), (unsigned)nat.width);
    {
        ProfScope ps("k_lde_a", st, 2.0 * nw);
        const int shape = VGPU_STRIDED_IO && VGPU_STRIDED_FIXED && p.threads_strided == 512 ? (p.k_hi == 8 && p.logT == 6 ? 8 : (p.k_hi == 10 && p.logT == 4 ? 10 : 0)) : 0;
#define VG_LDE_A(A, B, THREADS)                                                                                                       \
    do {                                                                                                                              \
        if (colmap) VK_LAUNCH((k_lde_a<A, B, true>), gs, dim3(THREADS), p.lds_strided, st, nat, s1, k, p.k_lo, p.logT, tb, colmap);      \
        else VK_LAUNCH((k_lde_a<A, B, false>), gs, dim3(THREADS), p.lds_strided, st, nat, s1, k, p.k_lo, p.logT, tb, colmap);           \
    } while (0)
        if (shape == 8) VG_LDE_A(8, 6, 512);
        else if (shape == 10) VG_LDE_A(10, 4, 512);
        else VG_LDE_A(0, 0, p.threads_strided);
#undef VG_LDE_A
    }
    if (p.k_lo == 12) {
        if (gm.x > 4096u) gm.x = 4096u;
        ProfScope ps("k_lde_mid12", st, nw * (1.0 + b));
        if (colmap) VK_LAUNCH(k_lde_mid12<true>, gm, dim3(256), (size_t)padded_words(4096) * 4, st, s1, s2, k, log_blowup, tb, lt, colmap);
        else VK_LAUNCH(k_lde_mid12<false>, gm, dim3(256), (size_t)padded_words(4096) * 4, st, s1, s2, k, log_blowup, tb, lt, colmap);
    } else if (p.k_lo == 14) {
        ProfScope ps("k_lde_mid14", st, nw * (1.0 + b));
        const size_t lds14 = 2 * (size_t)padded_words(16384) * 4;
        if (colmap) VK_LAUNCH(k_lde_mid14<true>, gm, dim3(1024), lds14, st, s1, s2, k, log_blowup, tb, lt, colmap);
        else VK_LAUNCH(k_lde_mid14<false>, gm, dim3(1024), lds14, st, s1, s2, k, log_blowup, tb, lt, colmap);
    } else {
        ProfScope ps("k_lde_mid", st, nw * (1.0 + b));
        if (p.threads_contig <= 256) {
            if (colmap) VK_LAUNCH((k_lde_mid<256, true>), gm, dim3(p.threads_contig), lds_mid, st, s1, s2, k, p.k_lo, log_blowup, tb, lt, colmap);
            else VK_LAUNCH(k_lde_mid<256>, gm, dim3(p.threads_contig), lds_mid, st, s1, s2, k, p.k_lo, log_blowup, tb, lt, colmap);
        } else {
            if (colmap) VK_LAUNCH((k_lde_mid<1024, true>), gm, dim3(p.threads_contig), lds_mid, st, s1, s2, k, p.k_lo, log_blowup, tb, lt, colmap);
            else VK_LAUNCH(k_lde_mid<1024>, gm, dim3(p.threads_contig), lds_mid, st, s1, s2, k, p.k_lo, log_blowup, tb, lt, colmap);
        }
    }
    dim3 gc((unsigned)((1u << p.k_lo) >> p.logT), (unsigned)nat.width, 1u << log_blowup);
    ProfScope ps("k_lde_c", st, 2.0 * nw * b);
    const int shape_c = VGPU_STRIDED_IO && VGPU_STRIDED_FIXED && p.threads_strided == 512 ? (p.k_hi == 8 && p.logT == 6 ? 8 : (p.k_hi == 10 && p.logT == 4 ? 10 : 0)) : 0;
#define VG_LDE_C(A, B, THREADS)                                                                                                              \
    do {                                                                                                                                     \
        if (colmap) VK_LAUNCH((k_lde_c<A, B, true>), gc, dim3(THREADS), p.lds_strided, st, s2, lde, k, p.k_lo, log_blowup, p.logT, tb, colmap); \
        else VK_LAUNCH((k_lde_c<A, B, false>), gc, dim3(THREADS), p.lds_strided, st, s2, lde, k, p.k_lo, log_blowup, p.logT, tb, colmap);     \
    } while (0)
    if (shape_c == 8) VG_LDE_C(8, 6, 512);
    else if (shape_c == 10) VG_LDE_C(10, 4, 512);
    else VG_LDE_C(0, 0, p.threads_strided);
#undef VG_LDE_C
}

}
```

valida_amd/csrc/kernels/quotient.hip:

```cpp
#include <cstdlib>
#include <stdexcept>
#include "launch.hpp"
#include "interactions.hpp"
#include "../chips/basic_machine.hpp"

namespace vk {

struct PointCtx {
    uint64_t row, next_row;
    Fp is_first, is_last, is_trans;
};

typedef uint32_t v32u __attribute__((ext_vector_type(32)));

#define VG_INTERP_BODY(GET, SET)                                                                                                        \
    switch (in.op) {                                                                                                                    \
        case vair::OP_CONST: SET(in.dst, (uint32_t)in.a | ((uint32_t)in.b << 16)); break;                                               \
        case vair::OP_LOAD_MAIN: SET(in.dst, in.flag ? a.main_nx[(uint64_t)in.a * a.main_lde.stride + p.next_row] : a.main_lde.data[(uint64_t)in.a * a.main_lde.stride + p.row]); break; \
        case vair::OP_LOAD_PREP: SET(in.dst, in.flag ? a.prep_nx[(uint64_t)in.a * a.prep_lde.stride + p.next_row] : a.prep_lde.data[(uint64_t)in.a * a.prep_lde.stride + p.row]); break; \
        case vair::OP_SEL_FIRST: SET(in.dst, p.is_first.v); break;                                                                      \
        case vair::OP_SEL_LAST: SET(in.dst, p.is_last.v); break;                                                                        \
        case vair::OP_SEL_TRANS: SET(in.dst, p.is_trans.v); break;                                                                      \
        case vair::OP_ADD: { uint32_t x = GET(in.a), y = GET(in.b); SET(in.dst, (Fp::raw(x) + Fp::raw(y)).v); } break;                  \
        case vair::OP_SUB: { uint32_t x = GET(in.a), y = GET(in.b); SET(in.dst, (Fp::raw(x) - Fp::raw(y)).v); } break;                  \
// ... 222 lines not shown
    vchips::visit_interactions(CHIP, v);
    const Ext5 cumulative_sum = ext_from_words(v.betas + 5 * maxf);
    const Ext5 phi_local = load_ext_at(a.perm_lde.data + (uint64_t)(5 * v.m) * a.perm_lde.stride, a.perm_lde.stride, v.roff);
    const Ext5 phi_next = load_ext_at(a.perm_nx + (uint64_t)(5 * v.m) * a.perm_lde.stride, a.perm_lde.stride, v.noff);
    Ext5 acc = v.acc;
    acc += ext_from_words(v.apow + 5 * v.m) * (((phi_next - phi_local) - v.rhs) * p.is_trans);
    acc += ext_from_words(v.apow + 5 * (v.m + 1)) * ((phi_local - v.phi_0) * p.is_first);
    acc += ext_from_words(v.apow + 5 * (v.m + 2)) * ((phi_local - cumulative_sum) * p.is_last);
    return acc;
}

template <int RFKIND, int CHIP = -1>
__global__ void __launch_bounds__(256) k_quotient(QuotientArgs a, DeviceTables tb) {
    extern __shared__ uint32_t regs[];
    const uint64_t n = 1ull << a.log_n;
    uint64_t m = (uint64_t)blockIdx.x * blockDim.x + threadIdx.x;
#ifndef VGPU_QUOT_TILE
#define VGPU_QUOT_TILE 1
#endif
    const bool tiled = VGPU_QUOT_TILE && a.log_n >= 9 && blockDim.x == 256;
    const bool nat_tile = tiled && a.out_natural;
    if (nat_tile) {
        m = ((uint64_t)(threadIdx.x >> 4) << (a.log_n - 4)) | ((uint64_t)blockIdx.x << 4) | (threadIdx.x & 15u);
    } else if (tiled) {
        const uint32_t B = blockIdx.x, top = B >> (a.log_n - 9), mid = B & ((1u << (a.log_n - 9)) - 1u);
        m = ((uint64_t)top << (a.log_n - 1)) | ((uint64_t)(threadIdx.x >> 5) << (a.log_n - 4)) | ((uint64_t)mid << 5) | (threadIdx.x & 31u);
    }
    if (m >= n) return;
    const int kq = a.log_n + 1;
    const uint32_t Qmask = (uint32_t)(2 * n - 1);
    const uint32_t j0 = (uint32_t)(2 * m), j1 = j0 + 1;
    const uint32_t i0 = vg::reverse_bits_len((uint32_t)m, (unsigned)a.log_n);
    const uint32_t i1 = i0 + (uint32_t)n;
    const Fp s = Fp::raw(a.coset_shift), g_inv = Fp::raw(a.g_inv);
    const Fp x0 = s * domain_point(tb, j0), x1 = -x0;
    Fp d00 = x0 - Fp::one(), d01 = x0 - g_inv, d10 = x1 - Fp::one(), d11 = x1 - g_inv;
    Fp p01 = d00 * d01, p23 = d10 * d11;
    Fp inv_all = (p01 * p23).inv();
    Fp ip01 = inv_all * p23, ip23 = inv_all * p01;
    Fp id00 = ip01 * d01, id01 = ip01 * d00, id10 = ip23 * d11, id11 = ip23 * d10;
    const uint32_t par0 = i0 & 1u, par1 = i1 & 1u;
    PointCtx p0, p1;
    p0.row = j0; p0.next_row = vg::reverse_bits_len((i0 + a.next_step_p1 - 1u) & Qmask, (unsigned)kq);
    p1.row = j1; p1.next_row = vg::reverse_bits_len((i1 + a.next_step_p1 - 1u) & Qmask, (unsigned)kq);
    p0.is_trans = d01; p0.is_first = Fp::raw(a.zh[par0]) * id00; p0.is_last = Fp::raw(a.zh[par0]) * id01;
    p1.is_trans = d11; p1.is_first = Fp::raw(a.zh[par1]) * id10; p1.is_last = Fp::raw(a.zh[par1]) * id11;
    Ext5 q0 = Ext5::zero(), q1 = Ext5::zero();
#pragma unroll 1
    for (int pt = 0; pt < 2; pt++) {
        PointCtx p;
        p.row = pt ? p1.row : p0.row; p.next_row = pt ? p1.next_row : p0.next_row;
        p.is_first = pt ? p1.is_first : p0.is_first; p.is_last = pt ? p1.is_last : p0.is_last; p.is_trans = pt ? p1.is_trans : p0.is_trans;
        Ext5 q;
        if (RFKIND == 3) q = run_native<CHIP>(a, p);
        else if (RFKIND == 0) q = run_program_lds(a, p, regs);
        else q = run_program_vgpr<RFKIND>(a, p);
        q = (q + perm_constraints(a, p)) * Fp::raw(a.zh_inv[pt ? par1 : par0]);
        if (pt) q1 = q; else q0 = q;
    }
    Fp x0_inv = Fp::raw(a.coset_shift_inv) * inv_domain_point(tb, j0);
    Ext5 sum = q0 + q1, diff = (q0 - q1) * x0_inv;
    if (nat_tile) {
        __shared__ uint32_t tr[10 * 256];
        const uint32_t A = threadIdx.x >> 4, r = threadIdx.x & 15u, slot = (r << 4) | (__brev(A) >> 28);
#pragma unroll
        for (int c = 0; c < 5; c++) { tr[c * 256 + slot] = sum.c[c].halve().v; tr[(5 + c) * 256 + slot] = diff.c[c].halve().v; }
        __syncthreads();
        const uint64_t row = ((uint64_t)(__brev(A) >> 28) << (a.log_n - 4)) | ((uint64_t)(a.log_n > 8 ? __brev((uint32_t)blockIdx.x) >> (32 - (a.log_n - 8)) : 0u) << 4) | r;
#pragma unroll
        for (int c = 0; c < 10; c++) a.out.data[(uint64_t)c * a.out.stride + row] = tr[c * 256 + threadIdx.x];
        return;
    }
    const uint64_t pos = a.out_natural ? (uint64_t)i0 : m;
#pragma unroll
    for (int c = 0; c < 5; c++) {
        a.out.data[(uint64_t)c * a.out.stride + pos] = sum.c[c].halve().v;
        a.out.data[(uint64_t)(5 + c) * a.out.stride + pos] = diff.c[c].halve().v;
    }
}

#ifndef VGPU_QUOT_PT_WAVES
#define VGPU_QUOT_PT_WAVES 6
#endif
template <int CHIP>
__global__ void __launch_bounds__(512)
#if VGPU_QUOT_PT_WAVES > 0
__attribute__((amdgpu_waves_per_eu(VGPU_QUOT_PT_WAVES)))
#endif
k_quotient_pt(QuotientArgs a, DeviceTables tb) {
    const uint64_t n = 1ull << a.log_n;
    const uint32_t T = threadIdx.x >> 1, pt = threadIdx.x & 1u;
    uint64_t m = (uint64_t)blockIdx.x * 256 + T;
    const bool tiled = a.log_n >= 9;
    const bool nat_tile = tiled && a.out_natural;
    if (nat_tile) {
        m = ((uint64_t)(T >> 4) << (a.log_n - 4)) | ((uint64_t)blockIdx.x << 4) | (T & 15u);
    } else if (tiled) {
        const uint32_t B = blockIdx.x, top = B >> (a.log_n - 9), mid = B & ((1u << (a.log_n - 9)) - 1u);
        m = ((uint64_t)top << (a.log_n - 1)) | ((uint64_t)(T >> 5) << (a.log_n - 4)) | ((uint64_t)mid << 5) | (T & 31u);
    }
    if (m >= n) return;
    const int kq = a.log_n + 1;
    const uint32_t Qmask = (uint32_t)(2 * n - 1);
    const uint32_t j = (uint32_t)(2 * m) + pt;
    const uint32_t i0 = vg::reverse_bits_len((uint32_t)m, (unsigned)a.log_n);
    const uint32_t i = i0 + pt * (uint32_t)n;
    const Fp s = Fp::raw(a.coset_shift), g_inv = Fp::raw(a.g_inv);
    const Fp x0 = s * domain_point(tb, (uint32_t)(2 * m));
    const Fp x = pt ? -x0 : x0;
    const Fp d0 = x - Fp::one(), d1 = x - g_inv;
    const Fp inv = (d0 * d1).inv();
    const uint32_t par = i & 1u;
    PointCtx p;
    p.row = j;
    p.next_row = vg::reverse_bits_len((i + a.next_step_p1 - 1u) & Qmask, (unsigned)kq);
    p.is_trans = d1;
    p.is_first = Fp::raw(a.zh[par]) * (inv * d1);
    p.is_last = Fp::raw(a.zh[par]) * (inv * d0);
#ifndef VGPU_QUOT_PERM_NATIVE
#define VGPU_QUOT_PERM_NATIVE 1
#endif
    Ext5 q = run_native<CHIP>(a, p);
    q = (q + (VGPU_QUOT_PERM_NATIVE ? perm_constraints_native<CHIP>(a, p) : perm_constraints(a, p))) * Fp::raw(a.zh_inv[par]);
    Ext5 o;
#pragma unroll
    for (int c = 0; c < 5; c++) o.c[c] = Fp::raw((uint32_t)__builtin_amdgcn_update_dpp(0, (int)q.c[c].v, 0xB1, 0xF, 0xF, true));
    const Fp x0_inv = Fp::raw(a.coset_shift_inv) * inv_domain_point(tb, (uint32_t)(2 * m));
    Fp outv[5];
#pragma unroll
    for (int c = 0; c < 5; c++) outv[c] = (pt ? (o.c[c] - q.c[c]) * x0_inv : q.c[c] + o.c[c]).halve();
    const uint32_t col0 = 5u * pt;
    if (nat_tile) {
        __shared__ uint32_t tr[10 * 256];
        const uint32_t A = T >> 4, r = T & 15u, slot = (r << 4) | (__brev(A) >> 28);
#pragma unroll
        for (int c = 0; c < 5; c++) tr[(col0 + c) * 256 + slot] = outv[c].v;
        __syncthreads();
        const uint32_t t = threadIdx.x & 255u, half = threadIdx.x >> 8, A2 = t >> 4, r2 = t & 15u;
        const uint64_t row = ((uint64_t)(__brev(A2) >> 28) << (a.log_n - 4)) | ((uint64_t)(a.log_n > 8 ? __brev((uint32_t)blockIdx.x) >> (32 - (a.log_n - 8)) : 0u) << 4) | r2;
#pragma unroll
        for (int c = 0; c < 5; c++) a.out.data[(uint64_t)(5 * half + c) * a.out.stride + row] = tr[(5 * half + c) * 256 + t];
        return;
    }
    const uint64_t pos = a.out_natural ? (uint64_t)i0 : m;
#pragma unroll
    for (int c = 0; c < 5; c++) a.out.data[(uint64_t)(col0 + c) * a.out.stride + pos] = outv[c].v;
}

template <int RFKIND>
__global__ void __launch_bounds__(256) k_quotient_general(QuotientArgs a, DeviceTables tb) {
    extern __shared__ uint32_t regs[];
    constexpr int QMAX = 8;
    const int lqd = a.lqd, Q = 1 << lqd;
    const uint64_t n = 1ull << a.log_n;
    const uint64_t m = (uint64_t)blockIdx.x * blockDim.x + threadIdx.x;
    if (m >= n) return;
    const int kq = a.log_n + lqd;
    const uint32_t Qmask = (uint32_t)(((uint64_t)Q << a.log_n) - 1);
    const uint32_t i0 = vg::reverse_bits_len((uint32_t)m, (unsigned)a.log_n);
    const Fp s = Fp::raw(a.coset_shift), g_inv = Fp::raw(a.g_inv);
    Ext5 v[QMAX];
#pragma unroll 1
    for (int r = 0; r < Q; r++) {
        const uint32_t j = (uint32_t)(Q * m) + (uint32_t)r;
        const uint32_t i = i0 + (uint32_t)(n * vg::reverse_bits_len((uint32_t)r, (unsigned)lqd));
        const Fp x = s * domain_point(tb, j);
        const Fp zh = Fp::raw(a.zh[i & (uint32_t)(Q - 1)]);
        PointCtx p;
        p.row = j;
        p.next_row = vg::reverse_bits_len((i + (uint32_t)Q) & Qmask, (unsigned)kq);
        p.is_trans = x - g_inv;
        p.is_first = zh * (x - Fp::one()).inv();
        p.is_last = zh * p.is_trans.inv();
        Ext5 q = RFKIND == 0 ? run_program_lds(a, p, regs) : run_program_vgpr<(RFKIND == 0 ? 1 : RFKIND)>(a, p);
        v[r] = (q + perm_constraints(a, p)) * Fp::raw(a.zh_inv[i & (uint32_t)(Q - 1)]);
    }
    Fp ybase = s * domain_point(tb, (uint32_t)(Q * m));
    for (int level = 0; level < lqd; level++) {
        const int G = Q >> level;
        const int lg = lqd - level;
        Ext5 t[QMAX];
        for (int base = 0; base < Q; base += G)
            for (int u = 0; u < G / 2; u++) {
                const Fp w = vg::two_adic_generator((unsigned)lg).pow(vg::reverse_bits_len((uint32_t)(2 * u), (unsigned)lg));
                const Fp yinv = (ybase * w).inv();
                const Ext5 av = v[base + 2 * u], bv = v[base + 2 * u + 1];
                Ext5 e = av + bv, o = (av - bv) * yinv;
                for (int c = 0; c < 5; c++) { e.c[c] = e.c[c].halve(); o.c[c] = o.c[c].halve(); }
                t[base + u] = e;
                t[base + G / 2 + u] = o;
            }
        for (int r = 0; r < Q; r++) v[r] = t[r];
        ybase = ybase * ybase;
    }
    for (int ch = 0; ch < Q; ch++)
        for (int c = 0; c < 5; c++) a.out.data[(uint64_t)(5 * ch + c) * a.out.stride + m] = v[ch].c[c].v;
}

struct DebugFolder {
    using Expr = Fp;
    const uint32_t* __restrict__ main_p;
    const uint32_t* __restrict__ main_n;
    uint64_t mstride;
    const uint32_t* __restrict__ prep_p;
    const uint32_t* __restrict__ prep_n;
    uint64_t pstride;
    Fp first, last, trans;
    uint32_t k, bad;
    __device__ __forceinline__ Fp constant(uint32_t c) const { return Fp::from_canonical(c); }
    __device__ __forceinline__ Fp main(int col, bool next) const { return Fp::raw((next ? main_n : main_p)[(uint64_t)col * mstride]); }
    __device__ __forceinline__ Fp preprocessed(int col, bool next) const { return Fp::raw((next ? prep_n : prep_p)[(uint64_t)col * pstride]); }
    __device__ __forceinline__ Fp is_first_row() const { return first; }
    __device__ __forceinline__ Fp is_last_row() const { return last; }
    __device__ __forceinline__ Fp is_transition() const { return trans; }
    __device__ __forceinline__ void assert_zero(const Fp& e) { if (!e.is_zero() && bad == 0xffffffffu) bad = k; k++; }
};

template <int CHIP>
__global__ void __launch_bounds__(256) k_check_constraints(QuotientArgs a, unsigned long long* __restrict__ first_bad) {
    extern __shared__ uint32_t regs[];
    const uint64_t n = 1ull << a.log_n;
    const uint64_t r = (uint64_t)blockIdx.x * blockDim.x + threadIdx.x;
    if (r >= n) return;
    PointCtx p;
    p.row = r; p.next_row = (r + 1) & (n - 1);
    p.is_first = r == 0 ? Fp::one() : Fp::zero();
    p.is_last = r == n - 1 ? Fp::one() : Fp::zero();
    p.is_trans = r == n - 1 ? Fp::zero() : Fp::one();
    uint32_t code = 0xffffffffu;
    if (CHIP == QuotientArgs::INTERPRET) {
        if (!run_program_lds(a, p, regs).is_zero()) code = 0xFFFDu;
    } else if (CHIP >= 0) {
        DebugFolder f;
        f.main_p = a.main_lde.data + p.row; f.main_n = a.main_nx + p.next_row; f.mstride = a.main_lde.stride;
        f.prep_p = a.prep_lde.data + p.row; f.prep_n = a.prep_nx + p.next_row; f.pstride = a.prep_lde.stride;
        f.first = p.is_first; f.last = p.is_last; f.trans = p.is_trans;
        f.k = 0; f.bad = 0xffffffffu;
        vchips::eval_chip(CHIP, f);
        code = f.bad;
    }
    if (code == 0xffffffffu && !perm_constraints(a, p).is_zero()) code = 0xFFFEu;
    if (code != 0xffffffffu) atomicMin(first_bad, (unsigned long long)((r << 16) | code));
}

void launch_check_constraints(hipStream_t st, const QuotientArgs& a_in, unsigned long long* first_bad_dev) {
    const QuotientArgs a = a_in.normalised();
    const uint64_t n = 1ull << a.log_n;
    const dim3 grid((unsigned)((n + 255) / 256)), block(256);
    ProfScope ps("k_check_constraints", st, 4.0 * n * (a.main_lde.width + a.perm_lde.width + a.prep_lde.width));
    switch (a.native_chip) {
#define VG_CHECK(C) case vchips::C: VK_LAUNCH((k_check_constraints<vchips::C>), grid, block, 0, st, a, first_bad_dev); break;
        VG_CHECK(CHIP_CPU) VG_CHECK(CHIP_ADD) VG_CHECK(CHIP_SUB) VG_CHECK(CHIP_MUL) VG_CHECK(CHIP_SHIFT) VG_CHECK(CHIP_LT)
        VG_CHECK(CHIP_COM) VG_CHECK(CHIP_BITWISE) VG_CHECK(CHIP_OUTPUT) VG_CHECK(CHIP_STATIC_DATA)
#undef VG_CHECK
        case QuotientArgs::INTERPRET: {
            static bool attr = false;
            if (!attr) { (void)hipFuncSetAttribute((const void*)k_check_constraints<QuotientArgs::INTERPRET>, hipFuncAttributeMaxDynamicSharedMemorySize, INTERP_LDS_BYTES_GENERAL); attr = true; }
            if (a.n_regs > INTERP_LDS_MAX_REGS_GENERAL) throw std::invalid_argument("check_constraints: the constraint program needs more registers than a workgroup's LDS holds");
            const unsigned threads = interp_lds_threads(a.n_regs);
            VK_LAUNCH((k_check_constraints<QuotientArgs::INTERPRET>), dim3((unsigned)((n + threads - 1) / threads)), dim3(threads), (size_t)a.n_regs * threads * 4, st, a,
                               first_bad_dev);
            break;
        }
        default: VK_LAUNCH((k_check_constraints<-1>), grid, block, 0, st, a, first_bad_dev); break;
    }
}

void launch_quotient(hipStream_t st, const QuotientArgs& a_in, const DeviceTables& tb) {
    const QuotientArgs a = a_in.normalised();
    static bool attr = false;
    if (!attr) {
        (void)hipFuncSetAttribute((const void*)k_quotient<0>, hipFuncAttributeMaxDynamicSharedMemorySize, INTERP_LDS_BYTES_PAIR);
        (void)hipFuncSetAttribute((const void*)k_quotient_general<0>, hipFuncAttributeMaxDynamicSharedMemorySize, INTERP_LDS_BYTES_GENERAL);
        attr = true;
    }
    if (a.native_chip == QuotientArgs::INTERPRET && a.n_regs > interp_lds_max_regs((unsigned)a.lqd))
        throw std::invalid_argument("quotient: the constraint program needs more registers than a workgroup's LDS holds");
    uint64_t n = 1ull << a.log_n;
    if (a.lqd != 1) {
        if (a.lqd < 1 || a.lqd > 3 || a.native_chip != QuotientArgs::INTERPRET) throw std::runtime_error("quotient: log_quotient_degree must be 1..3 (and above 1 only for interpreted AIRs)");
        ProfScope ps("k_quotient", st, 4.0 * n * ((double)(1 << a.lqd) * (a.main_lde.width + a.perm_lde.width + a.prep_lde.width) + 5.0 * (1 << a.lqd)));
        unsigned threads = 256;
        if (a.n_regs <= 64) {
            dim3 grid((unsigned)((n + threads - 1) / threads));
            if (a.n_regs <= 32) VK_LAUNCH(k_quotient_general<1>, grid, dim3(threads), 0, st, a, tb);
            else VK_LAUNCH(k_quotient_general<2>, grid, dim3(threads), 0, st, a, tb);
            return;
        }
        threads = interp_lds_threads(a.n_regs);
        VK_LAUNCH(k_quotient_general<0>, dim3((unsigned)((n + threads - 1) / threads)), dim3(threads), (size_t)a.n_regs * threads * 4, st, a, tb);
        return;
    }
    static const char* names[16] = {"k_quotient.cpu", "k_quotient.program", "k_quotient.mem", "k_quotient.add", "k_quotient.sub", "k_quotient.mul", "k_quotient.div",
                                    "k_quotient.shift", "k_quotient.lt", "k_quotient.com", "k_quotient.bitwise", "k_quotient.output", "k_quotient.range",
                                    "k_quotient.static_data", "k_quotient", "k_quotient"};
    static const bool per_point = [] { const char* e = getenv("VGPU_QUOT_PER_POINT"); return !(e && e[0] == '0'); }();
    const char* pname = getenv("VGPU_PROF_QUOTIENT_BY_CHIP") && a.native_chip >= 0 && a.native_chip < 14 ? names[a.native_chip]
                        : (per_point && a.native_chip != QuotientArgs::INTERPRET ? "k_quotient_pt" : "k_quotient");
    ProfScope ps(pname, st, 4.0 * n * (2.0 * (a.main_lde.width + a.perm_lde.width + a.prep_lde.width) + 10.0));
    if (a.native_chip != QuotientArgs::INTERPRET && per_point) {
        const dim3 grid((unsigned)((n + 255) / 256)), block(512);
        switch (a.native_chip) {
#define VG_NATIVE_PT(C) case vchips::C: VK_LAUNCH((k_quotient_pt<vchips::C>), grid, block, 0, st, a, tb); break;
            VG_NATIVE_PT(CHIP_CPU) VG_NATIVE_PT(CHIP_ADD) VG_NATIVE_PT(CHIP_SUB) VG_NATIVE_PT(CHIP_MUL) VG_NATIVE_PT(CHIP_SHIFT) VG_NATIVE_PT(CHIP_LT)
            VG_NATIVE_PT(CHIP_COM) VG_NATIVE_PT(CHIP_BITWISE) VG_NATIVE_PT(CHIP_OUTPUT) VG_NATIVE_PT(CHIP_STATIC_DATA)
            VG_NATIVE_PT(CHIP_PROGRAM) VG_NATIVE_PT(CHIP_MEM) VG_NATIVE_PT(CHIP_DIV) VG_NATIVE_PT(CHIP_RANGE)
#undef VG_NATIVE_PT
            default: throw std::logic_error("quotient: a native chip id outside the BasicMachine");
        }
        return;
    }
    if (a.native_chip != QuotientArgs::INTERPRET) {
        const dim3 grid((unsigned)((n + 255) / 256)), block(256);
        switch (a.native_chip) {
#define VG_NATIVE(C) case vchips::C: VK_LAUNCH((k_quotient<3, vchips::C>), grid, block, 0, st, a, tb); break;
            VG_NATIVE(CHIP_CPU) VG_NATIVE(CHIP_ADD) VG_NATIVE(CHIP_SUB) VG_NATIVE(CHIP_MUL) VG_NATIVE(CHIP_SHIFT) VG_NATIVE(CHIP_LT)
            VG_NATIVE(CHIP_COM) VG_NATIVE(CHIP_BITWISE) VG_NATIVE(CHIP_OUTPUT) VG_NATIVE(CHIP_STATIC_DATA)
#undef VG_NATIVE
            default: VK_LAUNCH((k_quotient<3, -1>), grid, block, 0, st, a, tb); break;
        }
        return;
    }
    if (a.n_regs <= 64) {
        const unsigned threads = 256;
        dim3 grid((unsigned)((n + threads - 1) / threads));
        if (a.n_regs <= 32) VK_LAUNCH(k_quotient<1>, grid, dim3(threads), 0, st, a, tb);
        else VK_LAUNCH(k_quotient<2>, grid, dim3(threads), 0, st, a, tb);
        return;
    }
    const unsigned threads = interp_lds_threads(a.n_regs);
    size_t lds = (size_t)a.n_regs * threads * 4;
    VK_LAUNCH(k_quotient<0>, dim3((unsigned)((n + threads - 1) / threads)), dim3(threads), lds, st, a, tb);
}

}
```

Measured before the change: 70.23 proofs/s.

## Cache quotient selector inverses and LDE middle-pass twiddles in device tables

Adds per-device cached tables that are built once and reused across proofs. One holds the vanishing-selector inverses for the quotient kernel, replacing a per-point field inversion with a load. The other holds precomputed coset twiddle factors for the 2^12 middle LDE pass, replacing a chain of multiplications and root_pow lookups with loads. Both are on by default, can be turned off through an env mask, and are freed on trim. The trade-off is extra device memory and memory bandwidth in place of arithmetic, plus a new prove mutex taken in commit_batches, which could serialise concurrent proofs in flight.

```diff
diff --git a/bindings/rust/src/lib.rs b/bindings/rust/src/lib.rs
--- a/bindings/rust/src/lib.rs
+++ b/bindings/rust/src/lib.rs
@@ -1,6 +1,9 @@
 #![allow(non_camel_case_types, dead_code)]
 use core::ffi::{c_char, c_int, c_void};
 
+pub const VGPU_DOMAIN_TABLE_QSEL: u32 = 1;
+pub const VGPU_DOMAIN_TABLE_TW4: u32 = 2;
+pub const VGPU_DOMAIN_TABLES_ALL: u32 = 3;
 pub const VGPU_CBOR_CANONICAL_FIELDS: u32 = 1;
 pub const VGPU_CBOR_PLAIN_DIGESTS: u32 = 2;
 pub const VGPU_CBOR_IN_BARE_IS_MONTGOMERY: u32 = 1;
@@ -346,6 +349,7 @@
     pub fn vgpu_prover_memory_reset_peak(p: *mut VgpuProver);
     pub fn vgpu_prover_set_dense_lane(p: *mut VgpuProver, on: u32, min_nodes: u64);
     pub fn vgpu_prover_set_const_columns(p: *mut VgpuProver, on: u32);
+    pub fn vgpu_prover_set_domain_tables(p: *mut VgpuProver, mask: u32);
     pub fn vgpu_prover_lane_stats(p: *const VgpuProver, entered: *mut u64, waited: *mut u64);
     pub fn vgpu_prover_set_profiling(p: *mut VgpuProver, on: u32);
     pub fn vgpu_prover_set_prep_cache(p: *mut VgpuProver, on: u32);
diff --git a/include/vgpu.h b/include/vgpu.h
--- a/include/vgpu.h
+++ b/include/vgpu.h
@@ -93,6 +93,10 @@
 void vgpu_prover_memory_reset_peak(vgpu_prover_t* p);
 void vgpu_prover_set_dense_lane(vgpu_prover_t* p, uint32_t on, uint64_t min_nodes);
 void vgpu_prover_set_const_columns(vgpu_prover_t* p, uint32_t on);
+#define VGPU_DOMAIN_TABLE_QSEL 1u
+#define VGPU_DOMAIN_TABLE_TW4 2u
+#define VGPU_DOMAIN_TABLES_ALL 3u
+void vgpu_prover_set_domain_tables(vgpu_prover_t* p, uint32_t mask);
 void vgpu_prover_lane_stats(const vgpu_prover_t* p, uint64_t* entered, uint64_t* waited);
 
 void vgpu_prover_set_profiling(vgpu_prover_t* p, uint32_t on);
diff --git a/valida_amd/__init__.py b/valida_amd/__init__.py
--- a/valida_amd/__init__.py
+++ b/valida_amd/__init__.py
@@ -15,6 +15,7 @@
 
 
 HASH_KECCAK256, HASH_POSEIDON16 = 0, 1
+DOMAIN_TABLE_QSEL, DOMAIN_TABLE_TW4, DOMAIN_TABLES_ALL = 1, 2, 3
 
 
 class VgpuError(RuntimeError):
@@ -2081,8 +2082,14 @@
             self.set_dense_lane(not lane_off, int(lane_min or 0))
         if os.environ.get("VGPU_CONST_COLS", "1") == "0":
             self.set_const_columns(False)
+        tables = os.environ.get("VGPU_DOMAIN_TABLES", "").strip()
+        if tables:
+            self.set_domain_tables(int(tables, 0))
         if poison is not None:
             self.set_pool_poison(poison)
+
+    def set_domain_tables(self, mask):
+        lib().vgpu_prover_set_domain_tables(self._h, ctypes.c_uint32(int(mask)))
 
     def set_const_columns(self, on):
         lib().vgpu_prover_set_const_columns(self._h, ctypes.c_uint32(1 if on else 0))
diff --git a/valida_amd/csrc/capi.cpp b/valida_amd/csrc/capi.cpp
--- a/valida_amd/csrc/capi.cpp
+++ b/valida_amd/csrc/capi.cpp
@@ -343,6 +343,12 @@
     std::lock_guard<std::mutex> lk(c.prove_mu);
     c.const_cols_on = on != 0;
 }
+void vgpu_prover_set_domain_tables(vgpu_prover_t* p, uint32_t mask) {
+    if (!p) return;
+    DeviceCtx& c = p->p->ctx();
+    std::lock_guard<std::mutex> lk(c.prove_mu);
+    c.domain_tables = mask & vhost::DOMAIN_TABLES_ALL;
+}
 void vgpu_prover_set_dense_lane(vgpu_prover_t* p, uint32_t on, uint64_t min_nodes) {
     if (!p) return;
     DeviceCtx& c = p->p->ctx();
@@ -366,7 +372,10 @@
     if (!p) return 0;
     DeviceCtx& c = p->p->ctx();
     (void)hipSetDevice(c.device);
-    return (uint64_t)c.trim();
+    uint64_t freed = (uint64_t)c.trim();
+    std::unique_lock<std::mutex> lk(c.prove_mu, std::try_to_lock);
+    if (lk.owns_lock()) { (void)hipDeviceSynchronize(); freed += (uint64_t)c.drop_domain_tables(); }
+    return freed;
 }
 void vgpu_prover_set_profiling(vgpu_prover_t* p, uint32_t on) {
     auto& c = p->p->ctx();
@@ -553,6 +562,8 @@
         if (!p || !mats || !n_mats || !root || !out) throw std::invalid_argument("null argument");
         DeviceCtx& c = p->p->ctx();
         c.activate();
+        std::lock_guard<std::mutex> one_at_a_time(c.prove_mu);
+        DeviceCtx::DomainTablesOpen tables_open(&c);
         size_t words = 0;
         for (uint32_t i = 0; i < n_mats; i++) {
             if (!mats[i] || mats[i]->owner != p->p) throw std::invalid_argument("null trace or trace of another prover");
diff --git a/valida_amd/csrc/host/pcs.hpp b/valida_amd/csrc/host/pcs.hpp
--- a/valida_amd/csrc/host/pcs.hpp
+++ b/valida_amd/csrc/host/pcs.hpp
@@ -202,7 +202,8 @@
     static const bool fused = [] { const char* e = getenv("VGPU_LDE_FUSED"); return !(e && e[0] == '0'); }();
     if (!in.rows_bitrev && fused) {
         DMat lde(c, n * b, in.mat->width);
-        const vk::LdeTables lt = c->lde_tables((int)k, (int)log_blowup, lde_shift);
+        vk::LdeTables lt = c->lde_tables((int)k, (int)log_blowup, lde_shift);
+        lt.tw4 = c->lde_tw4((int)k, (int)log_blowup, lde_shift, lt, st);
         DMat s1, s2;
         if (k > 12) { s1 = DMat(c, n, in.mat->width); s2 = DMat(c, n * b, in.mat->width); }
         DBuf colmap;
diff --git a/valida_amd/csrc/host/prover.cpp b/valida_amd/csrc/host/prover.cpp
--- a/valida_amd/csrc/host/prover.cpp
+++ b/valida_amd/csrc/host/prover.cpp
@@ -299,6 +299,7 @@
         ~Running() { n.fetch_sub(1); }
     } running(c.proofs_running);
     struct LaneOpen { explicit LaneOpen(const DeviceCtx* x) { DeviceCtx::lane_thread_ctx() = x; } ~LaneOpen() { DeviceCtx::lane_thread_ctx() = nullptr; } } lane_open(&c);
+    DeviceCtx::DomainTablesOpen tables_open(&c);
     const size_t NC = machine_.airs.size();
     if (main.size() != NC) throw std::invalid_argument("prove: need one main trace per chip");
     const Fp s = Fp::from_canonical(vg::GENERATOR);
@@ -532,10 +533,16 @@
             put_ext(pool, cumulative_sums[i]);
         }
         DBuf pool_dev(&c, pool);
+        std::vector<const uint32_t*> qsel(NC, nullptr);
+        if (c.domain_tables & vhost::DOMAIN_TABLE_QSEL)
+            for (size_t i = 0; i < NC; i++)
+                if (!fri_.interpret_air && machine_.airs[i].native_chip != vk::QuotientArgs::INTERPRET && machine_.airs[i].log_quotient_degree == 1)
+                    qsel[i] = c.quotient_selectors((int)log_deg[i], s);
         Section quotient_section(&c);
         for (size_t i = 0; i < NC; i++) {
             auto& air = machine_.airs[i];
             vk::QuotientArgs a{};
+            a.qsel = qsel[i];
             fill_quotient_args(a, (int)i, main_pd->ldes[i].view(), perm_pd->ldes[i].view(),
                                prep_slot[i] >= 0 ? prep_pd->ldes[prep_slot[i]].view() : vk::DMatView{nullptr, 0, 0, 0}, log_deg[i], pool_dev.data + off[i]);
             a.K = Ks[i];
diff --git a/valida_amd/csrc/host/runtime.hpp b/valida_amd/csrc/host/runtime.hpp
--- a/valida_amd/csrc/host/runtime.hpp
+++ b/valida_amd/csrc/host/runtime.hpp
@@ -35,6 +35,10 @@
     if (!l) l = new HipDenseLane;
     return *l;
 }
+
+constexpr uint32_t DOMAIN_TABLE_QSEL = 1u;
+constexpr uint32_t DOMAIN_TABLE_TW4 = 2u;
+constexpr uint32_t DOMAIN_TABLES_ALL = DOMAIN_TABLE_QSEL | DOMAIN_TABLE_TW4, DOMAIN_TABLES_DEFAULT = DOMAIN_TABLES_ALL;
 
 struct DeviceCtx {
     int device = 0;
@@ -67,6 +71,7 @@
     static const DeviceCtx*& lane_thread_ctx() { static thread_local const DeviceCtx* c = nullptr; return c; }
     bool lane_open_here() const { return lane_on && lane && lane_thread_ctx() == this; }
     bool const_cols_on = true;
+    uint32_t domain_tables = DOMAIN_TABLES_DEFAULT;
     std::vector<void*> deferred;
     std::mutex pool_mu;
     uint32_t poison_mode = 0, poison_word = 0;
@@ -110,6 +115,7 @@
         for (auto& kv : live_blocks) (void)hipFree(kv.first);
         if (table_mem) (void)hipFree(table_mem);
         for (auto& kv : lde_tabs) (void)hipFree(kv.second);
+        drop_domain_tables();
         if (upload_stream) { (void)hipStreamSynchronize(upload_stream); (void)hipStreamDestroy(upload_stream); (void)hipEventDestroy(upload_ev); }
         if (pinned) (void)hipHostFree(pinned);
         if (stage) (void)hipHostFree(stage);
@@ -298,6 +304,46 @@
         const size_t n_lo = (size_t)1 << vk::lde_k_lo(k);
         return vk::LdeTables{it->second, it->second + ((size_t)1 << log_blowup) * n_lo};
     }
+    std::map<std::pair<int, uint32_t>, uint32_t*> qsel_tabs;
+    const uint32_t* quotient_selectors(int log_n, Fp shift) {
+        const auto key = std::make_pair(log_n, shift.v);
+        auto it = qsel_tabs.find(key);
+        if (it == qsel_tabs.end()) {
+            uint32_t* d = nullptr;
+            if (hipMalloc((void**)&d, (size_t)8 << log_n) != hipSuccess) { (void)hipGetLastError(); return nullptr; }
+            it = qsel_tabs.emplace(key, d).first;
+            vk::launch_quotient_selectors(stream, d, log_n, shift.v, vg::two_adic_generator((unsigned)log_n).inv().v, tables);
+        }
+        return it->second;
+    }
+    static const DeviceCtx*& tables_thread_ctx() { static thread_local const DeviceCtx* c = nullptr; return c; }
+    struct DomainTablesOpen {
+        explicit DomainTablesOpen(const DeviceCtx* x) { tables_thread_ctx() = x; }
+        ~DomainTablesOpen() { tables_thread_ctx() = nullptr; }
+        DomainTablesOpen(const DomainTablesOpen&) = delete;
+    };
+    std::map<std::tuple<int, int, uint32_t>, uint32_t*> tw4_tabs;
+    const uint32_t* lde_tw4(int k, int log_blowup, Fp shift, const vk::LdeTables& lt, hipStream_t st) {
+        if (!(domain_tables & DOMAIN_TABLE_TW4) || tables_thread_ctx() != this || k <= 12 || vk::lde_k_lo(k) != 12) return nullptr;
+        const auto key = std::make_tuple(k, log_blowup, shift.v);
+        auto it = tw4_tabs.find(key);
+        if (it == tw4_tabs.end()) {
+            uint32_t* d = nullptr;
+            if (hipMalloc((void**)&d, (size_t)4 << (k + log_blowup)) != hipSuccess) { (void)hipGetLastError(); return nullptr; }
+            it = tw4_tabs.emplace(key, d).first;
+            vk::launch_lde_tw4(st, d, k, log_blowup, tables, lt);
+            VG_HIP_CHECK(hipStreamSynchronize(st));
+        }
+        return it->second;
+    }
+    size_t drop_domain_tables() {
+        size_t freed = 0;
+        for (auto& kv : qsel_tabs) { (void)hipFree(kv.second); freed += (size_t)8 << kv.first.first; }
+        for (auto& kv : tw4_tabs) { (void)hipFree(kv.second); freed += (size_t)4 << (std::get<0>(kv.first) + std::get<1>(kv.first)); }
+        qsel_tabs.clear();
+        tw4_tabs.clear();
+        return freed;
+    }
     uint32_t* upload_words(const std::vector<uint32_t>& w) {
         uint32_t* d = alloc_words(w.size());
         upload_async(d, w.data(), w.size() * 4);
diff --git a/valida_amd/csrc/kernels/device_common.hpp b/valida_amd/csrc/kernels/device_common.hpp
--- a/valida_amd/csrc/kernels/device_common.hpp
+++ b/valida_amd/csrc/kernels/device_common.hpp
@@ -102,7 +102,7 @@
     tb.itwc = tb.twc + DEVICE_TABLES_TWC;
 }
 
-struct LdeTables { const uint32_t* fac; const uint32_t* sig; };
+struct LdeTables { const uint32_t* fac; const uint32_t* sig; const uint32_t* tw4 = nullptr; };
 inline int lde_k_lo(int k) { return k < 12 ? k : (k >= 23 ? 14 : 12); }
 inline size_t lde_tables_words(int k, int log_blowup) { const int k_lo = lde_k_lo(k); return ((size_t)1 << log_blowup) * (((size_t)1 << k_lo) + ((size_t)1 << (k - k_lo))); }
 inline void build_lde_tables(int k, int log_blowup, Fp shift, uint32_t* h) {
diff --git a/valida_amd/csrc/kernels/launch.hpp b/valida_amd/csrc/kernels/launch.hpp
--- a/valida_amd/csrc/kernels/launch.hpp
+++ b/valida_amd/csrc/kernels/launch.hpp
@@ -28,6 +28,7 @@
     const uint32_t* perm_nx;
     const uint32_t* prep_nx;
     uint32_t next_step_p1;
+    const uint32_t* qsel;
     QuotientArgs normalised() const {
         QuotientArgs b = *this;
         if (!b.main_nx) b.main_nx = b.main_lde.data;
@@ -70,6 +71,7 @@
 constexpr uint32_t COLMAP_LIVE_COUNT = 0, COLMAP_CONST_COUNT = 1, COLMAP_LIVE = 2;
 inline size_t lde_colmap_words(uint64_t width) { return 2 + 2 * (size_t)width; }
 void launch_lde_colmap(hipStream_t st, const uint32_t* varies, uint64_t width, uint32_t* colmap);
+void launch_lde_tw4(hipStream_t st, uint32_t* tw4, int k, int log_blowup, const DeviceTables& tb, const LdeTables& lt);
 void launch_verify_chunk(hipStream_t st, const VerifyChunkArgs& a);
 void launch_keccak_leaves(hipStream_t st, const uint32_t* const* cols_dev, int n_elems, uint64_t n_rows, uint32_t* digests);
 void launch_keccak_leaves_strided(hipStream_t st, const uint32_t* base, uint64_t stride, int n_elems, uint64_t n_rows, uint32_t* digests);
@@ -112,6 +114,7 @@
 void launch_perm_trace(hipStream_t st, DMatView main, DMatView prep, const uint32_t* iw_dev, const uint32_t* chal_dev, uint32_t M, DMatView perm,
                        uint32_t* scratch, int native_chip = -2);
 void launch_quotient(hipStream_t st, const QuotientArgs& a, const DeviceTables& tb);
+void launch_quotient_selectors(hipStream_t st, uint32_t* qsel, int log_n, uint32_t coset_shift, uint32_t g_inv, const DeviceTables& tb);
 void launch_check_constraints(hipStream_t st, const QuotientArgs& a, unsigned long long* first_bad_dev);
 struct TgCpuOp { uint32_t pc, fp, opcode; int32_t operands[5]; uint32_t kind, has_imm, imm, mem_first; };
 struct TgMemOp { uint32_t clk, addr, value, is_write; };
diff --git a/valida_amd/csrc/kernels/ntt.hip b/valida_amd/csrc/kernels/ntt.hip
--- a/valida_amd/csrc/kernels/ntt.hip
+++ b/valida_amd/csrc/kernels/ntt.hip
@@ -446,7 +446,7 @@
     }
 }
 
-template <bool MAPPED>
+template <bool MAPPED, bool TW4 = false>
 __global__ void __launch_bounds__(256) k_lde_mid12(DMatView src, DMatView dst, int k, int lb, DeviceTables tb, LdeTables lt, const uint32_t* colmap) {
     extern __shared__ uint32_t lds[];
     constexpr int K_LO = 12, N_LO = 1 << K_LO;
@@ -490,7 +490,8 @@
         }
         butterflies<4, false, true>(x, tb.itwc, 0, 0);
         const uint32_t ca = __brev((uint32_t)p) >> (32 - k_hi);
-        const Fp step = root_pow(tb, k, (ca * 256u) & nmask), tw0 = root_pow(tb, k, (ca * (uint32_t)tid) & nmask);
+        Fp step, tw0;
+        if constexpr (!TW4) { step = root_pow(tb, k, (ca * 256u) & nmask); tw0 = root_pow(tb, k, (ca * (uint32_t)tid) & nmask); }
         for (int tc = 0; tc < b; tc++) {
             Fp y[16];
             {
@@ -505,6 +506,12 @@
                 for (int g = 0; g < 16; g++) p0[g] = y[g].v;
             }
             __syncthreads();
+            uint32_t f4[16];
+            if constexpr (TW4) {
+                const uint32_t* fp = lt.tw4 + (((size_t)tc * n_hi + p) << K_LO) + tid;
+#pragma unroll
+                for (int g = 0; g < 16; g++) f4[g] = fp[256 * g];
+            }
             ntt_round<4, true, true, 4>(lds, tb.twc, 12, 5, 0, 0);
             {
                 const uint32_t* p0 = lds + tile_addr<true>(tid, 0, 0);
@@ -513,9 +520,14 @@
             }
             butterflies<4, true, false>(y, tb.twc, tid, 8, held_out);
             uint32_t* out = dst.col(cidx) + (uint64_t)tc * N + p * N_LO + tid;
-            Fp cur = Fp::raw(lt.sig[(size_t)tc * n_hi + ca]) * tw0;
-#pragma unroll
-            for (int g = 0; g < 16; g++) { out[256 * g] = (y[g] * cur).v; cur *= step; }
+            if constexpr (TW4) {
+#pragma unroll
+                for (int g = 0; g < 16; g++) out[256 * g] = (y[g] * Fp::raw(f4[g])).v;
+            } else {
+                Fp cur = Fp::raw(lt.sig[(size_t)tc * n_hi + ca]) * tw0;
+#pragma unroll
+                for (int g = 0; g < 16; g++) { out[256 * g] = (y[g] * cur).v; cur *= step; }
+            }
             __syncthreads();
         }
     }
@@ -759,6 +771,20 @@
     }
 }
 
+__global__ void __launch_bounds__(256) k_lde_tw4(uint32_t* __restrict__ tw4, int k, DeviceTables tb, LdeTables lt) {
+    const int k_hi = k - 12, n_hi = 1 << k_hi, tid = threadIdx.x;
+    const uint32_t p = blockIdx.x, tc = blockIdx.y, nmask = (uint32_t)((1ull << k) - 1), ca = __brev(p) >> (32 - k_hi);
+    const Fp step = root_pow(tb, k, (ca * 256u) & nmask), tw0 = root_pow(tb, k, (ca * (uint32_t)tid) & nmask);
+    uint32_t* out = tw4 + (((size_t)tc * n_hi + p) << 12) + tid;
+    Fp cur = Fp::raw(lt.sig[(size_t)tc * n_hi + ca]) * tw0;
+    for (int g = 0; g < 16; g++) { out[256 * g] = cur.v; cur *= step; }
+}
+void launch_lde_tw4(hipStream_t st, uint32_t* tw4, int k, int log_blowup, const DeviceTables& tb, const LdeTables& lt) {
+    if (k <= 12 || lde_k_lo(k) != 12) throw std::invalid_argument("lde tw4: the table belongs to the 2^12-point middle pass (heights 2^13 .. 2^22)");
+    ProfScope ps("k_lde_tw4", st, 4.0 * (double)((uint64_t)1 << (k + log_blowup)));
+    VK_LAUNCH(k_lde_tw4, dim3(1u << (k - 12), 1u << log_blowup), dim3(256), 0, st, tw4, k, tb, lt);
+}
+
 void launch_lde_colmap(hipStream_t st, const uint32_t* varies, uint64_t width, uint32_t* colmap) {
     if (width == 0 || width > 16384) throw std::invalid_argument("lde colmap: width out of range");
     ProfScope ps("k_lde_colmap", st, 4.0 * 3 * width);
@@ -801,8 +827,10 @@
     if (p.k_lo == 12) {
         if (gm.x > 4096u) gm.x = 4096u;
         ProfScope ps("k_lde_mid12", st, nw * (1.0 + b));
-        if (colmap) VK_LAUNCH(k_lde_mid12<true>, gm, dim3(256), (size_t)padded_words(4096) * 4, st, s1, s2, k, log_blowup, tb, lt, colmap);
-        else VK_LAUNCH(k_lde_mid12<false>, gm, dim3(256), (size_t)padded_words(4096) * 4, st, s1, s2, k, log_blowup, tb, lt, colmap);
+#define VG_LDE_MID12(M, W) VK_LAUNCH((k_lde_mid12<M, W>), gm, dim3(256), (size_t)padded_words(4096) * 4, st, s1, s2, k, log_blowup, tb, lt, colmap)
+        if (colmap) { if (lt.tw4) VG_LDE_MID12(true, true); else VG_LDE_MID12(true, false); }
+        else { if (lt.tw4) VG_LDE_MID12(false, true); else VG_LDE_MID12(false, false); }
+#undef VG_LDE_MID12
     } else if (p.k_lo == 14) {
         ProfScope ps("k_lde_mid14", st, nw * (1.0 + b));
         const size_t lds14 = 2 * (size_t)padded_words(16384) * 4;
diff --git a/valida_amd/csrc/kernels/quotient.hip b/valida_amd/csrc/kernels/quotient.hip
--- a/valida_amd/csrc/kernels/quotient.hip
+++ b/valida_amd/csrc/kernels/quotient.hip
@@ -328,7 +328,7 @@
 #ifndef VGPU_QUOT_PT_WAVES
 #define VGPU_QUOT_PT_WAVES 6
 #endif
-template <int CHIP>
+template <int CHIP, bool QSEL = false>
 __global__ void __launch_bounds__(512)
 #if VGPU_QUOT_PT_WAVES > 0
 __attribute__((amdgpu_waves_per_eu(VGPU_QUOT_PT_WAVES)))
@@ -355,7 +355,9 @@
     const Fp x0 = s * domain_point(tb, (uint32_t)(2 * m));
     const Fp x = pt ? -x0 : x0;
     const Fp d0 = x - Fp::one(), d1 = x - g_inv;
-    const Fp inv = (d0 * d1).inv();
+    Fp inv;
+    if constexpr (QSEL) inv = Fp::raw(a.qsel[j]);
+    else inv = (d0 * d1).inv();
     const uint32_t par = i & 1u;
     PointCtx p;
     p.row = j;
@@ -391,6 +393,20 @@
     const uint64_t pos = a.out_natural ? (uint64_t)i0 : m;
 #pragma unroll
     for (int c = 0; c < 5; c++) a.out.data[(uint64_t)(col0 + c) * a.out.stride + pos] = outv[c].v;
+}
+
+__global__ void __launch_bounds__(256) k_quotient_selectors(uint32_t* __restrict__ qsel, int log_n, uint32_t coset_shift, uint32_t g_inv_raw, DeviceTables tb) {
+    const uint64_t j = (uint64_t)blockIdx.x * 256 + threadIdx.x;
+    if (j >= (2ull << log_n)) return;
+    const Fp x0 = Fp::raw(coset_shift) * domain_point(tb, (uint32_t)j & ~1u);
+    const Fp x = (j & 1) ? -x0 : x0;
+    const Fp d0 = x - Fp::one(), d1 = x - Fp::raw(g_inv_raw);
+    qsel[j] = (d0 * d1).inv().v;
+}
+void launch_quotient_selectors(hipStream_t st, uint32_t* qsel, int log_n, uint32_t coset_shift, uint32_t g_inv, const DeviceTables& tb) {
+    const uint64_t rows = 2ull << log_n;
+    ProfScope ps("k_quotient_selectors", st, 4.0 * rows);
+    VK_LAUNCH(k_quotient_selectors, dim3((unsigned)((rows + 255) / 256)), dim3(256), 0, st, qsel, log_n, coset_shift, g_inv, tb);
 }
 
 template <int RFKIND>
@@ -547,7 +563,7 @@
     if (a.native_chip != QuotientArgs::INTERPRET && per_point) {
         const dim3 grid((unsigned)((n + 255) / 256)), block(512);
         switch (a.native_chip) {
-#define VG_NATIVE_PT(C) case vchips::C: VK_LAUNCH((k_quotient_pt<vchips::C>), grid, block, 0, st, a, tb); break;
+#define VG_NATIVE_PT(C) case vchips::C: if (a.qsel) VK_LAUNCH((k_quotient_pt<vchips::C, true>), grid, block, 0, st, a, tb); else VK_LAUNCH((k_quotient_pt<vchips::C>), grid, block, 0, st, a, tb); break;
             VG_NATIVE_PT(CHIP_CPU) VG_NATIVE_PT(CHIP_ADD) VG_NATIVE_PT(CHIP_SUB) VG_NATIVE_PT(CHIP_MUL) VG_NATIVE_PT(CHIP_SHIFT) VG_NATIVE_PT(CHIP_LT)
             VG_NATIVE_PT(CHIP_COM) VG_NATIVE_PT(CHIP_BITWISE) VG_NATIVE_PT(CHIP_OUTPUT) VG_NATIVE_PT(CHIP_STATIC_DATA)
             VG_NATIVE_PT(CHIP_PROGRAM) VG_NATIVE_PT(CHIP_MEM) VG_NATIVE_PT(CHIP_DIV) VG_NATIVE_PT(CHIP_RANGE)
```

New measurement: 70.59 proofs/s (median of 5 runs). No clear change (+0.5%).
